# tqch/v-diffusion-torch

Measured on AMD Instinct MI355X. Metric: train_images_per_sec, higher is better.
Workload: dtype fp32 (bf16x3 split products in the tile-engine GEMMs)

## Files before the change

### include/vdiff_hip.h

```cpp
#ifndef VDIFF_HIP_H
#define VDIFF_HIP_H
#include <stddef.h>
#include <stdint.h>

#ifdef __cplusplus
extern "C" {
#endif

#define VD_VERSION 100

int         vd_version(void);
const char* vd_last_error(void);

int         vd_set_reserved_cus(int32_t n);
int         vd_reserved_cus(void);

int         vd_mfma_calibrate(float* sink, unsigned long long* stamps, int32_t blocks, int32_t iters, uint32_t seed, void* stream);

enum { VD_ROW = 0,
       VD_COL = 1,
       VD_IM2COL = 2 };

typedef struct vd_gemm_desc {
    const float* A; const float* B; float* C;
// ... 23 lines not shown
size_t vd_gemm_grouped_wgrad_ws_bytes(int32_t count, int32_t M, int32_t N, int32_t splitk);
int vd_gemm_grouped_wgrad_auto_split(int32_t count, int32_t M, int32_t N, int32_t K, int32_t min_slabs, int32_t max_slabs);
int vd_gemm_grouped_wgrad(const float* const* A, const float* const* B, float* const* C, float* const* colsum, int32_t count,
                          int32_t M, int32_t N, int32_t K, int64_t lda, int64_t ldb, int64_t ldc, int32_t splitk, float* ws, size_t ws_bytes,
                          void* stream);

int vd_conv3x3(const float* xin, int64_t ldx, const float* wpack, const float* bias,
               const float* res, int64_t ldres, float* y, int64_t ldy,
               int32_t nimg, int32_t H, int32_t W, int32_t Cin, int32_t Cout, int32_t accumulate,
               float* stats_part , void* stream);

int vd_conv3x3_wino_supported(int32_t nimg, int32_t H, int32_t W, int32_t Cin, int32_t Cout, int64_t ldx, int64_t ldy, int64_t ldres);
int vd_conv3x3_wino(const float* xin, int64_t ldx, const float* U, const float* bias, const float* res, int64_t ldres,
                    float* y, int64_t ldy, int32_t nimg, int32_t H, int32_t W, int32_t Cin, int32_t Cout,
                    float* stats_part, void* stream);
int vd_conv3x3_wgrad_wino_supported(int32_t nimg, int32_t H, int32_t W, int32_t Cin, int32_t Cout, int64_t ldx, int64_t lddy);
size_t vd_conv3x3_wgrad_wino_ws_bytes(int32_t nimg, int32_t H, int32_t W, int32_t Cin, int32_t Cout);
int vd_conv3x3_wgrad_wino(const float* xin, int64_t ldx, const float* dy, int64_t lddy, int32_t nimg, int32_t H, int32_t W,
                          int32_t Cin, int32_t Cout, float* dw_oihw, float* dbias, int32_t Cin_w, int32_t Cout_w,
                          int32_t accumulate, float* ws, size_t ws_bytes, void* stream);
int vd_conv3x3_wgrad_wino_phase(const float* xin, int64_t ldx, const float* dy, int64_t lddy, int32_t nimg, int32_t H, int32_t W,
                                int32_t Cin, int32_t Cout, float* dw_oihw, float* dbias, int32_t Cin_w, int32_t Cout_w,
                                int32_t accumulate, float* ws, size_t ws_bytes, int32_t phase, void* stream);
int vd_wino_last_kernel(void);
int vd_wino_wgrad_last_kernel(void);
#ifdef VD_PROBES
int vd_wino_set_probe(unsigned long long* buf);
int vd_wino43_set_probe(unsigned long long* buf);
int vd_gn_set_spin_probe(unsigned* buf);
#endif
int vd_wino_pack(const float* w_oihw, int32_t Cout, int32_t Cin, float* uf , float* ud , void* stream);
int vd_conv3x3_dgrad_wino43_supported(int32_t nimg, int32_t H, int32_t W, int32_t Cin, int32_t Cout, int64_t lddy, int64_t lddx);
size_t vd_wino43_u_floats(int32_t Cout, int32_t Cin);
int vd_conv3x3_dgrad_wino43(const float* dy, int64_t lddy, const float* U43, float* dx, int64_t lddx, int32_t nimg, int32_t H, int32_t W,
                            int32_t Cin, int32_t Cout, void* stream);
int vd_wino43_last_kernel(void);
int vd_wino43_pack(const float* w_oihw, int32_t Cout, int32_t Cin, float* U43, void* stream);
int vd_wino43_pack_batched(const int64_t* items_dev, int32_t n, int64_t total_blocks, void* stream);
int vd_conv3x3_wino43_preferred(int32_t nimg, int32_t H, int32_t W, int32_t N);
int vd_conv3x3_wino43_fwd_supported(int32_t nimg, int32_t H, int32_t W, int32_t Cin, int32_t Cout, int64_t ldx, int64_t ldy, int64_t ldres);
int vd_wino43_pack_fwd(const float* w_oihw, int32_t Cout, int32_t Cin, float* U43f, void* stream);
int vd_conv3x3_wino43_fwd_chunk_rows(int32_t H, int32_t W);
int vd_conv3x3_wino43_fwd(const float* xin, int64_t ldx, const float* U43f, const float* bias, const float* res, int64_t ldres, float* y,
                          int64_t ldy, int32_t nimg, int32_t H, int32_t W, int32_t Cin, int32_t Cout, float* stats_part, void* stream);
int vd_conv3x3_wgrad_wino43_supported(int32_t nimg, int32_t H, int32_t W, int32_t Cin, int32_t Cout, int64_t ldx, int64_t lddy);
size_t vd_conv3x3_wgrad_wino43_ws_bytes(int32_t nimg, int32_t H, int32_t W, int32_t Cin, int32_t Cout);
int vd_conv3x3_wgrad_wino43(const float* xin, int64_t ldx, const float* dy, int64_t lddy, int32_t nimg, int32_t H, int32_t W,
                            int32_t Cin, int32_t Cout, float* dw_oihw, float* dbias, int32_t Cin_w, int32_t Cout_w,
                            int32_t accumulate, float* ws, size_t ws_bytes, void* stream);
int vd_conv3x3_wgrad_wino43_phase(const float* xin, int64_t ldx, const float* dy, int64_t lddy, int32_t nimg, int32_t H, int32_t W,
                                  int32_t Cin, int32_t Cout, float* dw_oihw, float* dbias, int32_t Cin_w, int32_t Cout_w,
                                  int32_t accumulate, float* ws, size_t ws_bytes, int32_t phase, void* stream);
int vd_wino43_wgrad_last_kernel(void);

int vd_wino_pack_batched(const int64_t* items_dev, int32_t n, int64_t total_blocks, void* stream);

int vd_im2col3x3(const float* x, int64_t ldx, float* xc , int32_t nimg, int32_t H, int32_t W, int32_t C, void* stream);
int vd_tap_gather(const float* z, int64_t ldz, const float* bias, float* out, int64_t ldo, int32_t nimg, int32_t H, int32_t W, int32_t Cout, void* stream);
int vd_tap_spread(const float* dy, int64_t lddy, float* dz, int64_t ldz, int32_t nimg, int32_t H, int32_t W, int32_t Cout, void* stream);
int vd_thin_wgrad_finish(const float* g, int32_t Cout_w, int32_t Cin, int32_t Cin_w, float* dw_oihw, int32_t accumulate,
                         const float* colsum, int32_t cs_stride, int32_t cs_off, float* dbias, void* stream);

size_t vd_conv3x3_wgrad_ws_bytes(int32_t nimg, int32_t H, int32_t W, int32_t Cin, int32_t Cout);
int vd_conv3x3_wgrad(const float* xin, int64_t ldx, const float* dy, int64_t lddy,
                     int32_t nimg, int32_t H, int32_t W, int32_t Cin, int32_t Cout,
                     float* dw_oihw, float* dbias, int32_t Cin_w, int32_t Cout_w, int32_t accumulate,
                     float* ws, size_t ws_bytes, void* stream);
int vd_conv3x3_wgrad_phase(const float* xin, int64_t ldx, const float* dy, int64_t lddy,
                           int32_t nimg, int32_t H, int32_t W, int32_t Cin, int32_t Cout,
                           float* dw_oihw, float* dbias, int32_t Cin_w, int32_t Cout_w, int32_t accumulate,
                           float* ws, size_t ws_bytes, int32_t phase, void* stream);

int vd_pack_conv3x3(const float* w_oihw, int32_t Cout_w, int32_t Cin_w,
                    float* wf, int32_t Cin_p, float* wd, int32_t Cout_p, void* stream);
int vd_pack_conv3x3_batched(const int64_t* items_dev, int32_t n, int64_t total_blocks, void* stream);

enum { VD_RS_NONE = 0, VD_RS_DOWN = 1, VD_RS_UP = 2 };

size_t vd_gn_ws_bytes(int32_t nimg, int32_t HW, int32_t C);
int vd_gn_stats(const float* x, int64_t ldx, int32_t nimg, int32_t HW, int32_t C, int32_t G, float eps,
                float* stats, float* ws, size_t ws_bytes, void* stream);

int vd_gn_stats_from_partials(const float* part1, int32_t C1, int32_t chunks1, const float* part2, int32_t C2, int32_t chunks2,
                              int32_t nimg, int32_t HW, int32_t G, float eps, float* stats, void* stream);

int vd_gn_coef_from_partials(const float* part1, int32_t C1, int32_t chunks1, const float* part2, int32_t C2, int32_t chunks2,
                             int32_t nimg, int32_t HW, int32_t G, float eps, const float* gamma, const float* beta,
                             const float* film, float* coef, void* stream);

int vd_gn_apply(const float* x, int64_t ldx, const float* stats, const float* gamma, const float* beta,
                const float* film, int32_t act, float p_drop, uint64_t seed,
                int32_t resample, float* y, int64_t ldy,
                int32_t nimg, int32_t H, int32_t W, int32_t C, int32_t G, float* coef, void* stream);

int vd_gn_apply_from_partials(const float* x, int64_t ldx, const float* part1, int32_t C1, int32_t chunks1, const float* part2, int32_t C2,
                              int32_t chunks2, const float* gamma, const float* beta, const float* film, int32_t act, float p_drop,
                              uint64_t seed, int32_t resample, float* y, int64_t ldy, int32_t nimg, int32_t H, int32_t W, int32_t C,
                              int32_t G, float eps, float* coef, void* stream);

int vd_gn_apply_bwd(const float* dy, int64_t lddy, const float* x, int64_t ldx, const float* coef,
                    const float* gamma, const float* beta, const float* film, int32_t act, float p_drop, uint64_t seed,
                    int32_t resample, const float* add, int64_t ldadd, float* dx, int64_t lddx, int32_t accumulate_dx,
                    float* dfilm, float* dgamma, float* dbeta, int32_t accumulate_params,
                    int32_t nimg, int32_t H, int32_t W, int32_t C, int32_t G,
                    float* ws, size_t ws_bytes, void* stream);
int vd_gn_bwd_last_kernel(void);
int vd_gn_apply_bwd_keep(const float* dy, int64_t lddy, const float* x, int64_t ldx, const float* coef, const float* gamma,
                         const float* beta, const float* film, int32_t act, float p_drop, uint64_t seed, int32_t resample,
                         const float* add, int64_t ldadd, float* dx, int64_t lddx, int32_t accumulate_dx, float* dfilm, float* pgb_keep,
                         int32_t nimg, int32_t H, int32_t W, int32_t C, int32_t G, float* ws, size_t ws_bytes, void* stream);
int vd_gn_param_sums_batched(const int64_t* items_dev, int32_t n, int64_t total_blocks, void* stream);

size_t vd_colsum_ws_bytes(int64_t M, int32_t N);
int vd_colsum(const float* x, int64_t ldx, int64_t M, int32_t N, float* out, int32_t accumulate,
              float* ws, size_t ws_bytes, void* stream);
int vd_axpby(const float* x, int64_t ldx, float alpha, float* y, int64_t ldy, float beta, int64_t rows, int32_t C, void* stream);
int vd_silu(const float* x, float* y, int64_t n, void* stream);
int vd_silu_bwd(const float* x, const float* dy, float* dx, int64_t n, int32_t accumulate, void* stream);
int vd_softmax_rows(float* s, int64_t rows, int32_t L, void* stream);
int vd_softmax_rows_bwd(const float* p, float* dp, int64_t rows, int32_t L, float alpha, void* stream);

int vd_attn_supported(int32_t L, int32_t hd, int32_t backward);
int vd_attn_fwd(const float* q, const float* k, const float* v, int64_t ld, float* o, int64_t ldo, float* lse, int32_t B,
                int32_t nh, int32_t L, int32_t hd, float scale, void* stream);
int vd_attn_bwd(const float* q, const float* k, const float* v, int64_t ld, const float* o, int64_t ldo, const float* dout,
                int64_t lddo, const float* lse, float* delta, float* dq, float* dk, float* dv, int64_t ldd, int32_t B,
                int32_t nh, int32_t L, int32_t hd, float scale, void* stream);
int vd_attn_bwd_phase(const float* q, const float* k, const float* v, int64_t ld, const float* o, int64_t ldo, const float* dout,
                      int64_t lddo, const float* lse, float* delta, float* dq, float* dk, float* dv, int64_t ldd, int32_t B,
                      int32_t nh, int32_t L, int32_t hd, float scale, int32_t phase, void* stream);

int vd_nchw_to_nhwc(const float* x, float* y, int32_t nimg, int32_t C, int32_t H, int32_t W, int64_t ldy, void* stream);
int vd_nhwc_to_nchw(const float* x, int64_t ldx, float* y, int32_t nimg, int32_t C, int32_t H, int32_t W, void* stream);

int vd_images_to_uint8_hwc(const float* x_nchw, uint8_t* out_hwc, int32_t n, int32_t C, int32_t HW, void* stream);
int vd_images_from_uint8_hwc(const uint8_t* in_hwc, const uint8_t* flip, float* out_nchw, int32_t n, int32_t C,
                             int32_t H, int32_t W, void* stream);

int vd_timestep_embedding(const double* t, float* out, int32_t n, int32_t dim, double scale, void* stream);
int vd_class_embed(const float* y, const float* w, const float* bias, float* temb, int32_t n, int32_t emb, int32_t ncls, void* stream);
int vd_class_embed_bwd(const float* y, const float* dtemb, float* dw, float* dbias, int32_t n, int32_t emb, int32_t ncls,
                       int32_t accumulate, void* stream);
int vd_multitag_norm(const float* y, float* out, int32_t n, int32_t ncls, void* stream);

int vd_q_sample(const float* x0, const float* eps, const float* logsnr, float* xt, int32_t n, int32_t C, int32_t HW, void* stream);
int vd_loss_fwd(const float* x0, const float* eps, const float* xt, const float* out, const float* logsnr,
                int32_t model_out_type, int32_t reweight, float* loss, float* aux, int32_t n, int32_t C, int32_t HW, void* stream);
int vd_loss_bwd(const float* x0, const float* eps, const float* xt, const float* out, const float* logsnr,
                const float* aux, const float* gloss, int32_t model_out_type, int32_t reweight, float* dout,
                int32_t n, int32_t C, int32_t HW, void* stream);
int vd_bpd_terms(const float* x0, const float* xt, const float* out, const float* coef, int32_t model_out_type, int32_t clip,
// ... 36 lines not shown
```

### v-diffusion-torch_amd/csrc/common.h

```cpp
#pragma once
#include <hip/hip_runtime.h>
#include <stdint.h>
#include <stdio.h>
#include "../../include/vdiff_hip.h"

typedef float f32x4 __attribute__((ext_vector_type(4)));
typedef float f32x16 __attribute__((ext_vector_type(16)));

typedef float f32x2 __attribute__((ext_vector_type(2)));

#ifdef VD_PROBES
constexpr bool VD_PROBE_BUILD = true;
#else
constexpr bool VD_PROBE_BUILD = false;
#endif

void vd_set_error(const char* fmt, ...);
int vd_cu_count(void);
int vd_persistent_cus(void);
int vd_gemm_grouped_wgrad_kblk(const float* const* A, const float* const* B, float* const* C, float* const* colsum, int32_t count, int32_t M,
                               int32_t N, int32_t K, int64_t lda, int64_t ldb, int64_t ldc, int32_t splitk, float* ws, size_t ws_bytes,
                               void* stream, int64_t a_kblk, int64_t b_kblk, int32_t slabs_only);
int vd_gemm_grouped_wgrad_used_slabs(int32_t count, int32_t M, int32_t N, int32_t K, int32_t splitk);
extern thread_local int vd_g_last_tile;
inline int vd_tile_code(bool tr, bool spl, int kt, int bm, int bn) {
    return ((((tr ? 1 : 0) + (spl ? 2 : 0)) * 100 + kt) * 1000 + bm) * 1000 + bn;
}

#define VD_REQUIRE(cond, ...)                                   \
    do { if (!(cond)) { vd_set_error(__VA_ARGS__); return 1; } } while (0)

#define VD_LAUNCH_CHECK(name)                                                            \
    do { hipError_t e_ = hipGetLastError();                                              \
         if (e_ != hipSuccess) { vd_set_error("%s: %s", name, hipGetErrorString(e_)); return 2; } } while (0)

static inline bool vd_aligned16(const void* p) { return (reinterpret_cast<uintptr_t>(p) & 15) == 0; }

__device__ __forceinline__ float vd_sigmoid(float x) { return __builtin_amdgcn_rcpf(1.0f + __expf(-x)); }

__device__ __forceinline__ void vd_philox4(uint64_t seed, uint64_t ctr, uint32_t out[4]) {
    uint32_t k0 = (uint32_t)seed, k1 = (uint32_t)(seed >> 32);
    uint32_t c0 = (uint32_t)ctr, c1 = (uint32_t)(ctr >> 32), c2 = 0x243F6A88u, c3 = 0x85A308D3u;
#pragma unroll
    for (int r = 0; r < 10; ++r) {
        uint64_t p0 = (uint64_t)0xD2511F53u * c0, p1 = (uint64_t)0xCD9E8D57u * c2;
        uint32_t n0 = (uint32_t)(p1 >> 32) ^ c1 ^ k0, n2 = (uint32_t)(p0 >> 32) ^ c3 ^ k1;
        c1 = (uint32_t)p1; c3 = (uint32_t)p0; c0 = n0; c2 = n2;
        k0 += 0x9E3779B9u; k1 += 0xBB67AE85u;
    }
    out[0] = c0; out[1] = c1; out[2] = c2; out[3] = c3;
}
__device__ __forceinline__ f32x4 vd_dropout_scale4(uint64_t seed, uint64_t vec_index, float p) {
    uint32_t r[4];
    vd_philox4(seed, vec_index, r);
    const float inv = 1.0f / (1.0f - p);
    f32x4 m;
#pragma unroll
    for (int j = 0; j < 4; ++j) m[j] = ((r[j] >> 8) * (1.0f / 16777216.0f) >= p) ? inv : 0.0f;
    return m;
}
```

### v-diffusion-torch_amd/csrc/gemm.hip

```cpp
#include "common.h"
#include <math.h>
#include <stdlib.h>
#include <type_traits>

namespace {

constexpr int KT = 32;
#ifndef VD_GEMM_SPLIT_DEFAULT
#define VD_GEMM_SPLIT_DEFAULT 1
#endif

struct GemmArgs {
    const float* A; const float* B; float* C; const float* bias; const float* R;
    int M, N, K;
    long long lda, ldb, ldc, ldr;
    int nh;
    long long sAb, sAh, sBb, sBh, sCb, sCh, sRb, sRh;
    float alpha; int accumulate;
    int H, W, Cin;
    int kt_total, kt_per_split;
    long long slab_stride;
    float* colsum; int colsum_accumulate;
    int probe;
    float* stats; int stats_hw;
    long long sBias;
    int group_S;
    int lgW, lgHW;
    long long a_kblk, b_kblk;
};

__device__ __forceinline__ int PB(const GemmArgs& p) { return VD_PROBE_BUILD ? p.probe : 0; }

__device__ __forceinline__ int row_swz(int row, int chunk) { return row * KT + ((chunk ^ ((row >> 1) & 7)) << 2); }

template <int BM, int BN, int AK, int BK, bool SPLITK>
__global__ __launch_bounds__(256, 2) void gemm_kernel(const GemmArgs p) {
    __shared__ __attribute__((aligned(16))) float smem[2 * (BM + BN) * KT];
    float* As = smem;
    float* Bs = smem + 2 * BM * KT;

    constexpr int MT = BM / 64, NT = BN / 64;
    constexpr int AIT = BM / 32, BIT = BN / 32;
    constexpr int A_CPR = BM / 4, A_RPP = 256 / A_CPR;
    constexpr int B_CPR = BN / 4, B_RPP = 256 / B_CPR;

    const int tid = threadIdx.x, lane = tid & 63, wave = tid >> 6;
    const int li = lane & 31, lh = lane >> 5;
    const int wm = (wave >> 1) * (BM / 2), wn = (wave & 1) * (BN / 2);
    const int m0 = blockIdx.y * BM;
    int n0 = blockIdx.x * BN;
    int tapN = 0, ci0 = 0;
    if (BK == VD_IM2COL) {
        const int cchN = (p.Cin + BN - 1) / BN;
        tapN = blockIdx.x / cchN;
        ci0 = (blockIdx.x % cchN) * BN;
        n0 = tapN * p.Cin + ci0;
    }
    const float* A = p.A;
    const float* B = p.B;
    float* C = p.C;
    const float* R = p.R;
    const float* biasp = p.bias;
    int kt_begin = 0, kt_end = p.kt_total;
    if (SPLITK) {
        kt_begin = blockIdx.z * p.kt_per_split;
        kt_end = min(kt_begin + p.kt_per_split, p.kt_total);
        C += (long long)blockIdx.z * p.slab_stride;
    } else {
        const int zb = blockIdx.z / p.nh, zh = blockIdx.z % p.nh;
        A += zb * p.sAb + zh * p.sAh;
        B += zb * p.sBb + zh * p.sBh;
        C += zb * p.sCb + zh * p.sCh;
        if (R) R += zb * p.sRb + zh * p.sRh;
        if (biasp) biasp += zb * p.sBias;
    }

    const int r_row = tid >> 3, r_chunk = tid & 7;
    int ay[AIT], ax[AIT];
    if (AK == VD_IM2COL) {
#pragma unroll
        for (int it = 0; it < AIT; ++it) {
// ... 338 lines not shown
    } else {
        const int zb = tbz / p.nh, zh = tbz % p.nh;
        A += zb * p.sAb + zh * p.sAh;
        B += zb * p.sBb + zh * p.sBh;
        C += zb * p.sCb + zh * p.sCh;
        if (R) R += zb * p.sRb + zh * p.sRh;
        if (biasp) biasp += zb * p.sBias;
    }

    unsigned voA[AIT], voB[BIT];
    unsigned mkA[AIT];
    int kcA[AIT], kcB[BIT];
    int by[BIT], bx[BIT];
    int tapA = (AK == VD_IM2COL) ? kt_begin % 9 : 0, ccA = (AK == VD_IM2COL) ? kt_begin / 9 : 0;
    const int kinc_x = (BK == VD_IM2COL) ? KT % p.W : 0, kinc_y = (BK == VD_IM2COL) ? KT / p.W : 0;
#pragma unroll
    for (int j = 0; j < AIT; ++j) {
        const int q = j * 4 + wave;
        if (AK == VD_COL) {
            const int kk = q * A_RPP + lane / A_LPR, cm = (lane % A_LPR) * 4;
            const int rowoff = (GROUPED && p.a_kblk) ? (kk >> 4) * (int)p.a_kblk + (kk & 15) * (int)p.lda : kk * (int)p.lda;
            voA[j] = (m0 + cm < p.M) ? (unsigned)(rowoff + cm) * 4u : OOB;
            kcA[j] = kk; mkA[j] = 0;
        } else {
            const int row = q * RRPP + lane / RLPR;
            const int c = (lane % RLPR) ^ swz_of<KT>(row);
            const int m = m0 + row;
            kcA[j] = c * 4;
            voA[j] = (m < p.M) ? (unsigned)(row * (int)p.lda + c * 4) * 4u : OOB;
            unsigned mk = 0;
            if (AK == VD_IM2COL) {
                int y, x;
                pix_yx(p, m, y, x);
                const unsigned xm = (x > 0 ? 1u : 0u) | 2u | (x < p.W - 1 ? 4u : 0u);
                mk = (y > 0 ? xm : 0u) | (xm << 3) | (y < p.H - 1 ? xm << 6 : 0u);
            }
            mkA[j] = mk;
        }
    }
#pragma unroll
    for (int j = 0; j < BIT; ++j) {
        const int q = j * 4 + wave;
        if (BK == VD_ROW) {
            const int row = q * RRPP + lane / RLPR;
            const int c = (lane % RLPR) ^ swz_of<KT>(row);
            kcB[j] = c * 4;
            voB[j] = (n0 + row < p.N) ? (unsigned)(row * (int)p.ldb + c * 4) * 4u : OOB;
            by[j] = bx[j] = 0;
        } else {
            const int kk = q * B_RPP + lane / B_LPR, cn = (lane % B_LPR) * 4;
            kcB[j] = kk;
            const bool ok = (BK == VD_IM2COL) ? (ci0 + cn < p.Cin) : (n0 + cn < p.N);
            const int rowoff = (GROUPED && BK == VD_COL && p.b_kblk) ? (kk >> 4) * (int)p.b_kblk + (kk & 15) * (int)p.ldb : kk * (int)p.ldb;
            voB[j] = ok ? (unsigned)(rowoff + cn) * 4u : OOB;
            if (BK == VD_IM2COL) pix_yx(p, kt_begin * KT + kk, by[j], bx[j]);
            else by[j] = bx[j] = 0;
        }
    }
    const float* Ablk = (AK == VD_COL) ? A + m0 : A + (long long)m0 * p.lda;
    const float* Bblk = (BK == VD_ROW) ? B + (long long)n0 * p.ldb : ((BK == VD_COL) ? B + n0 : B + ci0);
    const long long tapoffB = (BK == VD_IM2COL) ? (long long)((tapN / 3 - 1) * p.W + (tapN % 3 - 1)) * p.ldb : 0;

#ifndef VD_ISSUE_IN
#define VD_ISSUE_IN 2
#endif
    constexpr bool ISSUE_IN = VD_ISSUE_IN == 2 ? (AK == VD_COL) : (VD_ISSUE_IN == 1);
    struct Prep { const float* pA; const float* pB; unsigned vA[AIT], vB[BIT]; };
    auto prep_tiles = [&](int kt, Prep& P) {
        {
            const int tap = tapA, c0 = ccA * KT;
            long long aoff;
            int kwidth;
            if (AK == VD_IM2COL) { aoff = (long long)((tap / 3 - 1) * p.W + (tap % 3 - 1)) * p.lda + c0; kwidth = p.Cin - c0; }
            else if (AK == VD_ROW) { aoff = (long long)kt * KT; kwidth = p.K - kt * KT; }
            else { aoff = (GROUPED && p.a_kblk) ? (long long)kt * (KT / 16) * p.a_kblk : (long long)kt * KT * p.lda; kwidth = p.K - kt * KT; }
            P.pA = Ablk + aoff;
#pragma unroll
            for (int j = 0; j < AIT; ++j) {
                unsigned vo = voA[j];
                if (kcA[j] >= kwidth) vo = OOB;
                if (AK == VD_IM2COL && !((mkA[j] >> tap) & 1u)) vo = OOB;
                P.vA[j] = vo;
            }
        }
        {
            long long boff;
            int kwidth;
            if (BK == VD_ROW) {
                if (AK == VD_IM2COL) { boff = (long long)tapA * p.Cin + ccA * KT; kwidth = p.Cin - ccA * KT; }
                else { boff = (long long)kt * KT; kwidth = p.K - kt * KT; }
            } else { boff = ((GROUPED && BK == VD_COL && p.b_kblk) ? (long long)kt * (KT / 16) * p.b_kblk : (long long)kt * KT * p.ldb) + tapoffB; kwidth = p.K - kt * KT; }
            P.pB = Bblk + boff;
            const int dy = tapN / 3 - 1, dx = tapN % 3 - 1;
            if (BK == VD_IM2COL && p.lgW >= 0) {
#pragma unroll
                for (int j = 0; j < BIT; ++j) {
                    const int k0 = kt * KT + (j * 4 + wave) * B_RPP;
                    unsigned long long lanes = 0;
#pragma unroll
                    for (int u = 0; u < B_RPP; ++u) {
                        const int k = k0 + u;
                        const int rem = k & ((1 << p.lgHW) - 1), y = (rem >> p.lgW) + dy, x = (rem & ((1 << p.lgW) - 1)) + dx;
                        const bool ok = k < p.K && (unsigned)y < (unsigned)p.H && (unsigned)x < (unsigned)p.W;
                        lanes |= ok ? (((B_LPR == 64 ? 0ull : (1ull << (B_LPR & 63))) - 1ull) << (u * (B_LPR & 63))) : 0ull;
                    }
                    unsigned vo;
                    const unsigned oob = OOB;
                    asm("v_cndmask_b32 %0, %1, %2, %3" : "=v"(vo) : "v"(oob), "v"(voB[j]), "s"(lanes));
                    P.vB[j] = vo;
                }
            } else
#pragma unroll
            for (int j = 0; j < BIT; ++j) {
// ... 359 lines not shown
                    v = (v * al + bb) + ad;
                    if (want_stats) {
                        if (!edge) { st1p += v; st2p += v * v; }
                        else {
                            if (rs0 + row_lane < rows_valid) { st1 += v[0]; st2 += v[0] * v[0]; }
                            if (rs1 + row_lane < rows_valid) { st1 += v[1]; st2 += v[1] * v[1]; }
                        }
                    }
                }
                const float v0 = v[0], v1 = v[1];
                __builtin_amdgcn_raw_buffer_store_b32(__float_as_uint(v0), crs, (int)voc, rs0 * ldc4, 0);
                __builtin_amdgcn_raw_buffer_store_b32(__float_as_uint(v1), crs, (int)voc, rs1 * ldc4, 0);
            }
        }
        st1 += st1p[0] + st1p[1];
        st2 += st2p[0] + st2p[1];
        if (want_stats && nok) {
            st1 += __shfl_xor(st1, 32, 64);
            st2 += __shfl_xor(st2, 32, 64);
            const int mrow = m0 + wm;
            if (lh == 0 && mrow < p.M) {
                const int chunks = p.stats_hw / (BM / 2);
                float* o = p.stats + ((long long)(mrow / p.stats_hw) * chunks + (mrow % p.stats_hw) / (BM / 2)) * 2 * p.N + n;
                o[0] = st1; o[p.N] = st2;
            }
        }
    }
    stamp_end();
}

template <int BM, int BN, int AK, int BK, bool SPLITK, int KT, bool TR, bool GROUPED = false>
__global__ __launch_bounds__(256, (KT == 16 ? VD_KT16_BLOCKS : 2)) void gemm_dma_kernel(const GemmArgs p,
                                                                                          const std::conditional_t<GROUPED, GroupPtrs, NoGroup> gp) {
    gemm_dma_body<BM, BN, AK, BK, SPLITK, KT, TR, GROUPED, false>(p, gp);
}
template <int BM, int BN, int AK, int BK, bool SPLITK, int KT, bool TR, bool GROUPED = false>
__global__ __launch_bounds__(256, (KT == 16 ? VD_SPL_BLOCKS : 2)) void gemm_split_kernel(const GemmArgs p,
                                                                                           const std::conditional_t<GROUPED, GroupPtrs, NoGroup> gp) {
    gemm_dma_body<BM, BN, AK, BK, SPLITK, KT, TR, GROUPED, true>(p, gp);
}

__global__ __launch_bounds__(512) void wgrad_planes256_kernel(const GemmArgs p, const GroupPtrs gp) {
    constexpr int BM = 256, BN = 256, KTT = 16, NBUF = 3, STG = (BM + BN) * KTT;
    __shared__ __attribute__((aligned(1024))) float smem[NBUF * STG];
    typedef float f32x2 __attribute__((ext_vector_type(2)));
    const int tid = threadIdx.x, lane = tid & 63;
    const int wave = __builtin_amdgcn_readfirstlane(tid >> 6);
    const int li = lane & 31, lh = lane >> 5;
    const int wm = (wave >> 1) * 64, wn = (wave & 1) * 128;
    const int tbx = blockIdx.x, tby = blockIdx.y, tbz = blockIdx.z;
    const int m0 = tby * BM, n0 = tbx * BN;
    const int e = tbz / p.group_S, slab = tbz - e * p.group_S;
    const float* A = gp.A[e] + m0;
    const float* B = gp.B[e] + n0;
    const int kt_begin = slab * p.kt_per_split, kt_end = min(kt_begin + p.kt_per_split, p.kt_total);
    float* C = p.C + (long long)tbz * p.slab_stride;

    auto issue = [&](int kt, int buf) {
        float* as = smem + buf * STG;
        float* bs = as + BM * KTT;
        const int rec = kt < kt_end ? (int)OOB : 0;
        const __amdgpu_buffer_rsrc_t rsA = make_rsrc(A + (p.a_kblk ? (long long)kt * p.a_kblk : (long long)kt * KTT * p.lda), rec);
        const __amdgpu_buffer_rsrc_t rsB = make_rsrc(B + (p.b_kblk ? (long long)kt * p.b_kblk : (long long)kt * KTT * p.ldb), rec);
#pragma unroll
        for (int h = 0; h < 2; ++h) {
            const int kk = wave + 8 * h;
            __builtin_amdgcn_raw_ptr_buffer_load_lds(rsA, (lds_ptr_t)(as + kk * BM), 16, lane * 16, kk * (int)p.lda * 4, 0, 0);
            __builtin_amdgcn_raw_ptr_buffer_load_lds(rsB, (lds_ptr_t)(bs + kk * BN), 16, lane * 16, kk * (int)p.ldb * 4, 0, 0);
        }
    };

    f32x16 acc[2][4];
#pragma unroll
    for (int a = 0; a < 2; ++a)
#pragma unroll
        for (int b = 0; b < 4; ++b)
#pragma unroll
            for (int r = 0; r < 16; ++r) acc[a][b][r] = 0.f;
    float csum[2] = {0.f, 0.f};
    const bool do_cs = p.colsum != nullptr && tbx == 0 && (wave & 1) == 0;

    if (kt_begin < kt_end) {
        issue(kt_begin, 0);
        issue(kt_begin + 1, 1);
        asm volatile("s_waitcnt vmcnt(4)" ::: "memory");
        asm volatile("s_waitcnt lgkmcnt(0)\n\ts_barrier" ::: "memory");
        int buf = 0;
        for (int kt = kt_begin; kt < kt_end; ++kt) {
            const float* as = smem + buf * STG;
            const float* bs = as + BM * KTT;
            issue(kt + 2, buf >= 1 ? buf - 1 : 2);
            float fa[2][8];
            f32x4 fbq[8];
#pragma unroll
            for (int j = 0; j < 8; ++j) {
                const f32x2 v = *reinterpret_cast<const f32x2*>(as + (8 * lh + j) * BM + wm + 2 * li);
                fa[0][j] = v[0]; fa[1][j] = v[1];
                fbq[j] = *reinterpret_cast<const f32x4*>(bs + (8 * lh + j) * BN + wn + 4 * li);
            }
            bf16x8 ah[2], am[2], al[2];
#pragma unroll
            for (int a = 0; a < 2; ++a) split8(fa[a], ah[a], am[a], al[a]);
            if (do_cs) {
                asm volatile("" ::: "memory");
#pragma unroll
                for (int a = 0; a < 2; ++a)
                    csum[a] += ((fa[a][0] + fa[a][1]) + (fa[a][2] + fa[a][3])) + ((fa[a][4] + fa[a][5]) + (fa[a][6] + fa[a][7]));
            }
#pragma unroll
            for (int hb = 0; hb < 2; ++hb) {
                bf16x8 bh[2], bm[2], bl[2];
#pragma unroll
                for (int b2 = 0; b2 < 2; ++b2) {
                    float fb[8];
#pragma unroll
                    for (int j = 0; j < 8; ++j) fb[j] = fbq[j][2 * hb + b2];
                    split8(fb, bh[b2], bm[b2], bl[b2]);
                }
#pragma unroll
                for (int a = 0; a < 2; ++a)
#pragma unroll
// ... 360 lines not shown
        if (eff > best) best = eff;
    }
    return best >= 0.85;
}

void grouped_tiles(int tile, bool p256, int M, int N, long long* nm, long long* nn) {
    const int bm = p256 ? 256 : TILES[tile].bm, bn = p256 ? 256 : TILES[tile].bn;
    *nm = (M + bm - 1) / bm; *nn = (N + bn - 1) / bn;
}

struct GroupedPlan { int tile; bool p256, k16; long long nm, nn; int kt_total, kt_per_split, used; };
GroupedPlan plan_grouped(int count, int M, int N, int K, int S) {
    GroupedPlan g;
    g.tile = choose_tile(M, N, false, (long long)count * S, 0);
    g.p256 = planes256(count, M, N, K);
    grouped_tiles(g.tile, g.p256, M, N, &g.nm, &g.nn);
    g.k16 = g.p256 || (g.tile == 0 && g.nm * g.nn * count * S >= GROUPED_K16_MIN_WGS);
    g.kt_total = g.k16 ? (K + 15) / 16 : (K + 31) / 32;
    g.kt_per_split = (g.kt_total + S - 1) / S;
    g.used = (g.kt_total + g.kt_per_split - 1) / g.kt_per_split;
    return g;
}
}

extern "C" int vd_gemm_grouped_wgrad_auto_split(int32_t count, int32_t M, int32_t N, int32_t K, int32_t min_slabs, int32_t max_slabs) {
    const int tile = choose_tile(M, N, false, (long long)count * 8, 0);
    const bool p256 = planes256(count, M, N, K);
    long long nm, nn;
    grouped_tiles(tile, p256, M, N, &nm, &nn);
    const long long blocks = nm * nn * count;
    const long long slots = (long long)vd_cu_count() * (p256 ? 1 : (tile == 0 && blocks * (min_slabs > 1 ? min_slabs : 1) >= GROUPED_K16_MIN_WGS / 2 ? 4 : TILES[tile].per_cu));
    int lo = min_slabs > 1 ? min_slabs : 1, hi = max_slabs > lo ? max_slabs : lo;
    const int kmax = K / 256 > 1 ? K / 256 : 1;
    if (hi > kmax) hi = kmax;
    if (lo > hi) lo = hi;
    int best = lo;
    double best_eff = -1.0;
    for (int s = lo; s <= hi; ++s) {
        const long long wgs = blocks * s, rounds = (wgs + slots - 1) / slots;
        double eff = (double)wgs / (double)(rounds * slots);
        eff *= 1.0 - 0.004 * s;
        if (eff > best_eff) { best_eff = eff; best = s; }
    }
    return best;
}

extern "C" size_t vd_gemm_grouped_wgrad_ws_bytes(int32_t count, int32_t M, int32_t N, int32_t splitk) {
    return (size_t)count * (splitk > 1 ? splitk : 1) * ((size_t)M * N + M) * sizeof(float);
}

extern "C" int vd_gemm_grouped_wgrad(const float* const* A, const float* const* B, float* const* C, float* const* colsum, int32_t count,
                                     int32_t M, int32_t N, int32_t K, int64_t lda, int64_t ldb, int64_t ldc, int32_t splitk, float* ws,
                                     size_t ws_bytes, void* stream) {
    return vd_gemm_grouped_wgrad_kblk(A, B, C, colsum, count, M, N, K, lda, ldb, ldc, splitk, ws, ws_bytes, stream, 0, 0, 0);
}

int vd_gemm_grouped_wgrad_used_slabs(int32_t count, int32_t M, int32_t N, int32_t K, int32_t splitk) {
    return plan_grouped(count, M, N, K, splitk > 1 ? splitk : 1).used;
}

int vd_gemm_grouped_wgrad_kblk(const float* const* A, const float* const* B, float* const* C, float* const* colsum, int32_t count,
                               int32_t M, int32_t N, int32_t K, int64_t lda, int64_t ldb, int64_t ldc, int32_t splitk, float* ws,
                               size_t ws_bytes, void* stream, int64_t a_kblk, int64_t b_kblk, int32_t slabs_only) {
    VD_REQUIRE(A && B && C && count > 0 && count <= VD_GROUP_MAX, "vd_gemm_grouped_wgrad: 1..%d entries (got %d)", VD_GROUP_MAX, count);
    VD_REQUIRE(M > 0 && N > 0 && K > 0 && M % 4 == 0 && N % 4 == 0 && lda % 4 == 0 && ldb % 4 == 0 && ldc >= N,
               "vd_gemm_grouped_wgrad: M, N, lda, ldb must be multiples of 4 (M=%d N=%d)", M, N);
    const int S = splitk > 1 ? splitk : 1;
    VD_REQUIRE(ws && ws_bytes >= vd_gemm_grouped_wgrad_ws_bytes(count, M, N, S), "vd_gemm_grouped_wgrad: workspace too small");
    GemmArgs a = {};
    GroupPtrs gp = {};
    GroupOut go = {};
    for (int e = 0; e < count; ++e) {
        VD_REQUIRE(A[e] && B[e] && C[e] && vd_aligned16(A[e]) && vd_aligned16(B[e]), "vd_gemm_grouped_wgrad: entry %d: null / unaligned operand", e);
        gp.A[e] = A[e]; gp.B[e] = B[e]; go.C[e] = C[e]; go.cs[e] = colsum ? colsum[e] : nullptr;
    }
    a.A = A[0]; a.B = B[0];
    a.M = M; a.N = N; a.K = K; a.lda = lda; a.ldb = ldb; a.ldc = N; a.ldr = 0; a.nh = 1;
    a.alpha = 1.f; a.lgW = a.lgHW = -1; a.probe = 0;
    a.a_kblk = a_kblk; a.b_kblk = b_kblk;
    VD_REQUIRE(a_kblk >= 0 && b_kblk >= 0 && a_kblk % 4 == 0 && b_kblk % 4 == 0 && 2 * a_kblk + 16 * lda + 128 < 0x70000000LL / 4 &&
               2 * b_kblk + 16 * ldb + 128 < 0x70000000LL / 4, "vd_gemm_grouped_wgrad: K-block strides outside the LDS-DMA kernel's range");
    VD_REQUIRE(dma_in_range(a), "vd_gemm_grouped_wgrad: operands outside the LDS-DMA kernel's range (alignment / row pitch)");
    const GroupedPlan g = plan_grouped(count, M, N, K, S);
    const int used = g.used;
    a.kt_total = g.kt_total; a.kt_per_split = g.kt_per_split; a.group_S = used;
    a.slab_stride = (long long)M * N;
    a.C = ws;
    float* cpart = ws + (long long)count * used * a.slab_stride;
    a.colsum = colsum ? cpart : nullptr;
    const dim3 grid((unsigned)g.nn, (unsigned)g.nm, (unsigned)(count * used));
    hipStream_t st = (hipStream_t)stream;
    if (g.p256) {
        vd_g_last_tile = vd_tile_code(true, true, 16, 256, 256);
        hipLaunchKernelGGL(wgrad_planes256_kernel, grid, dim3(512), 0, st, a, gp);
    } else if (g.tile == 0 && g.k16) launch_grouped<128, 128, 16>(a, gp, grid, st);
    else if (g.tile == 0) launch_grouped<128, 128>(a, gp, grid, st);
    else if (g.tile == 1) launch_grouped<128, 64>(a, gp, grid, st);
    else if (g.tile == 2) launch_grouped<64, 128>(a, gp, grid, st);
    else launch_grouped<64, 64>(a, gp, grid, st);
    VD_LAUNCH_CHECK("gemm_dma_kernel(grouped)");
    if (slabs_only) return 0;
    const long long tot = (long long)M * N;
    hipLaunchKernelGGL(reduce_slabs_grouped_kernel, dim3((unsigned)((tot + 255) / 256), (unsigned)count), dim3(256), 0, st, ws, used,
                       a.slab_stride, M, N, go, (long long)ldc, cpart);
    VD_LAUNCH_CHECK("reduce_slabs_grouped_kernel");
    return 0;
}

thread_local int vd_g_last_tile = 0;
extern "C" int vd_gemm_last_tile(void) { return vd_g_last_tile; }

extern "C" int vd_gemm(const vd_gemm_desc* d, void* stream) {
    VD_REQUIRE(d != nullptr, "vd_gemm: null descriptor");
    return run_gemm(*d, (hipStream_t)stream);
}

extern "C" int vd_conv3x3(const float* xin, int64_t ldx, const float* wpack, const float* bias, const float* res,
                          int64_t ldres, float* y, int64_t ldy, int32_t nimg, int32_t H, int32_t W, int32_t Cin,
                          int32_t Cout, int32_t accumulate, float* stats_part, void* stream) {
    VD_REQUIRE(Cin % 4 == 0, "vd_conv3x3: Cin must be a multiple of 4 (got %d)", Cin);
    vd_gemm_desc d = {};
    d.A = xin; d.B = wpack; d.C = y; d.bias = bias; d.R = res;
    d.M = nimg * H * W; d.N = Cout; d.K = 9 * Cin;
    d.a_kind = VD_IM2COL; d.b_kind = VD_ROW;
    d.lda = ldx; d.ldb = 9LL * Cin; d.ldc = ldy; d.ldr = ldres;
    d.batch = 1; d.nh = 1; d.alpha = 1.f; d.accumulate = accumulate;
    d.H = H; d.W = W; d.Cin = Cin;
    d.stats = stats_part; d.stats_hw = H * W;
    if (stats_part && (H * W) % 64 != 0) d.tile = 64;
    return run_gemm(d, (hipStream_t)stream);
}

// ... 107 lines not shown
```

### v-diffusion-torch_amd/csrc/norm.hip

```cpp
#include "common.h"
#include <stdlib.h>

namespace {

constexpr int PPC = 128;

template <bool NT>
__device__ __forceinline__ f32x4 ld_stream(const float* p) {
    if (NT) return __builtin_nontemporal_load(reinterpret_cast<const f32x4*>(p));
    return *reinterpret_cast<const f32x4*>(p);
}
template <bool NT>
__device__ __forceinline__ void st_stream(float* p, f32x4 v) {
    if (NT) __builtin_nontemporal_store(v, reinterpret_cast<f32x4*>(p));
    else *reinterpret_cast<f32x4*>(p) = v;
}

struct ReduceArgs {
    const float* x; long long ldx;
    const float* dy; long long lddy;
    const float* coef;
    int act; float p_drop; unsigned long long seed; int resample; int has_norm;
    int H, W;
    long long HW;
// ... 134 lines not shown
    const int idx = blockIdx.x * 4 + (threadIdx.x >> 6), lane = threadIdx.x & 63;
    if (idx >= nimg * G) return;
    const int b = idx / G, g = idx % G, C = C1 + C2, cg = C / G;
    double s1 = 0.0, s2 = 0.0;
    const int cbeg = g * cg;
    const int n1 = ch1 * cg, n2 = ch2 * cg;
    for (int e = lane; e < max(n1, n2); e += 64) {
        const int c = cbeg + e % cg, ch = e / cg;
        const bool first = c < C1;
        const int Cs = first ? C1 : C2, cs = first ? c : c - C1, chunks = first ? ch1 : ch2;
        if (ch < chunks) {
            const float* q = (first ? p1 : p2) + ((long long)(b * chunks + ch) * 2) * Cs + cs;
            s1 += (double)q[0]; s2 += (double)q[Cs];
        }
    }
#pragma unroll
    for (int o = 32; o > 0; o >>= 1) { s1 += __shfl_xor(s1, o, 64); s2 += __shfl_xor(s2, o, 64); }
    const double n = (double)cg * (double)HW;
    const double mean_d = s1 / n;
    double var = s2 / n - mean_d * mean_d;
    if (var < 0.0) var = 0.0;
    const float mean = (float)mean_d, rstd = (float)(1.0 / sqrt(var + (double)eps));
    if (stats && lane == 0) { stats[2 * idx] = mean; stats[2 * idx + 1] = rstd; }
    if (coef) {
        for (int c = cbeg + lane; c < cbeg + cg; c += 64) {
            float sc = rstd * gamma[c];
            float of = beta[c] - mean * sc;
            if (film) {
                const float shift = film[(long long)b * 2 * C + c], scale = film[(long long)b * 2 * C + C + c];
                sc *= (1.f + scale);
                of = of * (1.f + scale) + shift;
            }
            float* o = coef + (long long)b * 4 * C + c;
            o[0] = sc; o[C] = of; o[2 * C] = rstd; o[3 * C] = -mean * rstd;
        }
    }
}

__global__ void gn_coef_kernel(const float* stats, const float* gamma, const float* beta, const float* film, int nimg,
                               int C, int G, float* coef) {
    const int idx = blockIdx.x * blockDim.x + threadIdx.x;
    if (idx >= nimg * C) return;
    const int b = idx / C, c = idx % C, g = c / (C / G);
    const float mean = stats[2 * (b * G + g)], rstd = stats[2 * (b * G + g) + 1];
    float sc = rstd * gamma[c];
    float of = beta[c] - mean * sc;
    if (film) {
        const float shift = film[(long long)b * 2 * C + c], scale = film[(long long)b * 2 * C + C + c];
        sc *= (1.f + scale);
        of = of * (1.f + scale) + shift;
    }
    float* o = coef + (long long)b * 4 * C + c;
    o[0] = sc; o[C] = of; o[2 * C] = rstd; o[3 * C] = -mean * rstd;
}

struct ApplyArgs {
    const float* x; long long ldx; const float* coef; int has_norm; int act; float p_drop; unsigned long long seed;
    int resample; float* y; long long ldy; int nimg, H, W, C;
};
struct PartArgs {
    const float* p1; int C1, ch1; const float* p2; int C2, ch2; int G; float eps;
    const float* gamma; const float* beta; const float* film; float* coef_out;
};

__device__ __forceinline__ f32x4 fwd_val(const ApplyArgs& p, f32x4 v, int pix, int c4, f32x4 sc, f32x4 of, int b) {
    if (p.has_norm) v = v * sc + of;
    if (p.act) {
#pragma unroll
        for (int j = 0; j < 4; ++j) v[j] = v[j] * vd_sigmoid(v[j]);
    }
    if (p.p_drop > 0.f) {
        const unsigned long long vi = ((unsigned long long)b * p.H * p.W + pix) * (p.C >> 2) + (c4 >> 2);
        v *= vd_dropout_scale4(p.seed, vi, p.p_drop);
    }
    return v;
}
__device__ __forceinline__ f32x4 fwd_one(const ApplyArgs& p, const float* ximg, int pix, int c4, f32x4 sc, f32x4 of, int b) {
    return fwd_val(p, *reinterpret_cast<const f32x4*>(ximg + (long long)pix * p.ldx + c4), pix, c4, sc, of, b);
}

constexpr int APIX = 64;

template <bool FROM_PARTS>
__global__ __launch_bounds__(256) void gn_apply_kernel(const ApplyArgs p, int Cb, const PartArgs q) {
    __shared__ double ps[FROM_PARTS ? 2 : 1][FROM_PARTS ? 1024 : 1];
    __shared__ float gst[FROM_PARTS ? 2 : 1][FROM_PARTS ? 256 : 1];
    const int b = blockIdx.y, c0 = blockIdx.z * Cb;
    const int cbw = min(Cb, p.C - c0);
    const int vecs = cbw >> 2, rows = 256 / vecs;
    const int r = threadIdx.x / vecs, c4 = c0 + 4 * (threadIdx.x % vecs);
    const int Ho = p.resample == VD_RS_DOWN ? p.H >> 1 : (p.resample == VD_RS_UP ? p.H << 1 : p.H);
    const int Wo = p.resample == VD_RS_DOWN ? p.W >> 1 : (p.resample == VD_RS_UP ? p.W << 1 : p.W);
    const int p0 = blockIdx.x * APIX, np = min(APIX, Ho * Wo - p0);
    f32x4 sc = {1.f, 1.f, 1.f, 1.f}, of = {0.f, 0.f, 0.f, 0.f};
    if (FROM_PARTS) {
        const int C = p.C, cg = C / q.G;
        for (int cl = threadIdx.x; cl < cbw; cl += 256) {
            const int c = c0 + cl;
            const bool first = c < q.C1;
            const int Cs = first ? q.C1 : q.C2, cs = first ? c : c - q.C1, chunks = first ? q.ch1 : q.ch2;
            const float* src = (first ? q.p1 : q.p2) + (long long)b * chunks * 2 * Cs + cs;
            double s1 = 0.0, s2 = 0.0;
            for (int ch = 0; ch < chunks; ++ch) { s1 += (double)src[(long long)ch * 2 * Cs]; s2 += (double)src[(long long)ch * 2 * Cs + Cs]; }
            ps[0][cl] = s1; ps[1][cl] = s2;
        }
        __syncthreads();
        const int ng = cbw / cg;
        for (int g = threadIdx.x; g < ng; g += 256) {
            double s1 = 0.0, s2 = 0.0;
            for (int c = g * cg; c < (g + 1) * cg; ++c) { s1 += ps[0][c]; s2 += ps[1][c]; }
            const double n = (double)cg * (double)p.H * (double)p.W;
            const double mean = s1 / n;
            double var = s2 / n - mean * mean;
            if (var < 0.0) var = 0.0;
            gst[0][g] = (float)mean; gst[1][g] = (float)(1.0 / sqrt(var + (double)q.eps));
        }
        __syncthreads();
        if (r >= rows) return;
        f32x4 nr, nm;
#pragma unroll
        for (int j = 0; j < 4; ++j) {
            const int c = c4 + j, g = (c - c0) / cg;
            const float mean = gst[0][g], rstd = gst[1][g];
            float s_ = rstd * q.gamma[c];
            float o_ = q.beta[c] - mean * s_;
            if (q.film) {
                const float shift = q.film[(long long)b * 2 * C + c], scale = q.film[(long long)b * 2 * C + C + c];
                s_ *= (1.f + scale);
                o_ = o_ * (1.f + scale) + shift;
            }
            sc[j] = s_; of[j] = o_; nr[j] = rstd; nm[j] = -mean * rstd;
        }
        if (blockIdx.x == 0 && r == 0 && q.coef_out) {
            float* o = q.coef_out + (long long)b * 4 * C + c4;
            *reinterpret_cast<f32x4*>(o) = sc; *reinterpret_cast<f32x4*>(o + C) = of;
            *reinterpret_cast<f32x4*>(o + 2 * C) = nr; *reinterpret_cast<f32x4*>(o + 3 * C) = nm;
        }
    } else {
        if (r >= rows) return;
        if (p.has_norm) {
            const float* cf = p.coef + (long long)b * 4 * p.C;
            sc = *reinterpret_cast<const f32x4*>(cf + c4);
            of = *reinterpret_cast<const f32x4*>(cf + p.C + c4);
        }
    }
    const float* ximg = p.x + (long long)b * p.H * p.W * p.ldx;
    float* yimg = p.y + (long long)b * Ho * Wo * p.ldy;
    if (p.resample == VD_RS_NONE) {
        for (int i = r; i < np; i += 4 * rows) {
            f32x4 v[4];
#pragma unroll
            for (int u = 0; u < 4; ++u)
                if (i + u * rows < np) v[u] = *reinterpret_cast<const f32x4*>(ximg + (long long)(p0 + i + u * rows) * p.ldx + c4);
#pragma unroll
            for (int u = 0; u < 4; ++u)
                if (i + u * rows < np) {
                    const int po = p0 + i + u * rows;
                    *reinterpret_cast<f32x4*>(yimg + (long long)po * p.ldy + c4) = fwd_val(p, v[u], po, c4, sc, of, b);
                }
        }
        return;
    }
    for (int i = r; i < np; i += rows) {
        const int po = p0 + i;
        f32x4 out;
        {
            const int yo = po / Wo, xo = po - yo * Wo;
            if (p.resample == VD_RS_UP) out = fwd_one(p, ximg, (yo >> 1) * p.W + (xo >> 1), c4, sc, of, b);
            else {
                const int q = (2 * yo) * p.W + 2 * xo;
                out = (fwd_one(p, ximg, q, c4, sc, of, b) + fwd_one(p, ximg, q + 1, c4, sc, of, b) +
                       fwd_one(p, ximg, q + p.W, c4, sc, of, b) + fwd_one(p, ximg, q + p.W + 1, c4, sc, of, b)) * 0.25f;
            }
        }
        *reinterpret_cast<f32x4*>(yimg + (long long)po * p.ldy + c4) = out;
    }
}

__global__ __launch_bounds__(256) void gn_bwd_finalize_kernel(const float* part, int chunks, const float* coef,
                                                              const float* gamma, const float* beta, const float* film,
                                                              int C, int G, long long HW, float* q, float* dfilm,
                                                              float* pgb) {
    extern __shared__ float sh[];
    float* k1 = sh; float* k2 = sh + C; float* gm = sh + 2 * C;
    const int b = blockIdx.x, cg = C / G;
    const float* cf = coef + (long long)b * 4 * C;
    for (int c = threadIdx.x; c < C; c += blockDim.x) {
        float s1 = 0.f, s2 = 0.f;
        for (int ch = 0; ch < chunks; ++ch) {
            const float* pp = part + ((long long)(b * chunks + ch) * 2) * C;
            s1 += pp[c]; s2 += pp[C + c];
        }
        float fs = 1.f;
        if (film) {
            fs = 1.f + film[(long long)b * 2 * C + C + c];
            dfilm[(long long)b * 2 * C + c] = s1;
            dfilm[(long long)b * 2 * C + C + c] = gamma[c] * s2 + beta[c] * s1;
        }
        const float k = gamma[c] * fs;
        k1[c] = k * s1; k2[c] = k * s2;
        pgb[((long long)b * 2) * C + c] = fs * s2;
        pgb[((long long)b * 2 + 1) * C + c] = fs * s1;
    }
    __syncthreads();
    if (threadIdx.x < G) {
        float m1 = 0.f, m2 = 0.f;
        for (int c = threadIdx.x * cg; c < (threadIdx.x + 1) * cg; ++c) { m1 += k1[c]; m2 += k2[c]; }
        const float inv = 1.f / ((float)cg * (float)HW);
        gm[threadIdx.x] = m1 * inv; gm[G + threadIdx.x] = m2 * inv;
    }
    __syncthreads();
    for (int c = threadIdx.x; c < C; c += blockDim.x) {
        const int g = c / cg;
        const float rstd = cf[2 * C + c];
        const float fs = film ? 1.f + film[(long long)b * 2 * C + C + c] : 1.f;
        float* qq = q + (long long)b * 3 * C + c;
        qq[0] = rstd * gamma[c] * fs; qq[C] = rstd * gm[g]; qq[2 * C] = rstd * gm[G + g];
    }
}

__global__ __launch_bounds__(256) void sum_over_images_kernel(const float* pgb, int nimg, int C, float* dgamma, float* dbeta,
                                                              int accumulate) {
    __shared__ float sh[2][16][17];
    const int cx = threadIdx.x & 15, ly = threadIdx.x >> 4;
    const int c = blockIdx.x * 16 + cx;
    float a = 0.f, bsum = 0.f;
    if (c < C)
        for (int b = ly; b < nimg; b += 16) { a += pgb[((long long)b * 2) * C + c]; bsum += pgb[((long long)b * 2 + 1) * C + c]; }
// ... 405 lines not shown
}

extern "C" int vd_gn_apply(const float* x, int64_t ldx, const float* stats, const float* gamma, const float* beta,
                           const float* film, int32_t act, float p_drop, uint64_t seed, int32_t resample, float* y,
                           int64_t ldy, int32_t nimg, int32_t H, int32_t W, int32_t C, int32_t G, float* coef,
                           void* stream) {
    hipStream_t st = (hipStream_t)stream;
    VD_REQUIRE(C % 4 == 0 && ldx % 4 == 0 && ldy % 4 == 0, "vd_gn_apply: C/ld must be multiples of 4");
    VD_REQUIRE(resample != VD_RS_DOWN || (H % 2 == 0 && W % 2 == 0), "vd_gn_apply: odd size cannot be average-pooled");
    const int has_norm = gamma != nullptr;
    if (has_norm && !stats) {
        VD_REQUIRE(coef != nullptr, "vd_gn_apply: neither statistics nor a coefficient table given");
    } else if (has_norm) {
        VD_REQUIRE(stats && beta && coef && C % G == 0, "vd_gn_apply: missing norm operands");
        hipLaunchKernelGGL(gn_coef_kernel, dim3((nimg * C + 255) / 256), dim3(256), 0, st, stats, gamma, beta, film, nimg, C,
                           G, coef);
        VD_LAUNCH_CHECK("gn_coef_kernel");
    }
    ApplyArgs p = {x, ldx, coef, has_norm, act, p_drop, seed, resample, y, ldy, nimg, H, W, C};
    const long long Ho = resample == VD_RS_DOWN ? H / 2 : (resample == VD_RS_UP ? H * 2 : H);
    const long long Wo = resample == VD_RS_DOWN ? W / 2 : (resample == VD_RS_UP ? W * 2 : W);
    const int Cba = pick_cb(C);
    VD_REQUIRE(C % Cba == 0 && Cba % 4 == 0 && Cba <= 1024 && nimg <= 65535, "vd_gn_apply: cannot split C=%d / nimg=%d", C, nimg);
    hipLaunchKernelGGL(gn_apply_kernel<false>, dim3((unsigned)((Ho * Wo + APIX - 1) / APIX), nimg, C / Cba), dim3(256), 0, st, p, Cba, PartArgs{});
    VD_LAUNCH_CHECK("gn_apply_kernel");
    return 0;
}

extern "C" int vd_gn_apply_from_partials(const float* x, int64_t ldx, const float* part1, int32_t C1, int32_t chunks1, const float* part2,
                                         int32_t C2, int32_t chunks2, const float* gamma, const float* beta, const float* film, int32_t act,
                                         float p_drop, uint64_t seed, int32_t resample, float* y, int64_t ldy, int32_t nimg, int32_t H,
                                         int32_t W, int32_t C, int32_t G, float eps, float* coef, void* stream) {
    hipStream_t st = (hipStream_t)stream;
    VD_REQUIRE(x && y && part1 && gamma && beta, "vd_gn_apply_from_partials: null operand");
    VD_REQUIRE(C % 4 == 0 && ldx % 4 == 0 && ldy % 4 == 0 && C % G == 0 && C1 + C2 == C && C1 > 0 && chunks1 > 0,
               "vd_gn_apply_from_partials: bad channel split C=%d C1=%d C2=%d G=%d", C, C1, C2, G);
    VD_REQUIRE(C2 == 0 || (part2 && chunks2 > 0), "vd_gn_apply_from_partials: second source incomplete");
    VD_REQUIRE(resample != VD_RS_DOWN || (H % 2 == 0 && W % 2 == 0), "vd_gn_apply_from_partials: odd size cannot be average-pooled");
    VD_REQUIRE(vd_aligned16(x) && vd_aligned16(y) && (!coef || vd_aligned16(coef)), "vd_gn_apply_from_partials: operands must be 16-byte aligned");
    ApplyArgs p = {x, ldx, coef, 1, act, p_drop, seed, resample, y, ldy, nimg, H, W, C};
    PartArgs q = {part1, C1, chunks1, part2, C2, chunks2, G, eps, gamma, beta, film, coef};
    const long long Ho = resample == VD_RS_DOWN ? H / 2 : (resample == VD_RS_UP ? H * 2 : H);
    const long long Wo = resample == VD_RS_DOWN ? W / 2 : (resample == VD_RS_UP ? W * 2 : W);
    const int cg = C / G;
    int Cba = pick_cb(C);
    if (Cba % cg) {
        Cba = 0;
        for (int k = G; k >= 1; --k) if (G % k == 0 && (k * cg) % 4 == 0 && k * cg <= 1024) { Cba = k * cg; break; }
    }
    VD_REQUIRE(Cba > 0 && C % Cba == 0 && Cba % 4 == 0 && Cba % cg == 0 && Cba <= 1024 && Cba / cg <= 256 && nimg <= 65535,
               "vd_gn_apply_from_partials: cannot split C=%d into whole-group channel ranges", C);
    hipLaunchKernelGGL(gn_apply_kernel<true>, dim3((unsigned)((Ho * Wo + APIX - 1) / APIX), nimg, C / Cba), dim3(256), 0, st, p, Cba, q);
    VD_LAUNCH_CHECK("gn_apply_kernel<from partials>");
    return 0;
}

static int gn_apply_bwd_impl(const float* dy, int64_t lddy, const float* x, int64_t ldx, const float* coef,
                             const float* gamma, const float* beta, const float* film, int32_t act, float p_drop,
                             uint64_t seed, int32_t resample, const float* add, int64_t ldadd, float* dx, int64_t lddx,
                             int32_t accumulate_dx, float* dfilm, float* dgamma, float* dbeta, int32_t accumulate_params,
                             int32_t nimg, int32_t H, int32_t W, int32_t C, int32_t G, float* ws, size_t ws_bytes,
                             float* pgb_keep, void* stream) {
    hipStream_t st = (hipStream_t)stream;
    VD_REQUIRE(C % 4 == 0 && lddy % 4 == 0 && lddx % 4 == 0, "vd_gn_apply_bwd: C/ld must be multiples of 4");
    const int has_norm = gamma != nullptr;
    const long long HW = (long long)H * W;
    BwdApplyArgs a = {};
    ReduceArgs& p = a.r;
    p.x = x; p.ldx = ldx; p.dy = dy; p.lddy = lddy; p.coef = coef; p.act = act; p.p_drop = p_drop; p.seed = seed;
    p.resample = resample; p.has_norm = has_norm; p.H = H; p.W = W; p.HW = HW; p.C = C; p.nimg = nimg;
    p.chunks = (int)((HW + PPC - 1) / PPC);
    a.add = add; a.ldadd = ldadd; a.dx = dx; a.lddx = lddx; a.accumulate_dx = accumulate_dx;
    g_last_gn_bwd = has_norm ? -1 : 0;
    if (has_norm) {
        VD_REQUIRE(x && coef && beta && ((dgamma && dbeta) || pgb_keep) && C % G == 0 && ldx % 4 == 0, "vd_gn_apply_bwd: missing norm operands");
        VD_REQUIRE(!film || dfilm, "vd_gn_apply_bwd: film given without dfilm");
        VD_REQUIRE(ws && ws_bytes >= vd_gn_ws_bytes(nimg, (int)HW, C), "vd_gn_apply_bwd: workspace too small");
        const int Cb = pick_cb(C);
        VD_REQUIRE(C % Cb == 0 && Cb % 4 == 0 && Cb <= 1024, "vd_gn_apply_bwd: cannot split C=%d", C);
        float* part = ws;
        float* q = part + (long long)nimg * p.chunks * 2 * C;
        float* pgb = pgb_keep ? pgb_keep : q + (long long)nimg * 3 * C;
        p.part = part;
        static const bool two_pass = getenv("VD_GN_TWO_PASS") != nullptr;
        int CS = fused_slab(C, G);
        static const bool wide = !(getenv("VD_GN_WIDE") && atoi(getenv("VD_GN_WIDE")) == 0);
        if (wide && CS > 0 && CS % 32 != 0 && C >= 384) {
            const int cg = C / G;
            for (int k = 1; k * cg <= 128 && k <= G; ++k)
                if ((k * cg) % 32 == 0 && C % (k * cg) == 0) { CS = k * cg; break; }
        }
        if (!two_pass && CS > 0 && nimg <= 65535) {
            static const bool big = getenv("VD_GN_TPB") && atoi(getenv("VD_GN_TPB")) == 1024;
            const int TPB = (HW * (CS / 4) > 2048 || (big && HW * (CS / 4) >= 1024)) ? 1024 : 256;
            const int rows = TPB / (CS / 4);
            const int npt = (int)((HW + rows - 1) / rows);
            static const bool no_split = getenv("VD_GN_SPLIT") && atoi(getenv("VD_GN_SPLIT")) == 0;
            if (npt > 8 && !no_split && resample == VD_RS_NONE && CS % 32 == 0) {
                int nsplit = 0;
                for (int k = 2; k <= 32; k *= 2)
                    if (HW % k == 0 && (HW / k + (1024 / (CS / 4)) - 1) / (1024 / (CS / 4)) <= 8) { nsplit = k; break; }
                const long long units = (long long)nimg * (C / CS), upad = (units + 7) / 8 * 8;
                const size_t cnt_bytes = ((size_t)upad * sizeof(unsigned) + 255) / 256 * 256;
                static const int split_occ = [] {
                    int occ = 0;
                    if (hipOccupancyMaxActiveBlocksPerMultiprocessor(&occ, gn_bwd_fused_kernel<8, 1024, true, true>, 1024, 0) != hipSuccess) occ = 0;
// ... 105 lines not shown
```

### v-diffusion-torch_amd/csrc/wino43.hip

```cpp
#include "common.h"
#include <type_traits>

namespace {

typedef __attribute__((address_space(3))) void* lds_ptr_t;
constexpr unsigned OOB = 0x80000000u;
constexpr int KT = 8;
constexpr int TN = 32;
constexpr int TILES = 64;
constexpr int U_STAGE = 36 * 4 * 16 * 2 * 2;
constexpr int THREADS = 512;

struct Args43 {
    const float* x; long long ldx;
    const float* U;
    float* y; long long ldy;
    int nimg, H, W, K, N;
    int items_per_img;
    int ngrp;
    int ncb, nitems;
    const float* bias; const float* res; long long ldr;
    float* stats;
    int chunks_per_img;
    unsigned long long* probe;
// ... 9 lines not shown
constexpr int U_AHEAD = 2;
template <int HALF, bool DY, typename T>
__device__ __forceinline__ void bt_half(const T (&d)[6], T& o0, T& o1, T& o2) {
    if (DY) {
        if (HALF == 0) {
            const T e1 = d[4] - 2.25f * d[2], f1 = d[3] - 2.25f * d[1];
            o0 = 1.265625f * d[0] + (d[4] - 2.8125f * d[2]);
            o1 = e1 + 0.75f * f1;
            o2 = e1 - 0.75f * f1;
        } else {
            const T e2 = d[4] - 0.5625f * d[2], f2 = d[3] - 0.5625f * d[1];
            o0 = e2 + 1.5f * f2;
            o1 = e2 - 1.5f * f2;
            o2 = 1.265625f * d[1] + (d[5] - 2.8125f * d[3]);
        }
    } else if (HALF == 0) {
        const T t = d[4] - 4.f * d[2], u = d[3] - 4.f * d[1];
        o0 = 4.f * d[0] + (d[4] - 5.f * d[2]);
        o1 = t + u;
        o2 = t - u;
    } else {
        const T c = d[4] - d[2], e = d[3] - d[1];
        o0 = c + 2.f * e;
        o1 = c - 2.f * e;
        o2 = 4.f * d[1] + (d[5] - 5.f * d[3]);
    }
}
template <bool DY, typename T>
__device__ __forceinline__ void bt_full(const T (&r)[6], T (&v)[6]) {
    if (DY) {
        const T e1 = r[4] - 2.25f * r[2], f1 = r[3] - 2.25f * r[1];
        const T e2 = r[4] - 0.5625f * r[2], f2 = r[3] - 0.5625f * r[1];
        v[0] = 1.265625f * r[0] + (r[4] - 2.8125f * r[2]);
        v[1] = e1 + 0.75f * f1;
        v[2] = e1 - 0.75f * f1;
        v[3] = e2 + 1.5f * f2;
        v[4] = e2 - 1.5f * f2;
        v[5] = 1.265625f * r[1] + (r[5] - 2.8125f * r[3]);
        return;
    }
    const T t = r[4] - 4.f * r[2], u = r[3] - 4.f * r[1], c = r[4] - r[2], e = r[3] - r[1];
    v[0] = 4.f * r[0] + (r[4] - 5.f * r[2]);
    v[1] = t + u;
    v[2] = t - u;
    v[3] = c + 2.f * e;
    v[4] = c - 2.f * e;
    v[5] = 4.f * r[1] + (r[5] - 5.f * r[3]);
}
template <int HALF, bool DY>
__device__ __forceinline__ void bt_half2(const f32x2 (&d)[6], f32x2& o0, f32x2& o1, f32x2& o2) { bt_half<HALF, DY, f32x2>(d, o0, o1, o2); }
template <bool DY>
__device__ __forceinline__ void bt_full2(const f32x2 (&r)[6], f32x2 (&v)[6]) { bt_full<DY, f32x2>(r, v); }

template <int TWT, bool FWD>
__global__ __launch_bounds__(THREADS) void wino43_conv_kernel(const Args43 p) {
    constexpr bool QUAD = TWT == 4;
    constexpr int RUN = TWT + 1;
    constexpr int RUNS = QUAD ? 4 * RUN - 2 : 4 * RUN;
    constexpr int RP = QUAD ? RUNS + 1 : RUNS + ((TWT / 4) & 3);
    constexpr int NTR = TILES / TWT;
    constexpr int RIN = QUAD ? 4 * 17 + 1 : 4 * NTR + 2;
    constexpr int NS = RIN * RP;
    constexpr int NPG = (NS + 63) / 64;
    constexpr int A_STAGE = 2 * NPG * 256;
    constexpr int STAGE = A_STAGE + U_STAGE;
    constexpr int LGT = TWT == 4 ? 2 : TWT == 8 ? 3 : 4;
    static_assert((4 * RP * 16) % 256 == (TWT * 16) % 256 || (QUAD && (4 * RP * 16) % 256 == 192), "row pitch leaves bank conflicts");
    static_assert(2 * STAGE * 4 <= 163840, "stages exceed the LDS");
    static_assert(8 * 16 * 64 * 16 + 8 * 4 * 8 * 4 <= 2 * STAGE * 4, "epilogue exchange + statistics area exceeds the stages");
    __shared__ __attribute__((aligned(1024))) float smem[2 * STAGE];

    const int tid = threadIdx.x, lane = tid & 63;
    const int wave = __builtin_amdgcn_readfirstlane(tid >> 6);
    const int li = lane & 15, lq = lane >> 4;
    const int tg = wave & 3;
    const int nkt = p.K / KT;
    const int G = gridDim.x;
    int probe_n = 0;
    auto stamp = [&](int slot) {
        if (VD_PROBE_BUILD && p.probe && probe_n < 4) {
            const unsigned long long t = slot == 12 ? __builtin_amdgcn_s_memrealtime() : __builtin_amdgcn_s_memtime();
            if (lane == 0) p.probe[(((long long)blockIdx.x * 8 + wave) * 4 + probe_n) * 16 + slot] = t;
        }
    };
    auto stamp_val = [&](int slot, unsigned long long v) {
        if (VD_PROBE_BUILD && p.probe && probe_n < 4 && lane == 0) p.probe[(((long long)blockIdx.x * 8 + wave) * 4 + probe_n) * 16 + slot] = v;
    };

    constexpr int APL = (NPG + 3) / 4;
    unsigned pxo[APL];
    const float* xitem = p.x;
    auto offsets = [&](int grp) {
        const int img = grp / p.items_per_img;
        const int part = grp - img * p.items_per_img;
        const int y_first = 4 * NTR * part - 1;
#pragma unroll
        for (int j = 0; j < APL; ++j) {
            const int s = (wave >> 1) + 4 * j;
            const int slot = s * 64 + lane;
            const int r = slot / RP, cs = slot - r * RP;
            int c, idx, yy, im;
            if (QUAD) {
                c = cs >= 3 * RUN - 1 ? 3 : cs >= 2 * RUN ? 2 : cs >= RUN ? 1 : 0;
                idx = cs - (c * RUN - (c == 3 ? 1 : 0));
                const int i4 = r / 17;
                im = i4; yy = r - 17 * i4 - 1;
                if (i4 >= 4) yy = -1;
            } else {
                c = cs / RUN; idx = cs - c * RUN;
                im = 0; yy = y_first + r;
            }
            const int xx = 4 * idx + c - 1;
            unsigned vo = OOB;
            if (s < NPG && r < RIN && cs < RUNS && (unsigned)xx < (unsigned)p.W && (unsigned)yy < (unsigned)p.H)
                vo = (unsigned)(((im * p.H + yy) * p.W + xx) * (int)p.ldx) * 4u;
            pxo[j] = vo;
        }
    };
    auto issue_piece = [&](int i, int kt, int st, int cb) {
        float* sb = smem + st * STAGE;
        if (i < 5) {
            const int q = wave + 8 * i;
            if (q < 36) {
                const float* src = p.U + ((long long)cb * nkt + kt) * U_STAGE;
                const __amdgpu_buffer_rsrc_t rs = make_rsrc(src);
                __builtin_amdgcn_raw_ptr_buffer_load_lds(rs, (lds_ptr_t)(sb + A_STAGE + q * 256), 16, lane * 16, q * 1024, 0, 0);
            }
        } else {
            const int j = i - 5;
            const int s = (wave >> 1) + 4 * j, g = wave & 1;
            if (s < NPG) {
                const __amdgpu_buffer_rsrc_t rs = make_rsrc(xitem + kt * KT);
                __builtin_amdgcn_raw_ptr_buffer_load_lds(rs, (lds_ptr_t)(sb + (g * NPG + s) * 256), 16, (int)pxo[j], g * 16, 0, 0);
            }
        }
    };
    constexpr int NPIECE = 5 + APL;
    constexpr int SB = SB_STEP, NAFTER = 18 - SB, PAFTER = NAFTER;
    constexpr int UPF = U_AHEAD;
    static_assert(PAFTER <= NPIECE && NPIECE - PAFTER <= SB, "DMA schedule does not fit the tile");

    const int tl = 16 * tg + li;
    const int tyl = tl >> LGT, tx = tl & (TWT - 1);
    const int prow0 = QUAD ? 17 * (tyl >> 2) + 4 * (tyl & 3) : 4 * tyl;
    const int pbase = ((lq >> 1) * NPG * 64 + prow0 * RP + tx) * 4 + (lq & 1) * 2;
    auto poff = [](int pr, int q) { return (pr * RP + ((q & 3) * RUN - (QUAD && (q & 3) == 3 ? 1 : 0)) + (q >> 2)) * 4; };
    const int uoff = A_STAGE + lane * 4;

    const int ngrp = p.ngrp;
    auto item_of = [&](int n, int& cb, int& grp) -> bool {
        int t = n * G + (int)blockIdx.x;
        if ((G & 7) == 0 && (n + 1) * G <= p.nitems) t = n * G + ((int)blockIdx.x & 7) * (G >> 3) + ((int)blockIdx.x >> 3);
        if (t >= p.nitems) return false;
        if ((p.ncb & 3) == 0 && (ngrp & 7) == 0) {
            const int c = t >> 5, i = t & 31, ncg = p.ncb >> 2;
            cb = (c % ncg) * 4 + (i & 3); grp = (c / ncg) * 8 + (i >> 2);
            return true;
        }
        cb = t % p.ncb; grp = t / p.ncb;
        return true;
    };

    auto run = [&](auto Hc) {
        constexpr int HALF = decltype(Hc)::value;
        auto rowpass = [&](const float* sa, f32x2 (&Rn)[3][6], int q0, int q1) {
#pragma unroll
            for (int q = 0; q < 6; ++q) {
                if (q < q0 || q >= q1) continue;
                f32x2 d[6];
#pragma unroll
                for (int pr = 0; pr < 6; ++pr) {
                    if ((HALF == 0 && pr == 5) || (HALF == 1 && pr == 0)) d[pr] = f32x2{0.f, 0.f};
                    else d[pr] = *(const volatile __attribute__((address_space(3))) f32x2*)((const __attribute__((address_space(3))) float*)sa + poff(pr, q));
                }
                bt_half2<HALF, FWD>(d, Rn[0][q], Rn[1][q], Rn[2][q]);
            }
        };
        auto first_stage = [&](int cbx, int grpx) {
            if (QUAD) xitem = p.x + (long long)grpx * (4 * 16 * 16) * p.ldx;
            else { offsets(grpx); xitem = p.x + (long long)(grpx / p.items_per_img) * p.H * p.W * p.ldx; }
#pragma unroll
            for (int i = 0; i < NPIECE; ++i) issue_piece(i, 0, 0, cbx);
        };
        int cb = 0, grp = 0, cb_next = 0, grp_next = 0;
        if (QUAD) offsets(0);
        bool have = item_of(0, cb, grp);
        if (have) first_stage(cb, grp);
        for (int n = 0; have; ++n) {
            probe_n = n;
            stamp(0); stamp(12);
            unsigned long long t_vm = 0, t_bar = 0;
            f32x4 acc[18][2];
#pragma unroll
            for (int x = 0; x < 18; ++x) { acc[x][0] = f32x4{0.f, 0.f, 0.f, 0.f}; acc[x][1] = f32x4{0.f, 0.f, 0.f, 0.f}; }
            if (n == 0) asm volatile("s_waitcnt vmcnt(0)" ::: "memory");
            else asm volatile("s_waitcnt vmcnt(16)" ::: "memory");
            lds_barrier();
            stamp(1);
            if (nkt > 1) {
#pragma unroll
                for (int i = 0; i < PAFTER; ++i) issue_piece(i, 1, 1, cb);
            }
            f32x2 R[3][6];
            rowpass(smem + pbase, R, 0, 6);
            stamp(2);
            for (int kt = 0; kt < nkt; ++kt) {
                const int st = kt & 1;
                const float* su = smem + st * STAGE + uoff;
                const float* san = smem + (st ^ 1) * STAGE + pbase;
                const bool n1 = kt + 1 < nkt, n2 = kt + 2 < nkt;
                f32x2 Rn[3][6];
                f32x4 uf[UPF + 1], ufl[NAFTER];
#pragma unroll
                for (int e = 0; e < UPF; ++e) uf[e] = *reinterpret_cast<const f32x4*>(su + (18 * HALF + e) * 256);
#pragma unroll
                for (int a = 0; a < 3; ++a) {
                    f32x2 V[6];
                    bt_full2<FWD>(R[a], V);
#pragma unroll
                    for (int b = 0; b < 6; ++b) {
                        const int xl = 6 * a + b;
                        if (xl == SB) {
#pragma unroll
                            for (int e = 0; e < NAFTER; ++e) ufl[e] = *reinterpret_cast<const f32x4*>(su + (18 * HALF + SB + e) * 256);
                            if (VD_PROBE_BUILD && p.probe) {
                                const unsigned long long ta = __builtin_amdgcn_s_memtime();
                                asm volatile("s_waitcnt vmcnt(0)" ::: "memory");
                                const unsigned long long tb = __builtin_amdgcn_s_memtime();
                                __syncthreads();
                                const unsigned long long tc = __builtin_amdgcn_s_memtime();
                                t_vm += tb - ta; t_bar += tc - tb;
                            } else {
                                asm volatile("s_waitcnt vmcnt(0)" ::: "memory");
                                __syncthreads();
                            }
                        }
                        if (xl + UPF < SB) uf[(xl + UPF) % (UPF + 1)] = *reinterpret_cast<const f32x4*>(su + (18 * HALF + xl + UPF) * 256);
                        if (xl + PAFTER < NPIECE) { if (n1) issue_piece(xl + PAFTER, kt + 1, st ^ 1, cb); }
                        if (xl >= SB) {
                            if (n2) issue_piece(xl - SB, kt + 2, st, cb);
                            rowpass(san, Rn, (6 * (xl - SB)) / NAFTER, (6 * (xl - SB + 1)) / NAFTER);
                        }
                        const f32x4 u = xl < SB ? uf[xl % (UPF + 1)] : ufl[xl < SB ? 0 : xl - SB];
                        acc[xl][0] = __builtin_amdgcn_mfma_f32_16x16x4f32(u[0], V[b][0], acc[xl][0], 0, 0, 0);
                        acc[xl][1] = __builtin_amdgcn_mfma_f32_16x16x4f32(u[2], V[b][0], acc[xl][1], 0, 0, 0);
                        acc[xl][0] = __builtin_amdgcn_mfma_f32_16x16x4f32(u[1], V[b][1], acc[xl][0], 0, 0, 0);
                        acc[xl][1] = __builtin_amdgcn_mfma_f32_16x16x4f32(u[3], V[b][1], acc[xl][1], 0, 0, 0);
                    }
                }
#pragma unroll
                for (int a = 0; a < 3; ++a)
#pragma unroll
                    for (int q = 0; q < 6; ++q) R[a][q] = Rn[a][q];
            }
            stamp(3);
            __syncthreads();
            stamp(4);

            f32x4* xch = reinterpret_cast<f32x4*>(smem);
            const int lane_e = FWD ? (int)__builtin_amdgcn_mbcnt_hi(~0u, __builtin_amdgcn_mbcnt_lo(~0u, 0u)) : lane;
            const int li_e = lane_e & 15, lq_e = lane_e >> 4;
            const int tl_e = 16 * tg + li_e, tyl_e = tl_e >> LGT, tx_e = tl_e & (TWT - 1);
            f32x4 Y[4][4];
            f32x4 RV[FWD ? 4 : 1][FWD ? 4 : 1];
#pragma unroll
            for (int pass = 0; pass < 2; ++pass) {
                const int blk = pass == 0 ? 1 - HALF : HALF;
                f32x4 S[3][4];
#pragma unroll
                for (int a = 0; a < 3; ++a) {
                    const f32x4 m0 = acc[6 * a][blk], m1 = acc[6 * a + 1][blk], m2 = acc[6 * a + 2][blk], m3 = acc[6 * a + 3][blk],
                                m4 = acc[6 * a + 4][blk], m5 = acc[6 * a + 5][blk];
                    const f32x4 p12 = m1 + m2, q12 = m1 - m2, p34 = m3 + m4, q34 = m3 - m4;
                    S[a][0] = m0 + p12 + p34;
                    if (FWD) {
                        S[a][1] = 0.75f * q12 + 1.5f * q34;
                        S[a][2] = 0.5625f * p12 + 2.25f * p34;
                        S[a][3] = 0.421875f * q12 + 3.375f * q34 + m5;
                    } else {
                        S[a][1] = q12 + 2.f * q34;
                        S[a][2] = p12 + 4.f * p34;
                        S[a][3] = q12 + 8.f * q34 + m5;
                    }
                }
#pragma unroll
                for (int v = 0; v < 4; ++v) {
                    if (HALF == 0) {
                        const f32x4 s12 = S[1][v] + S[2][v], d12 = S[1][v] - S[2][v];
                        if (FWD) { Y[0][v] = S[0][v] + s12; Y[1][v] = 0.75f * d12; Y[2][v] = 0.5625f * s12; Y[3][v] = 0.421875f * d12; }
                        else { Y[0][v] = S[0][v] + s12; Y[1][v] = d12; Y[2][v] = s12; Y[3][v] = d12; }
                    } else {
                        const f32x4 s34 = S[0][v] + S[1][v], d34 = S[0][v] - S[1][v];
                        if (FWD) { Y[0][v] = s34; Y[1][v] = 1.5f * d34; Y[2][v] = 2.25f * s34; Y[3][v] = 3.375f * d34 + S[2][v]; }
                        else { Y[0][v] = s34; Y[1][v] = 2.f * d34; Y[2][v] = 4.f * s34; Y[3][v] = 8.f * d34 + S[2][v]; }
                    }
                }
                if (pass == 0) {
#pragma unroll
                    for (int u = 0; u < 4; ++u)
#pragma unroll
                        for (int v = 0; v < 4; ++v) xch[(wave * 16 + 4 * u + v) * 64 + lane_e] = Y[u][v];
                    if (FWD) {
                        const int img_r = QUAD ? 4 * grp + (tyl_e >> 2) : grp / p.items_per_img;
                        const int part_r = QUAD ? 0 : grp - img_r * p.items_per_img;
                        const int y0r = QUAD ? 4 * (tyl_e & 3) : 4 * (NTR * part_r + tyl_e);
                        const unsigned pixr = (unsigned)(((QUAD ? img_r : 0) * p.H + y0r) * p.W + 4 * tx_e);
// ... 97 lines not shown
    else run(std::integral_constant<int, 1>{});
}

__device__ __forceinline__ void pack43_tile(const float* w, float* U, int Cout, int Cin, int tile, int fwd) {
    const int nkt = (fwd ? Cin : Cout) / KT;
    const int nb = tile / nkt, kt = tile - nb * nkt;
    const int t = threadIdx.x;
    const int kq = t >> 6, n = (t >> 2) & 15, cbk = (t >> 1) & 1, j = t & 1;
    const int cn = nb * 32 + 16 * cbk + n, ck = kt * KT + 2 * kq + j;
    const int ci = fwd ? ck : cn, co = fwd ? cn : ck;
    const float* src = w + ((long long)co * Cin + ci) * 9;
    double g[3][3];
#pragma unroll
    for (int a = 0; a < 3; ++a)
#pragma unroll
        for (int b = 0; b < 3; ++b) g[a][b] = (double)(fwd ? src[a * 3 + b] : src[(2 - a) * 3 + (2 - b)]);
    const double Gc[6][3] = {{0.25, 0.0, 0.0}, {-1.0 / 6, -1.0 / 6, -1.0 / 6}, {-1.0 / 6, 1.0 / 6, -1.0 / 6},
                             {1.0 / 24, 1.0 / 12, 1.0 / 6}, {1.0 / 24, -1.0 / 12, 1.0 / 6}, {0.0, 0.0, 1.0}};
    const double Gd[6][3] = {{64.0 / 81, 0.0, 0.0}, {-128.0 / 243, -32.0 / 81, -8.0 / 27}, {-128.0 / 243, 32.0 / 81, -8.0 / 27},
                             {32.0 / 243, 16.0 / 81, 8.0 / 27}, {32.0 / 243, -16.0 / 81, 8.0 / 27}, {0.0, 0.0, 1.0}};
    double Gm[6][3];
#pragma unroll
    for (int a = 0; a < 6; ++a)
#pragma unroll
        for (int c = 0; c < 3; ++c) Gm[a][c] = fwd ? Gd[a][c] : Gc[a][c];
    double tmp[6][3];
#pragma unroll
    for (int a = 0; a < 6; ++a)
#pragma unroll
        for (int c = 0; c < 3; ++c) tmp[a][c] = Gm[a][0] * g[0][c] + Gm[a][1] * g[1][c] + Gm[a][2] * g[2][c];
    float* dst = U + ((long long)nb * nkt + kt) * U_STAGE + t;
#pragma unroll
    for (int a = 0; a < 6; ++a)
#pragma unroll
        for (int b = 0; b < 6; ++b)
            dst[(6 * a + b) * 256] = (float)(tmp[a][0] * Gm[b][0] + tmp[a][1] * Gm[b][1] + tmp[a][2] * Gm[b][2]);
}

__global__ __launch_bounds__(256) void wino43_pack_kernel(const float* w, float* U, int Cout, int Cin, int fwd) {
    pack43_tile(w, U, Cout, Cin, blockIdx.x, fwd);
}

__global__ __launch_bounds__(256) void wino43_pack_batched_kernel(const long long* items, int n) {
    int lo = 0, hi = n - 1;
    while (lo < hi) {
        const int mid = (lo + hi + 1) >> 1;
        if (items[8 * mid + 7] <= (long long)blockIdx.x) lo = mid; else hi = mid - 1;
    }
    const long long* it = items + 8 * lo;
    pack43_tile(reinterpret_cast<const float*>(it[0]), reinterpret_cast<float*>(it[1]), (int)it[3], (int)it[4],
                (int)((long long)blockIdx.x - it[7]), (int)it[2]);
}

__device__ __forceinline__ void bt6(const f32x4 (&d)[6], f32x4 (&o)[6]) {
    const f32x4 e1 = d[4] - 2.25f * d[2], f1 = 0.75f * d[3] - 1.6875f * d[1];
    const f32x4 e2 = d[4] - 0.5625f * d[2], f2 = 1.5f * d[3] - 0.84375f * d[1];
    o[0] = 1.265625f * d[0] + (d[4] - 2.8125f * d[2]);
    o[1] = e1 + f1;
    o[2] = e1 - f1;
    o[3] = e2 + f2;
    o[4] = e2 - f2;
    o[5] = 1.265625f * d[1] + (d[5] - 2.8125f * d[3]);
}
__device__ __forceinline__ void a6(const f32x4 (&y)[4], f32x4 (&o)[6]) {
    const f32x4 e1 = y[0] + 0.5625f * y[2], f1 = 0.75f * y[1] + 0.421875f * y[3];
    const f32x4 e2 = y[0] + 2.25f * y[2], f2 = 1.5f * y[1] + 3.375f * y[3];
    o[0] = y[0];
    o[1] = e1 + f1;
    o[2] = e1 - f1;
    o[3] = e2 + f2;
    o[4] = e2 - f2;
    o[5] = y[3];
}

__device__ __forceinline__ void st_once(float* p, f32x4 v) { *reinterpret_cast<f32x4*>(p) = v; }
struct WgT43 {
    const float* x; long long ldx; const float* dy; long long lddy;
    float* V; float* dM;
    int nimg, H, W, Cin, Cout, TW, TPI, T;
};

__global__ __launch_bounds__(256) void wino43_wgrad_transform_kernel(const WgT43 p) {
    const int quad = blockIdx.y * 64 + threadIdx.x, tile = blockIdx.x * 4 + threadIdx.y;
    if (tile >= p.T) return;
    const int img = tile / p.TPI, tin = tile - img * p.TPI;
    const int ty = tin / p.TW, tx = tin - ty * p.TW;
    const int c4 = 4 * quad;
    if (blockIdx.z == 0) {
        if (c4 >= p.Cin) return;
        f32x4 R[6][6];
#pragma unroll
        for (int pr = 0; pr < 6; ++pr) {
            const int yy = 4 * ty - 1 + pr;
            f32x4 d[6];
#pragma unroll
            for (int q = 0; q < 6; ++q) {
                const int xx = 4 * tx - 1 + q;
                d[q] = f32x4{0.f, 0.f, 0.f, 0.f};
                if ((unsigned)yy < (unsigned)p.H && (unsigned)xx < (unsigned)p.W)
                    d[q] = *reinterpret_cast<const f32x4*>(p.x + ((long long)(img * p.H + yy) * p.W + xx) * p.ldx + c4);
            }
            bt6(d, R[pr]);
        }
#pragma unroll
        for (int b = 0; b < 6; ++b) {
            f32x4 col[6], o[6];
#pragma unroll
            for (int pr = 0; pr < 6; ++pr) col[pr] = R[pr][b];
            bt6(col, o);
#pragma unroll
            for (int a = 0; a < 6; ++a)
                st_once(p.V + ((long long)((tile >> 4) * 36 + 6 * a + b) * 16 + (tile & 15)) * p.Cin + c4, o[a]);
        }
    } else {
        if (c4 >= p.Cout) return;
        f32x4 R[4][6];
#pragma unroll
        for (int u = 0; u < 4; ++u) {
            f32x4 y[4];
#pragma unroll
            for (int v = 0; v < 4; ++v)
                y[v] = *reinterpret_cast<const f32x4*>(p.dy + ((long long)(img * p.H + 4 * ty + u) * p.W + 4 * tx + v) * p.lddy + c4);
            a6(y, R[u]);
        }
#pragma unroll
        for (int b = 0; b < 6; ++b) {
            const f32x4 col[4] = {R[0][b], R[1][b], R[2][b], R[3][b]};
            f32x4 o[6];
            a6(col, o);
#pragma unroll
            for (int a = 0; a < 6; ++a)
                st_once(p.dM + ((long long)((tile >> 4) * 36 + 6 * a + b) * 16 + (tile & 15)) * p.Cout + c4, o[a]);
        }
    }
}

__global__ __launch_bounds__(256) void wino43_wgrad_finish_kernel(const float* dU, const float* cs, int Cout, int Cin, int Cout_w, int Cin_w,
                                                                  float* dw, float* dbias, int accumulate) {
    const long long idx = (long long)blockIdx.x * blockDim.x + threadIdx.x;
    if (dbias && idx < Cout_w) {
        const double pv[6] = {-1.0 / 9, 8.0 / 9, 0.0, 2.0 / 9, 0.0, -1.0 / 8};
// ... 139 lines not shown
               "vd_conv3x3_dgrad_wino43: unsupported geometry nimg=%d H=%d W=%d Cin=%d Cout=%d", nimg, H, W, Cin, Cout);
    VD_REQUIRE(vd_aligned16(dy) && vd_aligned16(U43) && vd_aligned16(dx), "vd_conv3x3_dgrad_wino43: operands must be 16-byte aligned");
    Args43 a = {};
    a.x = dy; a.ldx = lddy; a.U = U43; a.y = dx; a.ldy = lddx;
    a.nimg = nimg; a.H = H; a.W = W; a.K = Cout; a.N = Cin;
    a.items_per_img = W == 64 ? H / 16 : 1;
    a.ngrp = W == 16 ? nimg / 4 : nimg * a.items_per_img;
    a.ncb = Cin / TN;
    const long long items = (long long)a.ngrp * a.ncb;
    VD_REQUIRE(items < (1LL << 30), "vd_conv3x3_dgrad_wino43: too many work items");
    a.nitems = (int)items;
    a.probe = g_probe43;
    const int ncu = vd_persistent_cus();
    const dim3 grid((unsigned)(items < ncu ? items : ncu)), blk(THREADS);
    hipStream_t st = (hipStream_t)stream;
    if (W == 16) hipLaunchKernelGGL((wino43_conv_kernel<4, false>), grid, blk, 0, st, a);
    else if (W == 32) hipLaunchKernelGGL((wino43_conv_kernel<8, false>), grid, blk, 0, st, a);
    else hipLaunchKernelGGL((wino43_conv_kernel<16, false>), grid, blk, 0, st, a);
    VD_LAUNCH_CHECK("wino43_conv_kernel<., false>");
    g_last43 = W / 4;
    return 0;
}

extern "C" int vd_wino43_last_kernel(void) { return g_last43; }
#ifdef VD_PROBES
extern "C" int vd_wino43_set_probe(unsigned long long* buf) { g_probe43 = buf; return 0; }
#endif

extern "C" int vd_wino43_pack(const float* w_oihw, int32_t Cout, int32_t Cin, float* U43, void* stream) {
    VD_REQUIRE(w_oihw && U43 && Cout % KT == 0 && Cin % TN == 0, "vd_wino43_pack: needs Cout %% 8 == 0 and Cin %% 32 == 0");
    hipLaunchKernelGGL(wino43_pack_kernel, dim3((unsigned)((Cin / TN) * (Cout / KT))), dim3(256), 0, (hipStream_t)stream, w_oihw, U43, Cout, Cin, 0);
    VD_LAUNCH_CHECK("wino43_pack_kernel");
    return 0;
}

extern "C" int vd_conv3x3_wino43_fwd_supported(int32_t nimg, int32_t H, int32_t W, int32_t Cin, int32_t Cout, int64_t ldx, int64_t ldy,
                                               int64_t ldres) {
    if (nimg <= 0 || Cin % KT || Cout % TN || ldx % 4 || ldy % 4 || ldres % 4) return 0;
    if (!((W == 32 && H == 32) || (W == 64 && H % 16 == 0 && H >= 16) || (W == 16 && H == 16 && nimg % 4 == 0))) return 0;
    const long long px = (W == 16 ? (long long)nimg : 1LL) * H * W, lim = 0x7FFFFFF0LL / 4;
    if (px * ldx >= lim || px * ldy >= lim || (ldres > 0 && px * ldres >= lim)) return 0;
    return 1;
}

extern "C" int vd_wino43_pack_fwd(const float* w_oihw, int32_t Cout, int32_t Cin, float* U43f, void* stream) {
    VD_REQUIRE(w_oihw && U43f && Cin % KT == 0 && Cout % TN == 0, "vd_wino43_pack_fwd: needs Cin %% 8 == 0 and Cout %% 32 == 0");
    hipLaunchKernelGGL(wino43_pack_kernel, dim3((unsigned)((Cout / TN) * (Cin / KT))), dim3(256), 0, (hipStream_t)stream, w_oihw, U43f, Cout, Cin, 1);
    VD_LAUNCH_CHECK("wino43_pack_kernel(fwd)");
    return 0;
}

extern "C" int vd_conv3x3_wino43_fwd_chunk_rows(int32_t H, int32_t W) { return W == 16 ? H * W : (W == 32 ? H * W : 16 * W); }

extern "C" int vd_conv3x3_wino43_fwd(const float* xin, int64_t ldx, const float* U43f, const float* bias, const float* res, int64_t ldres,
                                     float* y, int64_t ldy, int32_t nimg, int32_t H, int32_t W, int32_t Cin, int32_t Cout,
                                     float* stats_part, void* stream) {
    VD_REQUIRE(xin && U43f && y, "vd_conv3x3_wino43_fwd: null operand");
    VD_REQUIRE(vd_conv3x3_wino43_fwd_supported(nimg, H, W, Cin, Cout, ldx, ldy, res ? ldres : 0),
               "vd_conv3x3_wino43_fwd: unsupported geometry nimg=%d H=%d W=%d Cin=%d Cout=%d", nimg, H, W, Cin, Cout);
    VD_REQUIRE(vd_aligned16(xin) && vd_aligned16(U43f) && vd_aligned16(y) && (!res || vd_aligned16(res)) && (!bias || vd_aligned16(bias)),
               "vd_conv3x3_wino43_fwd: operands must be 16-byte aligned");
    Args43 a = {};
    a.x = xin; a.ldx = ldx; a.U = U43f; a.y = y; a.ldy = ldy;
    a.nimg = nimg; a.H = H; a.W = W; a.K = Cin; a.N = Cout;
    a.items_per_img = W == 64 ? H / 16 : 1;
    a.ngrp = W == 16 ? nimg / 4 : nimg * a.items_per_img;
    a.ncb = Cout / TN;
    a.bias = bias; a.res = res; a.ldr = ldres; a.stats = stats_part;
    a.chunks_per_img = (H * W) / vd_conv3x3_wino43_fwd_chunk_rows(H, W);
    VD_REQUIRE(a.chunks_per_img == a.items_per_img, "vd_conv3x3_wino43_fwd: statistics chunks (%d per image) do not match the work items (%d)", a.chunks_per_img, a.items_per_img);
    const long long items = (long long)a.ngrp * a.ncb;
    VD_REQUIRE(items < (1LL << 30), "vd_conv3x3_wino43_fwd: too many work items");
    a.nitems = (int)items;
    a.probe = g_probe43;
    const int ncu = vd_persistent_cus();
    const dim3 grid((unsigned)(items < ncu ? items : ncu)), blk(THREADS);
    hipStream_t st = (hipStream_t)stream;
    if (W == 16) hipLaunchKernelGGL((wino43_conv_kernel<4, true>), grid, blk, 0, st, a);
    else if (W == 32) hipLaunchKernelGGL((wino43_conv_kernel<8, true>), grid, blk, 0, st, a);
    else hipLaunchKernelGGL((wino43_conv_kernel<16, true>), grid, blk, 0, st, a);
    VD_LAUNCH_CHECK("wino43_conv_kernel<., true>");
    g_last43 = -(W / 4);
    return 0;
}

extern "C" int vd_wino43_pack_batched(const int64_t* items_dev, int32_t n, int64_t total_blocks, void* stream) {
    VD_REQUIRE(items_dev && n > 0 && total_blocks > 0 && total_blocks < (1LL << 31), "vd_wino43_pack_batched: bad table");
    hipLaunchKernelGGL(wino43_pack_batched_kernel, dim3((unsigned)total_blocks), dim3(256), 0, (hipStream_t)stream,
                       reinterpret_cast<const long long*>(items_dev), n);
    VD_LAUNCH_CHECK("wino43_pack_batched_kernel");
    return 0;
}

extern "C" int vd_conv3x3_wgrad_wino43_supported(int32_t nimg, int32_t H, int32_t W, int32_t Cin, int32_t Cout, int64_t ldx, int64_t lddy) {
    const Wg43Plan g = wg43_plan(nimg, H, W, Cin, Cout);
    if (!g.ok || ldx % 4 || lddy % 4 || g.T < 512 || g.T % 4) return 0;
    const long long px = (long long)nimg * H * W, lim = 0x7FFFFFF0LL / 4;
    if (px * ldx >= lim || px * lddy >= lim) return 0;
    if ((long long)g.T * (Cin > Cout ? Cin : Cout) * 4 >= (1LL << 40)) return 0;
    return 1;
}

extern "C" size_t vd_conv3x3_wgrad_wino43_ws_bytes(int32_t nimg, int32_t H, int32_t W, int32_t Cin, int32_t Cout) {
    const Wg43Plan g = wg43_plan(nimg, H, W, Cin, Cout);
    if (!g.ok) return 0;
    return (g.v_f + g.m_f + g.u_f + g.cs_f) * sizeof(float) + g.gemm_bytes;
}

static int wgrad43_impl(const float* xin, int64_t ldx, const float* dy, int64_t lddy, int32_t nimg, int32_t H, int32_t W, int32_t Cin,
                        int32_t Cout, float* dw_oihw, float* dbias, int32_t Cin_w, int32_t Cout_w, int32_t accumulate, float* ws,
                        size_t ws_bytes, void* stream, int phases) {
    VD_REQUIRE(xin && dy && dw_oihw && ws, "vd_conv3x3_wgrad_wino43: null operand");
    VD_REQUIRE(vd_conv3x3_wgrad_wino43_supported(nimg, H, W, Cin, Cout, ldx, lddy),
               "vd_conv3x3_wgrad_wino43: unsupported geometry nimg=%d H=%d W=%d Cin=%d Cout=%d", nimg, H, W, Cin, Cout);
    VD_REQUIRE(Cin_w <= Cin && Cout_w <= Cout, "vd_conv3x3_wgrad_wino43: real dims exceed padded dims");
    VD_REQUIRE(vd_aligned16(xin) && vd_aligned16(dy) && vd_aligned16(ws), "vd_conv3x3_wgrad_wino43: operands must be 16-byte aligned");
    VD_REQUIRE(ws_bytes >= vd_conv3x3_wgrad_wino43_ws_bytes(nimg, H, W, Cin, Cout), "vd_conv3x3_wgrad_wino43: workspace too small");
    const Wg43Plan g = wg43_plan(nimg, H, W, Cin, Cout);
    float* V = ws;
    float* dM = V + g.v_f;
    float* dU = dM + g.m_f;
    float* cs = dU + g.u_f;
    float* gws = cs + g.cs_f;
    hipStream_t st = (hipStream_t)stream;
    if (phases & 1) {
        WgT43 t = {};
        t.x = xin; t.ldx = ldx; t.dy = dy; t.lddy = lddy; t.V = V; t.dM = dM;
        t.nimg = nimg; t.H = H; t.W = W; t.Cin = Cin; t.Cout = Cout; t.TW = W / 4; t.TPI = (H / 4) * (W / 4); t.T = g.T;
        const int cmax = Cin > Cout ? Cin : Cout;
        hipLaunchKernelGGL(wino43_wgrad_transform_kernel, dim3((unsigned)(g.T / 4), (unsigned)((cmax + 255) / 256), 2), dim3(64, 4), 0, st, t);
        VD_LAUNCH_CHECK("wino43_wgrad_transform_kernel");
    }
    if (phases & 2) {
        const float* A[36]; const float* B[36]; float* C[36]; float* colsum[36];
        for (int e = 0; e < 36; ++e) {
            A[e] = dM + (size_t)e * 16 * Cout; B[e] = V + (size_t)e * 16 * Cin;
            C[e] = dU + (size_t)e * Cout * Cin; colsum[e] = cs + (size_t)e * Cout;
        }
        const int rc = vd_gemm_grouped_wgrad_kblk(A, B, C, colsum, 36, Cout, Cin, g.T, Cout, Cin, Cin, g.S, gws, g.gemm_bytes, stream,
                                                  36LL * 16 * Cout, 36LL * 16 * Cin,
                                                  (long long)Cout * Cin >= FUSED_FINISH_MIN ? 1 : 0);
        if (rc) return rc;
        g_last43w = g.S;
    }
    if (phases & 4) {
        const long long tot = (long long)Cout * Cin;
        if (tot >= FUSED_FINISH_MIN) {
            const int used = vd_gemm_grouped_wgrad_used_slabs(36, Cout, Cin, g.T, g.S);
            hipLaunchKernelGGL(wino43_wgrad_reduce_finish_kernel, dim3((unsigned)((tot + 63) / 64)), dim3(64, 6), 0, st, gws,
                               gws + (size_t)36 * used * Cout * Cin, used, Cout, Cin, Cout_w, Cin_w, dw_oihw, dbias, accumulate);
        } else {
            hipLaunchKernelGGL(wino43_wgrad_finish_kernel, dim3((unsigned)((tot + 255) / 256)), dim3(256), 0, st, dU, cs, Cout, Cin, Cout_w, Cin_w,
                               dw_oihw, dbias, accumulate);
        }
        VD_LAUNCH_CHECK("wino43_wgrad_finish_kernel");
    }
    return 0;
}

extern "C" int vd_conv3x3_wgrad_wino43(const float* xin, int64_t ldx, const float* dy, int64_t lddy, int32_t nimg, int32_t H, int32_t W,
                                       int32_t Cin, int32_t Cout, float* dw_oihw, float* dbias, int32_t Cin_w, int32_t Cout_w,
                                       int32_t accumulate, float* ws, size_t ws_bytes, void* stream) {
    return wgrad43_impl(xin, ldx, dy, lddy, nimg, H, W, Cin, Cout, dw_oihw, dbias, Cin_w, Cout_w, accumulate, ws, ws_bytes, stream, 7);
}

extern "C" int vd_conv3x3_wgrad_wino43_phase(const float* xin, int64_t ldx, const float* dy, int64_t lddy, int32_t nimg, int32_t H,
                                             int32_t W, int32_t Cin, int32_t Cout, float* dw_oihw, float* dbias, int32_t Cin_w,
                                             int32_t Cout_w, int32_t accumulate, float* ws, size_t ws_bytes, int32_t phase, void* stream) {
    VD_REQUIRE(phase == 1 || phase == 2 || phase == 4, "vd_conv3x3_wgrad_wino43_phase: phase must be 1 (transforms), 2 (GEMMs) or 4 (reduction + finish)");
    return wgrad43_impl(xin, ldx, dy, lddy, nimg, H, W, Cin, Cout, dw_oihw, dbias, Cin_w, Cout_w, accumulate, ws, ws_bytes, stream, phase);
}

extern "C" int vd_wino43_wgrad_last_kernel(void) { return g_last43w; }
```

### v-diffusion-torch_amd/v_diffusion/_hip.py

```python
import ctypes as C
import os

import torch

_HERE = os.path.dirname(os.path.abspath(__file__))
LIB_PATH = os.environ.get("VDIFF_HIP_LIB") or os.path.join(os.path.dirname(_HERE), "lib", "libvdiff_hip.so")

ROW, COL, IM2COL = 0, 1, 2
RS_NONE, RS_DOWN, RS_UP = 0, 1, 2
OUT_TYPES = {"v": 0, "x0": 1, "eps": 2, "both": 3}
REWEIGHTS = {"constant": 0, "snr": 1, "snr_trunc": 2, "snr_1plus": 3}

_i32, _i64, _f32, _f64, _u64, _vp, _sz = C.c_int32, C.c_int64, C.c_float, C.c_double, C.c_uint64, C.c_void_p, C.c_size_t


class GemmDesc(C.Structure):
    _fields_ = [("A", _vp), ("B", _vp), ("C", _vp), ("bias", _vp), ("R", _vp),
                ("M", _i32), ("N", _i32), ("K", _i32), ("a_kind", _i32), ("b_kind", _i32),
                ("lda", _i64), ("ldb", _i64), ("ldc", _i64), ("ldr", _i64),
                ("batch", _i32), ("nh", _i32),
                ("sAb", _i64), ("sAh", _i64), ("sBb", _i64), ("sBh", _i64),
                ("sCb", _i64), ("sCh", _i64), ("sRb", _i64), ("sRh", _i64),
                ("alpha", _f32), ("accumulate", _i32), ("H", _i32), ("W", _i32), ("Cin", _i32),
                ("splitk", _i32), ("ws", _vp), ("ws_bytes", _i64), ("tile", _i32),
                ("colsum", _vp), ("colsum_accumulate", _i32), ("stats", _vp), ("stats_hw", _i32), ("sBias", _i64)]


_SIGNATURES = {
    "vd_version": (C.c_int, []),
    "vd_last_error": (C.c_char_p, []),
    "vd_set_reserved_cus": (C.c_int, [_i32]),
    "vd_reserved_cus": (C.c_int, []),
    "vd_mfma_calibrate": (C.c_int, [_vp, _vp, _i32, _i32, C.c_uint32, _vp]),
    "vd_gemm": (C.c_int, [C.POINTER(GemmDesc), _vp]),
    "vd_gemm_last_tile": (C.c_int, []),
    "vd_gemm_split_forms": (C.c_int, []),
    "vd_gemm_grouped_wgrad_ws_bytes": (_sz, [_i32, _i32, _i32, _i32]),
    "vd_gemm_grouped_wgrad_auto_split": (C.c_int, [_i32, _i32, _i32, _i32, _i32, _i32]),
    "vd_gemm_grouped_wgrad": (C.c_int, [_vp, _vp, _vp, _vp, _i32, _i32, _i32, _i32, _i64, _i64, _i64, _i32, _vp, _sz, _vp]),
    "vd_conv3x3": (C.c_int, [_vp, _i64, _vp, _vp, _vp, _i64, _vp, _i64, _i32, _i32, _i32, _i32, _i32, _i32, _vp, _vp]),
    "vd_conv3x3_wino_supported": (C.c_int, [_i32, _i32, _i32, _i32, _i32, _i64, _i64, _i64]),
    "vd_conv3x3_wino": (C.c_int, [_vp, _i64, _vp, _vp, _vp, _i64, _vp, _i64, _i32, _i32, _i32, _i32, _i32, _vp, _vp]),
    "vd_wino_pack": (C.c_int, [_vp, _i32, _i32, _vp, _vp, _vp]),
    "vd_conv3x3_wgrad_wino_supported": (C.c_int, [_i32, _i32, _i32, _i32, _i32, _i64, _i64]),
    "vd_conv3x3_wgrad_wino_ws_bytes": (_sz, [_i32, _i32, _i32, _i32, _i32]),
    "vd_conv3x3_wgrad_wino": (C.c_int, [_vp, _i64, _vp, _i64, _i32, _i32, _i32, _i32, _i32, _vp, _vp, _i32, _i32, _i32, _vp, _sz, _vp]),
    "vd_conv3x3_wgrad_wino_phase": (C.c_int, [_vp, _i64, _vp, _i64, _i32, _i32, _i32, _i32, _i32, _vp, _vp, _i32, _i32, _i32, _vp, _sz, _i32, _vp]),
    "vd_wino_last_kernel": (C.c_int, []),
    "vd_wino_wgrad_last_kernel": (C.c_int, []),
    "vd_wino_pack_batched": (C.c_int, [_vp, _i32, _i64, _vp]),
    "vd_conv3x3_dgrad_wino43_supported": (C.c_int, [_i32, _i32, _i32, _i32, _i32, _i64, _i64]),
    "vd_wino43_u_floats": (_sz, [_i32, _i32]),
    "vd_conv3x3_dgrad_wino43": (C.c_int, [_vp, _i64, _vp, _vp, _i64, _i32, _i32, _i32, _i32, _i32, _vp]),
    "vd_wino43_last_kernel": (C.c_int, []),
    "vd_conv3x3_wino43_fwd_supported": (C.c_int, [_i32, _i32, _i32, _i32, _i32, _i64, _i64, _i64]),
    "vd_conv3x3_wino43_preferred": (C.c_int, [_i32, _i32, _i32, _i32]),
    "vd_wino43_pack_fwd": (C.c_int, [_vp, _i32, _i32, _vp, _vp]),
    "vd_conv3x3_wino43_fwd_chunk_rows": (C.c_int, [_i32, _i32]),
    "vd_conv3x3_wino43_fwd": (C.c_int, [_vp, _i64, _vp, _vp, _vp, _i64, _vp, _i64, _i32, _i32, _i32, _i32, _i32, _vp, _vp]),
    "vd_wino43_pack": (C.c_int, [_vp, _i32, _i32, _vp, _vp]),
    "vd_wino43_pack_batched": (C.c_int, [_vp, _i32, _i64, _vp]),
    "vd_conv3x3_wgrad_wino43_supported": (C.c_int, [_i32, _i32, _i32, _i32, _i32, _i64, _i64]),
    "vd_conv3x3_wgrad_wino43_ws_bytes": (_sz, [_i32, _i32, _i32, _i32, _i32]),
    "vd_conv3x3_wgrad_wino43": (C.c_int, [_vp, _i64, _vp, _i64, _i32, _i32, _i32, _i32, _i32, _vp, _vp, _i32, _i32, _i32, _vp, _sz, _vp]),
    "vd_wino43_wgrad_last_kernel": (C.c_int, []),
    "vd_conv3x3_wgrad_wino43_phase": (C.c_int, [_vp, _i64, _vp, _i64, _i32, _i32, _i32, _i32, _i32, _vp, _vp, _i32, _i32, _i32, _vp, _sz, _i32, _vp]),
    "vd_gn_stats_from_partials": (C.c_int, [_vp, _i32, _i32, _vp, _i32, _i32, _i32, _i32, _i32, _f32, _vp, _vp]),
    "vd_gn_coef_from_partials": (C.c_int, [_vp, _i32, _i32, _vp, _i32, _i32, _i32, _i32, _i32, _f32, _vp, _vp, _vp, _vp, _vp]),
    "vd_conv3x3_wgrad_ws_bytes": (_sz, [_i32, _i32, _i32, _i32, _i32]),
    "vd_conv3x3_wgrad": (C.c_int, [_vp, _i64, _vp, _i64, _i32, _i32, _i32, _i32, _i32, _vp, _vp, _i32, _i32, _i32, _vp, _sz, _vp]),
    "vd_conv3x3_wgrad_phase": (C.c_int, [_vp, _i64, _vp, _i64, _i32, _i32, _i32, _i32, _i32, _vp, _vp, _i32, _i32, _i32, _vp, _sz, _i32, _vp]),
    "vd_pack_conv3x3": (C.c_int, [_vp, _i32, _i32, _vp, _i32, _vp, _i32, _vp]),
    "vd_pack_conv3x3_batched": (C.c_int, [_vp, _i32, _i64, _vp]),
    "vd_gn_ws_bytes": (_sz, [_i32, _i32, _i32]),
    "vd_gn_stats": (C.c_int, [_vp, _i64, _i32, _i32, _i32, _i32, _f32, _vp, _vp, _sz, _vp]),
    "vd_gn_apply": (C.c_int, [_vp, _i64, _vp, _vp, _vp, _vp, _i32, _f32, _u64, _i32, _vp, _i64, _i32, _i32, _i32, _i32, _i32, _vp, _vp]),
    "vd_gn_apply_from_partials": (C.c_int, [_vp, _i64, _vp, _i32, _i32, _vp, _i32, _i32, _vp, _vp, _vp, _i32, _f32, _u64, _i32, _vp, _i64, _i32,
                                            _i32, _i32, _i32, _i32, _f32, _vp, _vp]),
    "vd_gn_apply_bwd": (C.c_int, [_vp, _i64, _vp, _i64, _vp, _vp, _vp, _vp, _i32, _f32, _u64, _i32, _vp, _i64, _vp, _i64, _i32,
                                  _vp, _vp, _vp, _i32, _i32, _i32, _i32, _i32, _i32, _vp, _sz, _vp]),
    "vd_gn_bwd_last_kernel": (C.c_int, []),
    "vd_gn_apply_bwd_keep": (C.c_int, [_vp, _i64, _vp, _i64, _vp, _vp, _vp, _vp, _i32, _f32, _u64, _i32, _vp, _i64, _vp, _i64, _i32,
                                       _vp, _vp, _i32, _i32, _i32, _i32, _i32, _vp, _sz, _vp]),
    "vd_gn_param_sums_batched": (C.c_int, [_vp, _i32, _i64, _vp]),
    "vd_colsum_ws_bytes": (_sz, [_i64, _i32]),
    "vd_colsum": (C.c_int, [_vp, _i64, _i64, _i32, _vp, _i32, _vp, _sz, _vp]),
    "vd_axpby": (C.c_int, [_vp, _i64, _f32, _vp, _i64, _f32, _i64, _i32, _vp]),
    "vd_silu": (C.c_int, [_vp, _vp, _i64, _vp]),
    "vd_silu_bwd": (C.c_int, [_vp, _vp, _vp, _i64, _i32, _vp]),
    "vd_softmax_rows": (C.c_int, [_vp, _i64, _i32, _vp]),
    "vd_softmax_rows_bwd": (C.c_int, [_vp, _vp, _i64, _i32, _f32, _vp]),
    "vd_attn_supported": (C.c_int, [_i32, _i32, _i32]),
    "vd_attn_fwd": (C.c_int, [_vp, _vp, _vp, _i64, _vp, _i64, _vp, _i32, _i32, _i32, _i32, _f32, _vp]),
    "vd_attn_bwd": (C.c_int, [_vp, _vp, _vp, _i64, _vp, _i64, _vp, _i64, _vp, _vp, _vp, _vp, _vp, _i64, _i32, _i32, _i32, _i32, _f32, _vp]),
    "vd_attn_bwd_phase": (C.c_int, [_vp, _vp, _vp, _i64, _vp, _i64, _vp, _i64, _vp, _vp, _vp, _vp, _vp, _i64, _i32, _i32, _i32, _i32, _f32,
                                    _i32, _vp]),
    "vd_nchw_to_nhwc": (C.c_int, [_vp, _vp, _i32, _i32, _i32, _i32, _i64, _vp]),
    "vd_nhwc_to_nchw": (C.c_int, [_vp, _i64, _vp, _i32, _i32, _i32, _i32, _vp]),
    "vd_images_to_uint8_hwc": (C.c_int, [_vp, _vp, _i32, _i32, _i32, _vp]),
    "vd_images_from_uint8_hwc": (C.c_int, [_vp, _vp, _vp, _i32, _i32, _i32, _i32, _vp]),
    "vd_timestep_embedding": (C.c_int, [_vp, _vp, _i32, _i32, _f64, _vp]),
    "vd_class_embed": (C.c_int, [_vp, _vp, _vp, _vp, _i32, _i32, _i32, _vp]),
    "vd_class_embed_bwd": (C.c_int, [_vp, _vp, _vp, _vp, _i32, _i32, _i32, _i32, _vp]),
    "vd_multitag_norm": (C.c_int, [_vp, _vp, _i32, _i32, _vp]),
    "vd_im2col3x3": (C.c_int, [_vp, _i64, _vp, _i32, _i32, _i32, _i32, _vp]),
    "vd_tap_gather": (C.c_int, [_vp, _i64, _vp, _vp, _i64, _i32, _i32, _i32, _i32, _vp]),
    "vd_tap_spread": (C.c_int, [_vp, _i64, _vp, _i64, _i32, _i32, _i32, _i32, _vp]),
    "vd_thin_wgrad_finish": (C.c_int, [_vp, _i32, _i32, _i32, _vp, _i32, _vp, _i32, _i32, _vp, _vp]),
    "vd_q_sample": (C.c_int, [_vp, _vp, _vp, _vp, _i32, _i32, _i32, _vp]),
    "vd_loss_fwd": (C.c_int, [_vp, _vp, _vp, _vp, _vp, _i32, _i32, _vp, _vp, _i32, _i32, _i32, _vp]),
    "vd_loss_bwd": (C.c_int, [_vp, _vp, _vp, _vp, _vp, _vp, _vp, _i32, _i32, _vp, _i32, _i32, _i32, _vp]),
    "vd_bpd_terms": (C.c_int, [_vp, _vp, _vp, _vp, _i32, _i32, _vp, _vp, _vp, _vp, _i32, _i32, _i32, _vp]),
    "vd_bpd_bwd": (C.c_int, [_vp, _vp, _vp, _vp, _vp, _vp, _i32, _i32, _vp, _i32, _i32, _i32, _vp]),
    "vd_sample_step": (C.c_int, [_vp, _vp, _vp, C.POINTER(_f32), _vp, _i32, _i32, _i32, _i32, _vp, _vp, _i32, _i32, _i32, _vp]),
    "vd_sumsq_ws_bytes": (_sz, [_i64]),
    "vd_sumsq": (C.c_int, [_vp, _i64, _vp, _vp, _sz, _vp]),
    "vd_adamw_ema": (C.c_int, [_vp, _vp, _vp, _vp, _vp, _i64, _vp, _f32, _f32, _f32, _f32, _f32, _f32, _f32, _f32, _f32, _i64, _i64, _i32,
                               _f32, _f32, _vp]),
    "vd_adamw_ema_flagged": (C.c_int, [_vp, _vp, _vp, _vp, _vp, _i64, _vp, _f32, _f32, _f32, _f32, _f32, _f32, _f32, _f32, _f32, _i64, _i64,
# ... 235 lines not shown
        _check(lib().vd_mfma_calibrate(sink.data_ptr(), stamps.data_ptr(), blocks, iters, 12345, stream()), "vd_mfma_calibrate")
        e1.record()
        torch.cuda.synchronize()
        ms = e0.elapsed_time(e1)
        if time.perf_counter() >= t_end:
            break
    st = stamps.view(blocks, 2).double().cpu()
    mhz = float((st[:, 0] / st[:, 1].clamp(min=1)).median()) * 100.0
    tflops = blocks * 8 * iters * 16 * 2048.0 / (ms * 1e-3) / 1e12
    return mhz, tflops


WINO43 = os.environ.get("VD_WINO43", "1") != "0"
WINO43_MIN_W = int(os.environ.get("VD_WINO43_MIN_W", "16"))


WINO43_OCC = os.environ.get("VD_WINO43_OCC", "1") != "0"


def wino43_preferred(nimg, H, W, N):
    return not WINO43_OCC or bool(lib().vd_conv3x3_wino43_preferred(nimg, H, W, N))


def wino43_supported(nimg, H, W, Cin, Cout, lddy, lddx):
    return (WINO and WINO43 and W >= WINO43_MIN_W and bool(lib().vd_conv3x3_dgrad_wino43_supported(nimg, H, W, Cin, Cout, lddy, lddx))
            and wino43_preferred(nimg, H, W, Cin))


def wino43_pack(w, Cout, Cin, U43):
    _check(lib().vd_wino43_pack(ptr(w), Cout, Cin, ptr(U43), stream()), "vd_wino43_pack")


def wino43_pack_batched(table, n, total_blocks):
    assert table.is_cuda and table.dtype == torch.int64 and table.is_contiguous()
    _check(lib().vd_wino43_pack_batched(table.data_ptr(), n, total_blocks, stream()), "vd_wino43_pack_batched")


WINO43_FWD = os.environ.get("VD_WINO43_FWD", "1") != "0"


def wino43_fwd_supported(nimg, H, W, Cin, Cout, ldx, ldy, ldres=0):
    return (WINO and WINO43_FWD and bool(lib().vd_conv3x3_wino43_fwd_supported(nimg, H, W, Cin, Cout, ldx, ldy, ldres))
            and wino43_preferred(nimg, H, W, Cout))


def wino43_pack_fwd(w, Cout, Cin, U43f):
    _check(lib().vd_wino43_pack_fwd(ptr(w), Cout, Cin, ptr(U43f), stream()), "vd_wino43_pack_fwd")


def wino43_fwd_chunk_rows(H, W):
    return int(lib().vd_conv3x3_wino43_fwd_chunk_rows(H, W))


def conv3x3_wino43_fwd(x, ldx, U43f, bias, y, ldy, nimg, H, W, Cin, Cout, res=None, ldres=0, stats_part=None):
    name = f"wino43_conv_kernel<{W // 4}, true>"
    with _TimedName(name, 2.0 * nimg * H * W * Cout * 9 * Cin):
        _check(lib().vd_conv3x3_wino43_fwd(ptr(x), ldx, ptr(U43f), ptr(bias), ptr(res), ldres, ptr(y), ldy, nimg, H, W, Cin, Cout,
                                           ptr(stats_part), stream()), "vd_conv3x3_wino43_fwd")
    _note_bytes(name, 4.0 * (nimg * H * W * (Cin + Cout + (Cout if res is not None else 0)) + 36 * Cout * Cin))


def conv3x3_dgrad_wino43(dy, lddy, U43, dx, lddx, nimg, H, W, Cin, Cout):
    with _TimedName(f"wino43_conv_kernel<{W // 4}, false>", 2.0 * nimg * H * W * Cout * 9 * Cin):
        _check(lib().vd_conv3x3_dgrad_wino43(ptr(dy), lddy, ptr(U43), ptr(dx), lddx, nimg, H, W, Cin, Cout, stream()),
               "vd_conv3x3_dgrad_wino43")
    _note_bytes(f"wino43_conv_kernel<{W // 4}, false>", 4.0 * (nimg * H * W * (Cin + Cout) + 36 * Cout * Cin))


def conv3x3(x, ldx, wpack, bias, y, ldy, nimg, H, W, Cin, Cout, res=None, ldres=0, accumulate=False, stats_part=None):
    with _TimedTile("gemm_dma_kernel<{tile}, 2, 0, false, {kt}>", 2.0 * nimg * H * W * Cout * 9 * Cin):
        _check(lib().vd_conv3x3(ptr(x), ldx, ptr(wpack), ptr(bias), ptr(res), ldres, ptr(y), ldy, nimg, H, W, Cin, Cout,
                                int(accumulate), ptr(stats_part), stream()), "vd_conv3x3")


def conv3x3_wgrad_wino(x, ldx, dy, lddy, nimg, H, W, Cin, Cout, dw, Cin_w, Cout_w, accumulate=False, dbias=None):
    nb = lib().vd_conv3x3_wgrad_wino_ws_bytes(nimg, H, W, Cin, Cout)
    ws = workspace(nb, x.device, "wgrad")
    args = _wgrad_args(x, ldx, dy, lddy, nimg, H, W, Cin, Cout, dw, dbias, Cin_w, Cout_w, accumulate, ws)
    if PROFILE is None:
        _check(lib().vd_conv3x3_wgrad_wino(*args, stream()), "vd_conv3x3_wgrad_wino")
        return
    tws = min(W // 2, 16)
    with _TimedName(f"wino_wgrad_kernel<{tws}, {'true' if dbias is not None else 'false'}>", 2.0 * nimg * H * W * Cout * 9 * Cin):
        _check(lib().vd_conv3x3_wgrad_wino_phase(*args, 1, stream()), "vd_conv3x3_wgrad_wino_phase")
    with _TimedName("wino_wgrad_reduce_kernel", 0.0):
        _check(lib().vd_conv3x3_wgrad_wino_phase(*args, 2, stream()), "vd_conv3x3_wgrad_wino_phase")


WGRAD_STREAM = os.environ.get("VD_WGRAD_STREAM", "1") != "0"
GROUPED_AUTO_SPLIT = os.environ.get("VD_GROUPED_AUTO_SPLIT", "1") != "0"
GN_FOLD = os.environ.get("VD_GN_FOLD", "1") != "0"
GN_FOLD_MAX_CHUNKS = int(os.environ.get("VD_GN_FOLD_MAX_CHUNKS", "8"))
READY_PER_BLOCK = os.environ.get("VD_READY_PER_BLOCK", "0") != "0"
AUTOGRAD_CHAIN = os.environ.get("VD_AUTOGRAD_CHAIN", "1") != "0"
WINO43_WGRAD = os.environ.get("VD_WINO43_WGRAD", "1") != "0"
WINO43_WGRAD_MIN_TILES = int(os.environ.get("VD_WINO43_WGRAD_MIN_TILES", "512"))


W43_WGRAD_TAG = "[36 planes of the F(4x4,3x3) weight gradient]"


def wgrad43_supported(nimg, H, W, Cin, Cout, ldx, lddy):
    return (WINO and WINO43_WGRAD and nimg * (H // 4) * (W // 4) >= WINO43_WGRAD_MIN_TILES
            and bool(lib().vd_conv3x3_wgrad_wino43_supported(nimg, H, W, Cin, Cout, ldx, lddy)))


def conv3x3_wgrad_wino43(x, ldx, dy, lddy, nimg, H, W, Cin, Cout, dw, Cin_w, Cout_w, accumulate=False, dbias=None):
    nb = lib().vd_conv3x3_wgrad_wino43_ws_bytes(nimg, H, W, Cin, Cout)
    ws = workspace(nb, x.device, "wgrad43")
    args = _wgrad_args(x, ldx, dy, lddy, nimg, H, W, Cin, Cout, dw, dbias, Cin_w, Cout_w, accumulate, ws)
    if PROFILE is None:
        _check(lib().vd_conv3x3_wgrad_wino43(*args, stream()), "vd_conv3x3_wgrad_wino43")
        return
    with _TimedBytes("wino43_wgrad_transform_kernel", 4.0 * nimg * H * W * (Cin + Cout) * (1 + 2.25)):
        _check(lib().vd_conv3x3_wgrad_wino43_phase(*args, 1, stream()), "vd_conv3x3_wgrad_wino43_phase")
    with _TimedTile("gemm_dma_kernel<{tile}, 1, 1, true, {kt}, true> " + W43_WGRAD_TAG, 2.0 * nimg * H * W * Cout * 9 * Cin) as t:
        _check(lib().vd_conv3x3_wgrad_wino43_phase(*args, 2, stream()), "vd_conv3x3_wgrad_wino43_phase")
    _note_bytes(PROFILE[-1][0], 4.0 * (36.0 * nimg * (H // 4) * (W // 4) * (Cin + Cout) + 36.0 * Cout * Cin))
    with _TimedName("wino43_wgrad_finish_kernel", 0.0):
        _check(lib().vd_conv3x3_wgrad_wino43_phase(*args, 4, stream()), "vd_conv3x3_wgrad_wino43_phase")


def conv3x3_wgrad(x, ldx, dy, lddy, nimg, H, W, Cin, Cout, dw, Cin_w, Cout_w, accumulate=False, dbias=None, direct=False):
    if not direct and wgrad43_supported(nimg, H, W, Cin, Cout, ldx, lddy):
        return conv3x3_wgrad_wino43(x, ldx, dy, lddy, nimg, H, W, Cin, Cout, dw, Cin_w, Cout_w, accumulate, dbias)
    if WINO and not direct and lib().vd_conv3x3_wgrad_wino_supported(nimg, H, W, Cin, Cout, ldx, lddy):
        return conv3x3_wgrad_wino(x, ldx, dy, lddy, nimg, H, W, Cin, Cout, dw, Cin_w, Cout_w, accumulate, dbias)
    nb = lib().vd_conv3x3_wgrad_ws_bytes(nimg, H, W, Cin, Cout)
    ws = workspace(nb, x.device, "wgrad")
    args = _wgrad_args(x, ldx, dy, lddy, nimg, H, W, Cin, Cout, dw, dbias, Cin_w, Cout_w, accumulate, ws)
    flops = 2.0 * nimg * H * W * Cout * 9 * Cin
    if PROFILE is None:
        _check(lib().vd_conv3x3_wgrad(*args, stream()), "vd_conv3x3_wgrad")
        return
    with _TimedTile("gemm_dma_kernel<{tile}, 1, 2, true, {kt}>", flops):
        _check(lib().vd_conv3x3_wgrad_phase(*args, 1, stream()), "vd_conv3x3_wgrad_phase")
    with _TimedTile("reduce_slabs_oihw_kernel", 0.0):
        _check(lib().vd_conv3x3_wgrad_phase(*args, 2, stream()), "vd_conv3x3_wgrad_phase")


def im2col3x3(x, ldx, xc, nimg, H, W, Cc):
    _check(lib().vd_im2col3x3(ptr(x), ldx, ptr(xc), nimg, H, W, Cc, stream()), "vd_im2col3x3")


def tap_gather(z, ldz, bias, out, ldo, nimg, H, W, Cout):
    _check(lib().vd_tap_gather(ptr(z), ldz, ptr(bias), ptr(out), ldo, nimg, H, W, Cout, stream()), "vd_tap_gather")


def tap_spread(dy, lddy, dz, ldz, nimg, H, W, Cout):
    _check(lib().vd_tap_spread(ptr(dy), lddy, ptr(dz), ldz, nimg, H, W, Cout, stream()), "vd_tap_spread")


def thin_wgrad_finish(g, Cout_w, Cin, Cin_w, dw, accumulate=False, colsum=None, cs_stride=1, cs_off=0, dbias=None):
    _check(lib().vd_thin_wgrad_finish(ptr(g), Cout_w, Cin, Cin_w, ptr(dw), int(accumulate), ptr(colsum), cs_stride, cs_off,
                                      ptr(dbias), stream()), "vd_thin_wgrad_finish")


def pack_conv3x3(w, Cout_w, Cin_w, wf=None, Cin_p=0, wd=None, Cout_p=0):
    _check(lib().vd_pack_conv3x3(ptr(w), Cout_w, Cin_w, ptr(wf), Cin_p, ptr(wd), Cout_p, stream()), "vd_pack_conv3x3")


def pack_conv3x3_batched(table, n, total_blocks):
    assert table.is_cuda and table.dtype == torch.int64 and table.is_contiguous()
    _check(lib().vd_pack_conv3x3_batched(table.data_ptr(), n, total_blocks, stream()), "vd_pack_conv3x3_batched")


def gn_stats(x, ldx, nimg, HW, Cc, stats, G=32, eps=1e-6):
    nb = lib().vd_gn_ws_bytes(nimg, HW, Cc)
    ws = workspace(nb, x.device, "gn")
    _check(lib().vd_gn_stats(ptr(x), ldx, nimg, HW, Cc, G, eps, ptr(stats), ws.data_ptr(), ws.numel() * 4, stream()),
           "vd_gn_stats")


def _gn_bwd_name():
    k = lib().vd_gn_bwd_last_kernel()
    if k > 0:
# ... 290 lines not shown
```

### v-diffusion-torch_amd/v_diffusion/engine.py

```python
import math

import torch

from . import _hip as H

GROUPS = 32
EPS = 1e-6
THIN = 8


def _ld(t):
    return t.stride(2)


def _chk(t):
    B, Hh, Ww, C = t.shape
    ld = t.stride(2)
    assert t.stride(3) == 1 and t.stride(1) == Ww * ld and t.stride(0) == Hh * Ww * ld, "not an NHWC view"
    return B, Hh, Ww, C, ld


def _splitk(M, N, K):
    tiles = ((M + 63) // 64) * ((N + 63) // 64)
    s = max(1, min(64, 1024 // max(tiles, 1), K // 256))
# ... 73 lines not shown
        self.levels = levels
        self.film_groups, self.film_slot = {}, {}
        for b in plan:
            if b.res is not None:
                pre = b.prefix + (".0" if b.att is not None else "")
                grp = self.film_groups.setdefault(2 * b.cout, [])
                self.film_slot[pre] = (2 * b.cout, len(grp))
                grp.append(b.res)
        self.pack_cache = None
        self._pack_state = None
        self._last_pack_state = None
        self._packed = None
        self._norm_channels = sum(p.numel() for k, p in model.named_parameters()
                                  if k.endswith(".weight") and p.ndim == 1)
        self._pgb_arena = self._pgb_table = None
        self._side = self._side_stream = None
        self._wq = None
        self._active_run = None
        self._segments = None

    @staticmethod
    def _new(ref, *shape):
        return torch.empty(shape, dtype=torch.float32, device=ref.device)

    def _res_of(self, level, H0, W0):
        return H0 >> level, W0 >> level

    def _part(self, ref, nimg, HW, C):
        if HW % 32:
            return None
        return torch.empty(H.stats_part_numel(nimg, HW, C), dtype=torch.float32, device=ref.device)

    @staticmethod
    def _parts(part, C, HW, rows=None):
        if part is None:
            return None
        return [(part, C, HW // (rows or (H.last_row_tile() // 2)))]

    def _norm(self, x, x_parts, gn, film, act, p_drop, seed, rs, y, B, Hh, Ww, C):
        coef = self._new(x, B, 4, C)
        stats = None
        if x_parts is not None and H.GN_FOLD and max(k for _, _, k in x_parts) <= H.GN_FOLD_MAX_CHUNKS:
            H.gn_apply_from_partials(x, _ld(x), x_parts, gn.weight, gn.bias, film, act, p_drop, seed, rs, y, _ld(y), B, Hh, Ww, C, coef,
                                     GROUPS, EPS)
            return coef
        if x_parts is not None:
            H.gn_coef_from_partials(x_parts, B, Hh * Ww, gn.weight, gn.bias, film, coef, GROUPS, EPS)
        else:
            stats = self._new(x, B, GROUPS, 2)
            H.gn_stats(x, _ld(x), B, Hh * Ww, C, stats, GROUPS, EPS)
        H.gn_apply(x, _ld(x), stats, gn.weight, gn.bias, film, act, p_drop, seed, rs, y, _ld(y), B, Hh, Ww, C, coef, GROUPS)
        return coef

    def _wgrad(self, dy, x, dw, db, M, N, K, lda, ldb, ldc):
        if self._wq is None or not H.GROUPED_WGRAD:
            H.gemm(dy, x, dw, M, N, K, a_kind=H.COL, b_kind=H.COL, lda=lda, ldb=ldb, ldc=ldc, splitk=_splitk(M, N, K), colsum=db)
            return
        key = (M, N, K, lda, ldb, ldc, db is not None)
        q = self._wq.setdefault(key, [])
        q.append((dy, x, dw, db))
        if len(q) == H.GROUP_MAX:
            self._wgrad_flush_key(key)

    def _cwgrad(self, x, ldx, dy, lddy, *args, **kw):
        side = self._side
        if side is None:
            return H.conv3x3_wgrad(x, ldx, dy, lddy, *args, **kw)
        side.wait_stream(torch.cuda.current_stream())
        x.record_stream(side)
        dy.record_stream(side)
        with torch.cuda.stream(side):
            H.conv3x3_wgrad(x, ldx, dy, lddy, *args, **kw)

    def _side_join(self):
        if self._side is not None:
            torch.cuda.current_stream().wait_stream(self._side)

    def _wgrad_flush_key(self, key):
        q = self._wq.pop(key, None)
        if not q:
            return
        M, N, K, lda, ldb, ldc, _ = key
        ok = M % 4 == 0 and N % 4 == 0 and lda % 4 == 0 and ldb % 4 == 0 and max(lda, ldb, ldc) * 128 + 128 < 0x70000000 // 4 and \
            all(dy.data_ptr() % 16 == 0 and x.data_ptr() % 16 == 0 for dy, x, _, _ in q)
        if len(q) == 1 or not ok:
            for dy, x, dw, db in q:
                H.gemm(dy, x, dw, M, N, K, a_kind=H.COL, b_kind=H.COL, lda=lda, ldb=ldb, ldc=ldc, splitk=_splitk(M, N, K), colsum=db)
            return
        if H.GROUPED_AUTO_SPLIT:
            S = H.lib().vd_gemm_grouped_wgrad_auto_split(len(q), M, N, K, 1, 64)
        else:
            tiles = ((M + 63) // 64) * ((N + 63) // 64) * len(q)
            S = max(1, min(64, 1024 // max(tiles, 1), K // 256))
        H.gemm_grouped_wgrad(q, M, N, K, lda, ldb, ldc, S)

    def _wgrad_flush(self):
        if not self._wq:
            return
        side = self._side
        if side is None:
            for key in list(self._wq):
                self._wgrad_flush_key(key)
            return
        side.wait_stream(torch.cuda.current_stream())
        for q in self._wq.values():
            for dy, x, _, _ in q:
                dy.record_stream(side)
                x.record_stream(side)
        with torch.cuda.stream(side):
            for key in list(self._wq):
                self._wgrad_flush_key(key)

    def _pgb_begin(self, ref, B):
        need = B * 2 * self._norm_channels
        if self._pgb_arena is None or self._pgb_arena.numel() < need or self._pgb_arena.device != ref.device:
            self._pgb_arena = torch.empty(need, dtype=torch.float32, device=ref.device)
            self._pgb_table = None
        self._pgb_rows, self._pgb_off, self._pgb_blk = [], 0, 0

    def _pgb(self, B, C, dgamma, dbeta):
        sl = self._pgb_arena[self._pgb_off: self._pgb_off + B * 2 * C]
        self._pgb_rows.append([sl.data_ptr(), dgamma.data_ptr(), dbeta.data_ptr(), B, C, 0, 0, self._pgb_blk])
        self._pgb_off += B * 2 * C
        self._pgb_blk += (C + 15) // 16
        return sl
# ... 223 lines not shown
        dte = torch.empty_like(dta)
        H.silu_bwd(te, dta, dte)
        if yn is not None:
            if m.multitags:
                self._linear_bwd(yn, m.class_embed.weight, dte, G["class_embed.weight"], G["class_embed.bias"], None)
            else:
                H.class_embed_bwd(yn, dte, G["class_embed.1.weight"], G["class_embed.1.bias"], B, m.embedding_dim, m.num_classes)
        elif m.num_classes:
            for k in G:
                if k.startswith("class_embed."):
                    G[k].zero_()
        l0, l2 = m.time_embed[0], m.time_embed[2]
        da0 = torch.empty_like(dte)
        self._linear_bwd(a0, l2.weight, dte, G["time_embed.2.weight"], G["time_embed.2.bias"], da0)
        dh0 = torch.empty_like(da0)
        H.silu_bwd(h0, da0, dh0)
        self._linear_bwd(te0, l0.weight, dh0, G["time_embed.0.weight"], G["time_embed.0.bias"], None)

    def _film_fwd(self, ta, tape):
        B, E = ta.shape
        films, stacks = {}, {}
        cache = self.pack_cache
        for c2, mods in self.film_groups.items():
            key = ("film", c2)
            if cache is not None and key in cache:
                W, bv = cache[key]
            else:
                W = torch.stack([mm.fc.weight.detach() for mm in mods])
                bv = torch.stack([mm.fc.bias.detach() for mm in mods])
                if cache is not None:
                    cache[key] = (W, bv)
            nb = len(mods)
            out = self._new(ta, nb, B, c2)
            H.gemm(ta, W, out, B, c2, E, a_kind=H.ROW, b_kind=H.ROW, lda=E, ldb=E, ldc=c2, bias=bv, sBias=c2, batch=nb,
                   sA=(0, 0), sB=(c2 * E, 0), sC=(B * c2, 0))
            films[c2], stacks[c2] = out, W
        if tape is not None:
            tape["film_w"] = stacks
        return films

    def _film_bwd(self, dfilms, stacks, dta):
        B, E = dta.shape
        for c2, df in dfilms.items():
            nb, W = df.shape[0], stacks[c2]
            P = self._new(dta, nb, B * E)
            H.gemm(df, W, P, B, E, c2, a_kind=H.ROW, b_kind=H.COL, lda=c2, ldb=E, ldc=E, batch=nb, sA=(B * c2, 0), sB=(c2 * E, 0),
                   sC=(B * E, 0))
            H.colsum(P, B * E, nb, B * E, dta.view(-1), accumulate=True)

    def _res_fwd(self, blk, mod, prefix, x, films, dest, p_drop, seed, tape, x_parts=None):
        B, Hh, Ww, Cin, ldx = _chk(x)
        Cout, rs = blk.cout, blk.rs
        Ho, Wo = (Hh // 2, Ww // 2) if rs == H.RS_DOWN else ((Hh * 2, Ww * 2) if rs == H.RS_UP else (Hh, Ww))
        a1 = self._new(x, B, Ho, Wo, Cin)
        coef1 = self._norm(x, x_parts, mod.norm1, None, 1, 0.0, 0, rs, a1, B, Hh, Ww, Cin)
        h1 = self._new(x, B, Ho, Wo, Cout)
        ph = self._part(x, B, Ho * Wo, Cout)
        rows = self._conv(a1, Cin, mod.conv1.weight, mod.conv1.bias, h1, Cout, B, Ho, Wo, Cin, Cout, stats_part=ph)
        h1_parts = self._parts(ph, Cout, Ho * Wo, rows)
        c2, fi = self.film_slot[prefix]
        film = films[c2][fi]
        a2 = self._new(x, B, Ho, Wo, Cout)
        coef2 = self._norm(h1, h1_parts, mod.norm2, film, 1, p_drop, seed, H.RS_NONE, a2, B, Ho, Wo, Cout)
        if rs != H.RS_NONE:
            xs = self._new(x, B, Ho, Wo, Cin)
            H.gn_apply(x, ldx, None, None, None, None, 0, 0.0, 0, rs, xs, Cin, B, Hh, Ww, Cin, None, GROUPS)
        else:
            xs = x
        has_skip = Cin != Cout
        if has_skip:
            sk = self._new(x, B, Ho, Wo, Cout)
            w = mod.skip.weight
            H.gemm(xs, w, sk, B * Ho * Wo, Cout, Cin, a_kind=H.ROW, b_kind=H.ROW, lda=_ld(xs), ldb=Cin, ldc=Cout, bias=mod.skip.bias)
        else:
            sk = xs
        pd = self._part(x, B, Ho * Wo, Cout)
        rows = self._conv(a2, Cout, mod.conv2.weight, mod.conv2.bias, dest, _ld(dest), B, Ho, Wo, Cout, Cout, res=sk,
                          ldres=_ld(sk), stats_part=pd)
        out_parts = self._parts(pd, Cout, Ho * Wo, rows)
        if tape is not None:
            tape[prefix] = dict(x=x, coef1=coef1, a1=a1, h1=h1, coef2=coef2, a2=a2, film=film, xs=xs if has_skip else None,
                                seed=seed, p=p_drop)
        return out_parts

    def _res_bwd(self, blk, mod, prefix, ctx, dy, dx, dx_accumulate, ta, dfilms, G):
        x, a1, h1, a2, film = ctx["x"], ctx["a1"], ctx["h1"], ctx["a2"], ctx["film"]
        B, Hh, Ww, Cin, ldx = _chk(x)
        _, Ho, Wo, Cout, lddy = _chk(dy)
        rs = blk.rs
        self._cwgrad(a2, Cout, dy, lddy, B, Ho, Wo, Cout, Cout, G[prefix + ".conv2.weight"], Cout, Cout,
                        dbias=G[prefix + ".conv2.bias"])
        da2 = self._new(x, B, Ho, Wo, Cout)
        self._conv(dy, lddy, mod.conv2.weight, None, da2, Cout, B, Ho, Wo, Cout, Cout, dgrad=True)
        dh1 = self._new(x, B, Ho, Wo, Cout)
        c2, fi = self.film_slot[prefix]
        dfilm = dfilms[c2][fi]
        H.gn_apply_bwd(da2, Cout, h1, Cout, ctx["coef2"], mod.norm2.weight, mod.norm2.bias, film, 1, ctx["p"], ctx["seed"],
                       H.RS_NONE, None, 0, dh1, Cout, False, dfilm, None, None, False, B, Ho, Wo, Cout, GROUPS,
                       pgb_keep=self._pgb(B, Cout, G[prefix + ".norm2.weight"], G[prefix + ".norm2.bias"]))
        del da2
        self._cwgrad(a1, Cin, dh1, Cout, B, Ho, Wo, Cin, Cout, G[prefix + ".conv1.weight"], Cin, Cout,
                        dbias=G[prefix + ".conv1.bias"])
        da1 = self._new(x, B, Ho, Wo, Cin)
        self._conv(dh1, Cout, mod.conv1.weight, None, da1, Cin, B, Ho, Wo, Cout, Cin, dgrad=True)
        del dh1
        if Cin != Cout:
            xs = ctx["xs"]
            P = B * Ho * Wo
            w = mod.skip.weight
            self._wgrad(dy, xs, G[prefix + ".skip.weight"], G[prefix + ".skip.bias"], Cout, Cin, P, lddy, _ld(xs), Cin)
            dsk = self._new(x, B, Ho, Wo, Cin)
            H.gemm(dy, w, dsk, P, Cin, Cout, a_kind=H.ROW, b_kind=H.COL, lda=lddy, ldb=Cin, ldc=Cin)
        else:
            dsk = dy
        if rs != H.RS_NONE:
            addt = self._new(x, B, Hh, Ww, Cin)
            H.gn_apply_bwd(dsk, _ld(dsk), None, 0, None, None, None, None, 0, 0.0, 0, rs, None, 0, addt, Cin, False, None, None,
                           None, False, B, Hh, Ww, Cin, GROUPS)
        else:
            addt = dsk
        H.gn_apply_bwd(da1, Cin, x, ldx, ctx["coef1"], mod.norm1.weight, mod.norm1.bias, None, 1, 0.0, 0, rs, addt, _ld(addt),
                       dx, _ld(dx), dx_accumulate, None, None, None, False, B, Hh, Ww, Cin, GROUPS,
                       pgb_keep=self._pgb(B, Cin, G[prefix + ".norm1.weight"], G[prefix + ".norm1.bias"]))
        self._linear_bwd(ta, mod.fc.weight, dfilm, G[prefix + ".fc.weight"], G[prefix + ".fc.bias"], None)

    def _attn_fwd(self, mod, prefix, x, dest, tape, x_parts=None):
        B, Hh, Ww, C, ldx = _chk(x)
        L, nh, hd = Hh * Ww, mod.num_heads, mod.head_dim
        hid = nh * hd
        xn = self._new(x, B, Hh, Ww, C)
        coef = self._norm(x, x_parts, mod.norm, None, 0, 0.0, 0, H.RS_NONE, xn, B, Hh, Ww, C)
        qkv = self._new(x, B, L, 3 * hid)
        H.gemm(xn, mod.proj_in.weight, qkv, B * L, 3 * hid, C, a_kind=H.ROW, b_kind=H.ROW, lda=C, ldb=C, ldc=3 * hid,
               bias=mod.proj_in.bias)
        ld = 3 * hid
        alpha = 1.0 / math.sqrt(hd)
        q, k, v = qkv[0, 0, 0:], qkv[0, 0, hid:], qkv[0, 0, 2 * hid:]
        O = self._new(x, B, L, hid)
        S = lse = None
        if B * nh <= 65535 and H.attn_use_fused(L, hd, B * nh, tape is not None):
            if tape is not None:
                lse = self._new(x, B * nh * L)
            H.attn_fwd(q, k, v, ld, O, hid, lse, B, nh, L, hd, alpha)
        else:
            S = self._new(x, B, nh, L, L)
            H.gemm(q, k, S, L, L, hd, a_kind=H.ROW, b_kind=H.ROW, lda=ld, ldb=ld, ldc=L, batch=B * nh, nh=nh, sA=(L * ld, hd),
                   sB=(L * ld, hd), sC=(nh * L * L, L * L), alpha=alpha)
            H.softmax_rows(S, B * nh * L, L)
            H.gemm(S, v, O, L, hd, L, a_kind=H.ROW, b_kind=H.COL, lda=L, ldb=ld, ldc=hid, batch=B * nh, nh=nh, sA=(nh * L * L, L * L),
                   sB=(L * ld, hd), sC=(L * hid, hd))
        pd = self._part(x, B, L, C)
        if pd is not None and L % 64:
            pd = None
        H.gemm(O, mod.proj_out.weight, dest, B * L, C, hid, a_kind=H.ROW, b_kind=H.ROW, lda=hid, ldb=hid, ldc=_ld(dest),
               bias=mod.proj_out.bias, R=x, ldr=ldx, stats=pd, stats_hw=L)
# ... 331 lines not shown
```

Measured before the change: 2210.

## Fuse GroupNorm apply with Winograd input transform and reuse V in wgrad

Adds a GroupNorm-apply kernel that writes the Winograd F(4,3) input-transformed tiles (V) directly instead of the normalized activation. The forward conv and the weight-gradient GEMM then consume V through new entry points. For wgrad this uses a K-tile-major channel-grouped B layout in the grouped GEMM. The aim is to drop the activation write/read round trip and the separate input transforms in both forward and backward. In exchange it stores the 2.25x-larger V tensor on the tape for backward, which raises memory traffic and footprint.

```diff
diff --git a/include/vdiff_hip.h b/include/vdiff_hip.h
--- a/include/vdiff_hip.h
+++ b/include/vdiff_hip.h
@@ -99,6 +99,13 @@
                                   int32_t Cin, int32_t Cout, float* dw_oihw, float* dbias, int32_t Cin_w, int32_t Cout_w,
                                   int32_t accumulate, float* ws, size_t ws_bytes, int32_t phase, void* stream);
 int vd_wino43_wgrad_last_kernel(void);
+size_t vd_wino43_v_floats(int32_t nimg, int32_t H, int32_t W, int32_t Cin);
+int vd_conv3x3_wino43_fwd_v_supported(int32_t nimg, int32_t H, int32_t W, int32_t Cin, int32_t Cout, int64_t ldy, int64_t ldres);
+int vd_conv3x3_wino43_fwd_v(const float* V, const float* U43f, const float* bias, const float* res, int64_t ldres, float* y, int64_t ldy,
+                            int32_t nimg, int32_t H, int32_t W, int32_t Cin, int32_t Cout, float* stats_part, void* stream);
+int vd_conv3x3_wgrad_wino43_v(const float* V, const float* dy, int64_t lddy, int32_t nimg, int32_t H, int32_t W, int32_t Cin, int32_t Cout,
+                              float* dw_oihw, float* dbias, int32_t Cin_w, int32_t Cout_w, int32_t accumulate, float* ws, size_t ws_bytes,
+                              int32_t phase, void* stream);
 
 int vd_wino_pack_batched(const int64_t* items_dev, int32_t n, int64_t total_blocks, void* stream);
 
@@ -144,6 +151,11 @@
                               int32_t chunks2, const float* gamma, const float* beta, const float* film, int32_t act, float p_drop,
                               uint64_t seed, int32_t resample, float* y, int64_t ldy, int32_t nimg, int32_t H, int32_t W, int32_t C,
                               int32_t G, float eps, float* coef, void* stream);
+int vd_gn_apply_from_partials_v_supported(int32_t nimg, int32_t H, int32_t W, int32_t C, int32_t G, int64_t ldx);
+int vd_gn_apply_from_partials_v(const float* x, int64_t ldx, const float* part1, int32_t C1, int32_t chunks1, const float* part2, int32_t C2,
+                                int32_t chunks2, const float* gamma, const float* beta, const float* film, int32_t act, float p_drop,
+                                uint64_t seed, float* V, int32_t nimg, int32_t H, int32_t W, int32_t C, int32_t G, float eps, float* coef,
+                                void* stream);
 
 int vd_gn_apply_bwd(const float* dy, int64_t lddy, const float* x, int64_t ldx, const float* coef,
                     const float* gamma, const float* beta, const float* film, int32_t act, float p_drop, uint64_t seed,
diff --git a/v-diffusion-torch_amd/csrc/common.h b/v-diffusion-torch_amd/csrc/common.h
--- a/v-diffusion-torch_amd/csrc/common.h
+++ b/v-diffusion-torch_amd/csrc/common.h
@@ -20,7 +20,7 @@
 int vd_persistent_cus(void);
 int vd_gemm_grouped_wgrad_kblk(const float* const* A, const float* const* B, float* const* C, float* const* colsum, int32_t count, int32_t M,
                                int32_t N, int32_t K, int64_t lda, int64_t ldb, int64_t ldc, int32_t splitk, float* ws, size_t ws_bytes,
-                               void* stream, int64_t a_kblk, int64_t b_kblk, int32_t slabs_only);
+                               void* stream, int64_t a_kblk, int64_t b_kblk, int32_t slabs_only, int64_t b_cgrp);
 int vd_gemm_grouped_wgrad_used_slabs(int32_t count, int32_t M, int32_t N, int32_t K, int32_t splitk);
 extern thread_local int vd_g_last_tile;
 inline int vd_tile_code(bool tr, bool spl, int kt, int bm, int bn) {
@@ -59,3 +59,14 @@
     for (int j = 0; j < 4; ++j) m[j] = ((r[j] >> 8) * (1.0f / 16777216.0f) >= p) ? inv : 0.0f;
     return m;
 }
+
+__device__ __forceinline__ void vd_wino43_bt6(const f32x4 (&d)[6], f32x4 (&o)[6]) {
+    const f32x4 e1 = d[4] - 2.25f * d[2], f1 = 0.75f * d[3] - 1.6875f * d[1];
+    const f32x4 e2 = d[4] - 0.5625f * d[2], f2 = 1.5f * d[3] - 0.84375f * d[1];
+    o[0] = 1.265625f * d[0] + (d[4] - 2.8125f * d[2]);
+    o[1] = e1 + f1;
+    o[2] = e1 - f1;
+    o[3] = e2 + f2;
+    o[4] = e2 - f2;
+    o[5] = 1.265625f * d[1] + (d[5] - 2.8125f * d[3]);
+}
diff --git a/v-diffusion-torch_amd/csrc/gemm.hip b/v-diffusion-torch_amd/csrc/gemm.hip
--- a/v-diffusion-torch_amd/csrc/gemm.hip
+++ b/v-diffusion-torch_amd/csrc/gemm.hip
@@ -27,6 +27,7 @@
     int group_S;
     int lgW, lgHW;
     long long a_kblk, b_kblk;
+    long long b_cgrp;
 };
 
 __device__ __forceinline__ int PB(const GemmArgs& p) { return VD_PROBE_BUILD ? p.probe : 0; }
@@ -471,13 +472,14 @@
             kcB[j] = kk;
             const bool ok = (BK == VD_IM2COL) ? (ci0 + cn < p.Cin) : (n0 + cn < p.N);
             const int rowoff = (GROUPED && BK == VD_COL && p.b_kblk) ? (kk >> 4) * (int)p.b_kblk + (kk & 15) * (int)p.ldb : kk * (int)p.ldb;
-            voB[j] = ok ? (unsigned)(rowoff + cn) * 4u : OOB;
+            const int coloff = (GROUPED && BK == VD_COL && p.b_cgrp) ? (cn >> 3) * (int)p.b_cgrp + (cn & 7) : cn;
+            voB[j] = ok ? (unsigned)(rowoff + coloff) * 4u : OOB;
             if (BK == VD_IM2COL) pix_yx(p, kt_begin * KT + kk, by[j], bx[j]);
             else by[j] = bx[j] = 0;
         }
     }
     const float* Ablk = (AK == VD_COL) ? A + m0 : A + (long long)m0 * p.lda;
-    const float* Bblk = (BK == VD_ROW) ? B + (long long)n0 * p.ldb : ((BK == VD_COL) ? B + n0 : B + ci0);
+    const float* Bblk = (BK == VD_ROW) ? B + (long long)n0 * p.ldb : ((BK == VD_COL) ? B + ((GROUPED && p.b_cgrp) ? (long long)(n0 >> 3) * p.b_cgrp : (long long)n0) : B + ci0);
     const long long tapoffB = (BK == VD_IM2COL) ? (long long)((tapN / 3 - 1) * p.W + (tapN % 3 - 1)) * p.ldb : 0;
 
 #ifndef VD_ISSUE_IN
@@ -943,7 +945,8 @@
     const int m0 = tby * BM, n0 = tbx * BN;
     const int e = tbz / p.group_S, slab = tbz - e * p.group_S;
     const float* A = gp.A[e] + m0;
-    const float* B = gp.B[e] + n0;
+    const float* B = gp.B[e] + (p.b_cgrp ? (long long)(n0 >> 3) * p.b_cgrp : (long long)n0);
+    const int boffB = p.b_cgrp ? ((lane >> 1) * (int)p.b_cgrp + (lane & 1) * 4) * 4 : lane * 16;
     const int kt_begin = slab * p.kt_per_split, kt_end = min(kt_begin + p.kt_per_split, p.kt_total);
     float* C = p.C + (long long)tbz * p.slab_stride;
 
@@ -957,7 +960,7 @@
         for (int h = 0; h < 2; ++h) {
             const int kk = wave + 8 * h;
             __builtin_amdgcn_raw_ptr_buffer_load_lds(rsA, (lds_ptr_t)(as + kk * BM), 16, lane * 16, kk * (int)p.lda * 4, 0, 0);
-            __builtin_amdgcn_raw_ptr_buffer_load_lds(rsB, (lds_ptr_t)(bs + kk * BN), 16, lane * 16, kk * (int)p.ldb * 4, 0, 0);
+            __builtin_amdgcn_raw_ptr_buffer_load_lds(rsB, (lds_ptr_t)(bs + kk * BN), 16, boffB, kk * (int)p.ldb * 4, 0, 0);
         }
     };
 
@@ -1424,7 +1427,7 @@
 extern "C" int vd_gemm_grouped_wgrad(const float* const* A, const float* const* B, float* const* C, float* const* colsum, int32_t count,
                                      int32_t M, int32_t N, int32_t K, int64_t lda, int64_t ldb, int64_t ldc, int32_t splitk, float* ws,
                                      size_t ws_bytes, void* stream) {
-    return vd_gemm_grouped_wgrad_kblk(A, B, C, colsum, count, M, N, K, lda, ldb, ldc, splitk, ws, ws_bytes, stream, 0, 0, 0);
+    return vd_gemm_grouped_wgrad_kblk(A, B, C, colsum, count, M, N, K, lda, ldb, ldc, splitk, ws, ws_bytes, stream, 0, 0, 0, 0);
 }
 
 int vd_gemm_grouped_wgrad_used_slabs(int32_t count, int32_t M, int32_t N, int32_t K, int32_t splitk) {
@@ -1433,7 +1436,7 @@
 
 int vd_gemm_grouped_wgrad_kblk(const float* const* A, const float* const* B, float* const* C, float* const* colsum, int32_t count,
                                int32_t M, int32_t N, int32_t K, int64_t lda, int64_t ldb, int64_t ldc, int32_t splitk, float* ws,
-                               size_t ws_bytes, void* stream, int64_t a_kblk, int64_t b_kblk, int32_t slabs_only) {
+                               size_t ws_bytes, void* stream, int64_t a_kblk, int64_t b_kblk, int32_t slabs_only, int64_t b_cgrp) {
     VD_REQUIRE(A && B && C && count > 0 && count <= VD_GROUP_MAX, "vd_gemm_grouped_wgrad: 1..%d entries (got %d)", VD_GROUP_MAX, count);
     VD_REQUIRE(M > 0 && N > 0 && K > 0 && M % 4 == 0 && N % 4 == 0 && lda % 4 == 0 && ldb % 4 == 0 && ldc >= N,
                "vd_gemm_grouped_wgrad: M, N, lda, ldb must be multiples of 4 (M=%d N=%d)", M, N);
@@ -1449,7 +1452,10 @@
     a.A = A[0]; a.B = B[0];
     a.M = M; a.N = N; a.K = K; a.lda = lda; a.ldb = ldb; a.ldc = N; a.ldr = 0; a.nh = 1;
     a.alpha = 1.f; a.lgW = a.lgHW = -1; a.probe = 0;
-    a.a_kblk = a_kblk; a.b_kblk = b_kblk;
+    a.a_kblk = a_kblk; a.b_kblk = b_kblk; a.b_cgrp = b_cgrp;
+    VD_REQUIRE(b_cgrp >= 0 && (b_cgrp == 0 || (b_kblk > 0 && ldb == 8 && N % 8 == 0 && b_cgrp % 4 == 0 && b_cgrp >= 128 &&
+                                               2 * b_kblk + (long long)(N / 8) * b_cgrp + 256 < 0x70000000LL / 4)),
+               "vd_gemm_grouped_wgrad: K-tile-major B operand needs K blocks, ldb = 8 and N %% 8 == 0");
     VD_REQUIRE(a_kblk >= 0 && b_kblk >= 0 && a_kblk % 4 == 0 && b_kblk % 4 == 0 && 2 * a_kblk + 16 * lda + 128 < 0x70000000LL / 4 &&
                2 * b_kblk + 16 * ldb + 128 < 0x70000000LL / 4, "vd_gemm_grouped_wgrad: K-block strides outside the LDS-DMA kernel's range");
     VD_REQUIRE(dma_in_range(a), "vd_gemm_grouped_wgrad: operands outside the LDS-DMA kernel's range (alignment / row pitch)");
diff --git a/v-diffusion-torch_amd/csrc/norm.hip b/v-diffusion-torch_amd/csrc/norm.hip
--- a/v-diffusion-torch_amd/csrc/norm.hip
+++ b/v-diffusion-torch_amd/csrc/norm.hip
@@ -210,6 +210,13 @@
     }
     float* o = coef + (long long)b * 4 * C + c;
     o[0] = sc; o[C] = of; o[2 * C] = rstd; o[3 * C] = -mean * rstd;
+}
+
+__device__ __forceinline__ void group_stat(double s1, double s2, double n, float eps, float& mean_o, float& rstd_o) {
+    const double mean = s1 / n;
+    double var = s2 / n - mean * mean;
+    if (var < 0.0) var = 0.0;
+    mean_o = (float)mean; rstd_o = (float)(1.0 / sqrt(var + (double)eps));
 }
 
 struct ApplyArgs {
@@ -267,11 +274,7 @@
         for (int g = threadIdx.x; g < ng; g += 256) {
             double s1 = 0.0, s2 = 0.0;
             for (int c = g * cg; c < (g + 1) * cg; ++c) { s1 += ps[0][c]; s2 += ps[1][c]; }
-            const double n = (double)cg * (double)p.H * (double)p.W;
-            const double mean = s1 / n;
-            double var = s2 / n - mean * mean;
-            if (var < 0.0) var = 0.0;
-            gst[0][g] = (float)mean; gst[1][g] = (float)(1.0 / sqrt(var + (double)q.eps));
+            group_stat(s1, s2, (double)cg * (double)p.H * (double)p.W, q.eps, gst[0][g], gst[1][g]);
         }
         __syncthreads();
         if (r >= rows) return;
@@ -332,6 +335,101 @@
             }
         }
         *reinterpret_cast<f32x4*>(yimg + (long long)po * p.ldy + c4) = out;
+    }
+}
+
+constexpr int VA_CB = 32, VA_PIX = 402;
+__global__ __launch_bounds__(256) void gn_apply_v_kernel(const ApplyArgs p, const PartArgs q, float* V, int TW) {
+    __shared__ f32x4 act[8 * VA_PIX];
+    __shared__ double ps[2][VA_CB + 64];
+    __shared__ float gst[2][VA_CB + 2];
+    const int tid = threadIdx.x, b = blockIdx.y, c0 = blockIdx.z * VA_CB;
+    const int C = p.C, cg = C / q.G;
+    const int g_lo = c0 / cg, g_hi = (min(c0 + VA_CB, C) - 1) / cg, cbeg = g_lo * cg, ncs = (g_hi + 1) * cg - cbeg;
+    for (int cl = tid; cl < ncs; cl += 256) {
+        const int c = cbeg + cl;
+        const bool first = c < q.C1;
+        const int Cs = first ? q.C1 : q.C2, cs = first ? c : c - q.C1, chunks = first ? q.ch1 : q.ch2;
+        const float* src = (first ? q.p1 : q.p2) + (long long)b * chunks * 2 * Cs + cs;
+        double s1 = 0.0, s2 = 0.0;
+        for (int ch = 0; ch < chunks; ++ch) { s1 += (double)src[(long long)ch * 2 * Cs]; s2 += (double)src[(long long)ch * 2 * Cs + Cs]; }
+        ps[0][cl] = s1; ps[1][cl] = s2;
+    }
+    __syncthreads();
+    for (int g = tid; g <= g_hi - g_lo; g += 256) {
+        double s1 = 0.0, s2 = 0.0;
+        for (int c = g * cg; c < (g + 1) * cg; ++c) { s1 += ps[0][c]; s2 += ps[1][c]; }
+        group_stat(s1, s2, (double)cg * (double)p.H * (double)p.W, q.eps, gst[0][g], gst[1][g]);
+    }
+    __syncthreads();
+    const int TWR = 16 / TW, RW = p.W + 2, RH = 4 * TWR + 2, npix = RH * RW;
+    const int row0 = 4 * TWR * (int)blockIdx.x - 1;
+    {
+        const int qd = tid & 7, c4 = c0 + 4 * qd;
+        const bool chan = c4 < C;
+        f32x4 sc = {1.f, 1.f, 1.f, 1.f}, of = {0.f, 0.f, 0.f, 0.f}, nr = sc, nm = of;
+        if (chan) {
+#pragma unroll
+            for (int j = 0; j < 4; ++j) {
+                const int c = c4 + j, g = c / cg - g_lo;
+                const float mean = gst[0][g], rstd = gst[1][g];
+                float s_ = rstd * q.gamma[c];
+                float o_ = q.beta[c] - mean * s_;
+                if (q.film) {
+                    const float shift = q.film[(long long)b * 2 * C + c], scale = q.film[(long long)b * 2 * C + C + c];
+                    s_ *= (1.f + scale);
+                    o_ = o_ * (1.f + scale) + shift;
+                }
+                sc[j] = s_; of[j] = o_; nr[j] = rstd; nm[j] = -mean * rstd;
+            }
+            if (blockIdx.x == 0 && tid < 8 && q.coef_out) {
+                float* o = q.coef_out + (long long)b * 4 * C + c4;
+                *reinterpret_cast<f32x4*>(o) = sc; *reinterpret_cast<f32x4*>(o + C) = of;
+                *reinterpret_cast<f32x4*>(o + 2 * C) = nr; *reinterpret_cast<f32x4*>(o + 3 * C) = nm;
+            }
+        }
+        const float* ximg = p.x + (long long)b * p.H * p.W * p.ldx;
+        for (int i0 = tid >> 3; i0 < npix; i0 += 4 * 32) {
+            f32x4 v[4];
+            int pix[4];
+#pragma unroll
+            for (int u = 0; u < 4; ++u) {
+                const int i = i0 + 32 * u;
+                const int ry = i / RW, yy = row0 + ry, xx = i - ry * RW - 1;
+                pix[u] = (chan && i < npix && (unsigned)yy < (unsigned)p.H && (unsigned)xx < (unsigned)p.W) ? yy * p.W + xx : -1;
+                if (pix[u] >= 0) v[u] = *reinterpret_cast<const f32x4*>(ximg + (long long)pix[u] * p.ldx + c4);
+            }
+#pragma unroll
+            for (int u = 0; u < 4; ++u) {
+                const int i = i0 + 32 * u;
+                if (i < npix) act[qd * VA_PIX + i] = pix[u] >= 0 ? fwd_val(p, v[u], pix[u], c4, sc, of, b) : f32x4{0.f, 0.f, 0.f, 0.f};
+            }
+        }
+    }
+    __syncthreads();
+    const int lane = tid & 63, wave = tid >> 6;
+    const int ti = (lane >> 1) & 15, h = lane >> 5, qd = 2 * wave + (lane & 1);
+    if (c0 + 8 * wave >= C) return;
+    const int tyl = ti / TW, tx = ti - tyl * TW;
+    const f32x4* a0 = act + qd * VA_PIX + (4 * tyl) * RW + 4 * tx;
+    f32x4 R[6][6];
+#pragma unroll
+    for (int pr = 0; pr < 6; ++pr) {
+        f32x4 d[6];
+#pragma unroll
+        for (int qq = 0; qq < 6; ++qq) d[qq] = a0[pr * RW + qq];
+        vd_wino43_bt6(d, R[pr]);
+    }
+    const long long tb = (long long)b * (p.H / 4) * (p.W / 4) / 16 + blockIdx.x;
+    float* vo = V + ((tb * (C / 8) + (c0 / 8 + wave)) * 36) * 128 + ti * 8 + (lane & 1) * 4;
+#pragma unroll
+    for (int bb = 0; bb < 3; ++bb) {
+        f32x4 col[6], o[6];
+#pragma unroll
+        for (int pr = 0; pr < 6; ++pr) col[pr] = h ? R[pr][bb + 3] : R[pr][bb];
+        vd_wino43_bt6(col, o);
+#pragma unroll
+        for (int a = 0; a < 6; ++a) *reinterpret_cast<f32x4*>(vo + (6 * a + bb + 3 * h) * 128) = o[a];
     }
 }
 
@@ -843,6 +941,29 @@
                "vd_gn_apply_from_partials: cannot split C=%d into whole-group channel ranges", C);
     hipLaunchKernelGGL(gn_apply_kernel<true>, dim3((unsigned)((Ho * Wo + APIX - 1) / APIX), nimg, C / Cba), dim3(256), 0, st, p, Cba, q);
     VD_LAUNCH_CHECK("gn_apply_kernel<from partials>");
+    return 0;
+}
+
+extern "C" int vd_gn_apply_from_partials_v_supported(int32_t nimg, int32_t H, int32_t W, int32_t C, int32_t G, int64_t ldx) {
+    if (nimg <= 0 || nimg > 65535 || G <= 0 || C % 8 || C % G || C / G > 32 || ldx % 4 || H % 4 || H < 4) return 0;
+    if (!(W == 16 || W == 32 || W == 64) || ((H / 4) * (W / 4)) % 16) return 0;
+    if (H * (long long)W * ldx >= 0x7FFFFFF0LL / 4) return 0;
+    return 1;
+}
+extern "C" int vd_gn_apply_from_partials_v(const float* x, int64_t ldx, const float* part1, int32_t C1, int32_t chunks1, const float* part2,
+                                           int32_t C2, int32_t chunks2, const float* gamma, const float* beta, const float* film, int32_t act,
+                                           float p_drop, uint64_t seed, float* V, int32_t nimg, int32_t H, int32_t W, int32_t C, int32_t G,
+                                           float eps, float* coef, void* stream) {
+    VD_REQUIRE(x && V && part1 && gamma && beta, "vd_gn_apply_from_partials_v: null operand");
+    VD_REQUIRE(C1 + C2 == C && C1 > 0 && chunks1 > 0 && (C2 == 0 || (part2 && chunks2 > 0)), "vd_gn_apply_from_partials_v: bad channel split C=%d C1=%d C2=%d", C, C1, C2);
+    VD_REQUIRE(vd_gn_apply_from_partials_v_supported(nimg, H, W, C, G, ldx), "vd_gn_apply_from_partials_v: unsupported geometry nimg=%d H=%d W=%d C=%d", nimg, H, W, C);
+    VD_REQUIRE(vd_aligned16(x) && vd_aligned16(V) && (!coef || vd_aligned16(coef)), "vd_gn_apply_from_partials_v: operands must be 16-byte aligned");
+    ApplyArgs p = {x, ldx, coef, 1, act, p_drop, seed, VD_RS_NONE, nullptr, 0, nimg, H, W, C};
+    PartArgs q = {part1, C1, chunks1, part2, C2, chunks2, G, eps, gamma, beta, film, coef};
+    const int TW = W / 4;
+    hipLaunchKernelGGL(gn_apply_v_kernel, dim3((unsigned)((H / 4) * TW / 16), nimg, (unsigned)((C + VA_CB - 1) / VA_CB)), dim3(256), 0,
+                       (hipStream_t)stream, p, q, V, TW);
+    VD_LAUNCH_CHECK("gn_apply_v_kernel");
     return 0;
 }
 
diff --git a/v-diffusion-torch_amd/csrc/wino43.hip b/v-diffusion-torch_amd/csrc/wino43.hip
--- a/v-diffusion-torch_amd/csrc/wino43.hip
+++ b/v-diffusion-torch_amd/csrc/wino43.hip
@@ -85,8 +85,9 @@
 template <bool DY>
 __device__ __forceinline__ void bt_full2(const f32x2 (&r)[6], f32x2 (&v)[6]) { bt_full<DY, f32x2>(r, v); }
 
-template <int TWT, bool FWD>
+template <int TWT, bool FWD, bool VIN = false>
 __global__ __launch_bounds__(THREADS) void wino43_conv_kernel(const Args43 p) {
+    static_assert(FWD || !VIN, "the input gradient has no V-input form");
     constexpr bool QUAD = TWT == 4;
     constexpr int RUN = TWT + 1;
     constexpr int RUNS = QUAD ? 4 * RUN - 2 : 4 * RUN;
@@ -95,13 +96,14 @@
     constexpr int RIN = QUAD ? 4 * 17 + 1 : 4 * NTR + 2;
     constexpr int NS = RIN * RP;
     constexpr int NPG = (NS + 63) / 64;
-    constexpr int A_STAGE = 2 * NPG * 256;
+    constexpr int A_STAGE = VIN ? 0 : 2 * NPG * 256;
     constexpr int STAGE = A_STAGE + U_STAGE;
     constexpr int LGT = TWT == 4 ? 2 : TWT == 8 ? 3 : 4;
     static_assert((4 * RP * 16) % 256 == (TWT * 16) % 256 || (QUAD && (4 * RP * 16) % 256 == 192), "row pitch leaves bank conflicts");
     static_assert(2 * STAGE * 4 <= 163840, "stages exceed the LDS");
-    static_assert(8 * 16 * 64 * 16 + 8 * 4 * 8 * 4 <= 2 * STAGE * 4, "epilogue exchange + statistics area exceeds the stages");
-    __shared__ __attribute__((aligned(1024))) float smem[2 * STAGE];
+    constexpr int XCH_F = 8 * 16 * 64 * 4 + 8 * 4 * 8;
+    static_assert(VIN || XCH_F <= 2 * STAGE, "epilogue exchange + statistics area exceeds the stages");
+    __shared__ __attribute__((aligned(1024))) float smem[2 * STAGE > XCH_F ? 2 * STAGE : XCH_F];
 
     const int tid = threadIdx.x, lane = tid & 63;
     const int wave = __builtin_amdgcn_readfirstlane(tid >> 6);
@@ -168,8 +170,8 @@
             }
         }
     };
-    constexpr int NPIECE = 5 + APL;
-    constexpr int SB = SB_STEP, NAFTER = 18 - SB, PAFTER = NAFTER;
+    constexpr int NPIECE = VIN ? 5 : 5 + APL;
+    constexpr int SB = SB_STEP, NAFTER = 18 - SB, PAFTER = VIN ? NPIECE : NAFTER;
     constexpr int UPF = U_AHEAD;
     static_assert(PAFTER <= NPIECE && NPIECE - PAFTER <= SB, "DMA schedule does not fit the tile");
 
@@ -210,13 +212,14 @@
             }
         };
         auto first_stage = [&](int cbx, int grpx) {
-            if (QUAD) xitem = p.x + (long long)grpx * (4 * 16 * 16) * p.ldx;
+            if (VIN) {}
+            else if (QUAD) xitem = p.x + (long long)grpx * (4 * 16 * 16) * p.ldx;
             else { offsets(grpx); xitem = p.x + (long long)(grpx / p.items_per_img) * p.H * p.W * p.ldx; }
 #pragma unroll
             for (int i = 0; i < NPIECE; ++i) issue_piece(i, 0, 0, cbx);
         };
         int cb = 0, grp = 0, cb_next = 0, grp_next = 0;
-        if (QUAD) offsets(0);
+        if (QUAD && !VIN) offsets(0);
         bool have = item_of(0, cb, grp);
         if (have) first_stage(cb, grp);
         for (int n = 0; have; ++n) {
@@ -226,7 +229,18 @@
             f32x4 acc[18][2];
 #pragma unroll
             for (int x = 0; x < 18; ++x) { acc[x][0] = f32x4{0.f, 0.f, 0.f, 0.f}; acc[x][1] = f32x4{0.f, 0.f, 0.f, 0.f}; }
-            if (n == 0) asm volatile("s_waitcnt vmcnt(0)" ::: "memory");
+            f32x2 Vg[VIN ? 18 : 1];
+            const float* vitem = p.x + (long long)(4 * grp + tg) * nkt * (36 * 128);
+            auto vload = [&](const __amdgpu_buffer_rsrc_t& rs, int x) {
+                return __builtin_bit_cast(f32x2, __builtin_amdgcn_raw_buffer_load_b64(rs, li * 32 + lq * 8, (18 * HALF + x) * 512, 0));
+            };
+            if (VIN) {
+                const __amdgpu_buffer_rsrc_t rs0 = make_rsrc(vitem);
+#pragma unroll
+                for (int x = 0; x < 18; ++x) Vg[x] = vload(rs0, x);
+                if (n == 0) asm volatile("s_waitcnt vmcnt(18)" ::: "memory");
+                else asm volatile("s_waitcnt vmcnt(34)" ::: "memory");
+            } else if (n == 0) asm volatile("s_waitcnt vmcnt(0)" ::: "memory");
             else asm volatile("s_waitcnt vmcnt(16)" ::: "memory");
             lds_barrier();
             stamp(1);
@@ -235,7 +249,7 @@
                 for (int i = 0; i < PAFTER; ++i) issue_piece(i, 1, 1, cb);
             }
             f32x2 R[3][6];
-            rowpass(smem + pbase, R, 0, 6);
+            if (!VIN) rowpass(smem + pbase, R, 0, 6);
             stamp(2);
             for (int kt = 0; kt < nkt; ++kt) {
                 const int st = kt & 1;
@@ -243,13 +257,14 @@
                 const float* san = smem + (st ^ 1) * STAGE + pbase;
                 const bool n1 = kt + 1 < nkt, n2 = kt + 2 < nkt;
                 f32x2 Rn[3][6];
+                const __amdgpu_buffer_rsrc_t vrs = make_rsrc(vitem + (long long)(VIN && n1 ? kt + 1 : 0) * (36 * 128), VIN && n1 ? (int)OOB : 0);
                 f32x4 uf[UPF + 1], ufl[NAFTER];
 #pragma unroll
                 for (int e = 0; e < UPF; ++e) uf[e] = *reinterpret_cast<const f32x4*>(su + (18 * HALF + e) * 256);
 #pragma unroll
                 for (int a = 0; a < 3; ++a) {
                     f32x2 V[6];
-                    bt_full2<FWD>(R[a], V);
+                    if (!VIN) bt_full2<FWD>(R[a], V);
 #pragma unroll
                     for (int b = 0; b < 6; ++b) {
                         const int xl = 6 * a + b;
@@ -263,6 +278,11 @@
                                 __syncthreads();
                                 const unsigned long long tc = __builtin_amdgcn_s_memtime();
                                 t_vm += tb - ta; t_bar += tc - tb;
+                            } else if (VIN) {
+                                static_assert(!VIN || (SB == 12 && PAFTER == 5), "vmcnt arithmetic of the V-input form");
+                                if (kt == 0) asm volatile("s_waitcnt vmcnt(12)" ::: "memory");
+                                else asm volatile("s_waitcnt vmcnt(14)" ::: "memory");
+                                lds_barrier();
                             } else {
                                 asm volatile("s_waitcnt vmcnt(0)" ::: "memory");
                                 __syncthreads();
@@ -271,20 +291,24 @@
                         if (xl + UPF < SB) uf[(xl + UPF) % (UPF + 1)] = *reinterpret_cast<const f32x4*>(su + (18 * HALF + xl + UPF) * 256);
                         if (xl + PAFTER < NPIECE) { if (n1) issue_piece(xl + PAFTER, kt + 1, st ^ 1, cb); }
                         if (xl >= SB) {
-                            if (n2) issue_piece(xl - SB, kt + 2, st, cb);
-                            rowpass(san, Rn, (6 * (xl - SB)) / NAFTER, (6 * (xl - SB + 1)) / NAFTER);
+                            if (n2 && xl - SB < PAFTER) issue_piece(xl - SB, kt + 2, st, cb);
+                            if (!VIN) rowpass(san, Rn, (6 * (xl - SB)) / NAFTER, (6 * (xl - SB + 1)) / NAFTER);
                         }
                         const f32x4 u = xl < SB ? uf[xl % (UPF + 1)] : ufl[xl < SB ? 0 : xl - SB];
-                        acc[xl][0] = __builtin_amdgcn_mfma_f32_16x16x4f32(u[0], V[b][0], acc[xl][0], 0, 0, 0);
-                        acc[xl][1] = __builtin_amdgcn_mfma_f32_16x16x4f32(u[2], V[b][0], acc[xl][1], 0, 0, 0);
-                        acc[xl][0] = __builtin_amdgcn_mfma_f32_16x16x4f32(u[1], V[b][1], acc[xl][0], 0, 0, 0);
-                        acc[xl][1] = __builtin_amdgcn_mfma_f32_16x16x4f32(u[3], V[b][1], acc[xl][1], 0, 0, 0);
+                        const f32x2 vop = VIN ? Vg[VIN ? xl : 0] : V[b];
+                        acc[xl][0] = __builtin_amdgcn_mfma_f32_16x16x4f32(u[0], vop[0], acc[xl][0], 0, 0, 0);
+                        acc[xl][1] = __builtin_amdgcn_mfma_f32_16x16x4f32(u[2], vop[0], acc[xl][1], 0, 0, 0);
+                        acc[xl][0] = __builtin_amdgcn_mfma_f32_16x16x4f32(u[1], vop[1], acc[xl][0], 0, 0, 0);
+                        acc[xl][1] = __builtin_amdgcn_mfma_f32_16x16x4f32(u[3], vop[1], acc[xl][1], 0, 0, 0);
+                        if (VIN) Vg[VIN ? xl : 0] = vload(vrs, xl);
                     }
                 }
-#pragma unroll
-                for (int a = 0; a < 3; ++a)
-#pragma unroll
-                    for (int q = 0; q < 6; ++q) R[a][q] = Rn[a][q];
+                if (!VIN) {
+#pragma unroll
+                    for (int a = 0; a < 3; ++a)
+#pragma unroll
+                        for (int q = 0; q < 6; ++q) R[a][q] = Rn[a][q];
+                }
             }
             stamp(3);
             __syncthreads();
@@ -488,16 +512,7 @@
                 (int)((long long)blockIdx.x - it[7]), (int)it[2]);
 }
 
-__device__ __forceinline__ void bt6(const f32x4 (&d)[6], f32x4 (&o)[6]) {
-    const f32x4 e1 = d[4] - 2.25f * d[2], f1 = 0.75f * d[3] - 1.6875f * d[1];
-    const f32x4 e2 = d[4] - 0.5625f * d[2], f2 = 1.5f * d[3] - 0.84375f * d[1];
-    o[0] = 1.265625f * d[0] + (d[4] - 2.8125f * d[2]);
-    o[1] = e1 + f1;
-    o[2] = e1 - f1;
-    o[3] = e2 + f2;
-    o[4] = e2 - f2;
-    o[5] = 1.265625f * d[1] + (d[5] - 2.8125f * d[3]);
-}
+__device__ __forceinline__ void bt6(const f32x4 (&d)[6], f32x4 (&o)[6]) { vd_wino43_bt6(d, o); }
 __device__ __forceinline__ void a6(const f32x4 (&y)[4], f32x4 (&o)[6]) {
     const f32x4 e1 = y[0] + 0.5625f * y[2], f1 = 0.75f * y[1] + 0.421875f * y[3];
     const f32x4 e2 = y[0] + 2.25f * y[2], f2 = 1.5f * y[1] + 3.375f * y[3];
@@ -514,6 +529,7 @@
     const float* x; long long ldx; const float* dy; long long lddy;
     float* V; float* dM;
     int nimg, H, W, Cin, Cout, TW, TPI, T;
+    int z0;
 };
 
 __global__ __launch_bounds__(256) void wino43_wgrad_transform_kernel(const WgT43 p) {
@@ -522,7 +538,7 @@
     const int img = tile / p.TPI, tin = tile - img * p.TPI;
     const int ty = tin / p.TW, tx = tin - ty * p.TW;
     const int c4 = 4 * quad;
-    if (blockIdx.z == 0) {
+    if (blockIdx.z + p.z0 == 0) {
         if (c4 >= p.Cin) return;
         f32x4 R[6][6];
 #pragma unroll
@@ -768,9 +784,9 @@
 
 extern "C" int vd_conv3x3_wino43_fwd_chunk_rows(int32_t H, int32_t W) { return W == 16 ? H * W : (W == 32 ? H * W : 16 * W); }
 
-extern "C" int vd_conv3x3_wino43_fwd(const float* xin, int64_t ldx, const float* U43f, const float* bias, const float* res, int64_t ldres,
-                                     float* y, int64_t ldy, int32_t nimg, int32_t H, int32_t W, int32_t Cin, int32_t Cout,
-                                     float* stats_part, void* stream) {
+static int wino43_fwd_impl(const float* xin, int64_t ldx, const float* U43f, const float* bias, const float* res, int64_t ldres,
+                           float* y, int64_t ldy, int32_t nimg, int32_t H, int32_t W, int32_t Cin, int32_t Cout,
+                           float* stats_part, void* stream, bool vin) {
     VD_REQUIRE(xin && U43f && y, "vd_conv3x3_wino43_fwd: null operand");
     VD_REQUIRE(vd_conv3x3_wino43_fwd_supported(nimg, H, W, Cin, Cout, ldx, ldy, res ? ldres : 0),
                "vd_conv3x3_wino43_fwd: unsupported geometry nimg=%d H=%d W=%d Cin=%d Cout=%d", nimg, H, W, Cin, Cout);
@@ -792,12 +808,35 @@
     const int ncu = vd_persistent_cus();
     const dim3 grid((unsigned)(items < ncu ? items : ncu)), blk(THREADS);
     hipStream_t st = (hipStream_t)stream;
-    if (W == 16) hipLaunchKernelGGL((wino43_conv_kernel<4, true>), grid, blk, 0, st, a);
+    if (vin) {
+        if (W == 16) hipLaunchKernelGGL((wino43_conv_kernel<4, true, true>), grid, blk, 0, st, a);
+        else if (W == 32) hipLaunchKernelGGL((wino43_conv_kernel<8, true, true>), grid, blk, 0, st, a);
+        else hipLaunchKernelGGL((wino43_conv_kernel<16, true, true>), grid, blk, 0, st, a);
+    } else if (W == 16) hipLaunchKernelGGL((wino43_conv_kernel<4, true>), grid, blk, 0, st, a);
     else if (W == 32) hipLaunchKernelGGL((wino43_conv_kernel<8, true>), grid, blk, 0, st, a);
     else hipLaunchKernelGGL((wino43_conv_kernel<16, true>), grid, blk, 0, st, a);
     VD_LAUNCH_CHECK("wino43_conv_kernel<., true>");
-    g_last43 = -(W / 4);
+    g_last43 = -(W / 4) - (vin ? 100 : 0);
     return 0;
+}
+
+extern "C" int vd_conv3x3_wino43_fwd(const float* xin, int64_t ldx, const float* U43f, const float* bias, const float* res, int64_t ldres,
+                                     float* y, int64_t ldy, int32_t nimg, int32_t H, int32_t W, int32_t Cin, int32_t Cout,
+                                     float* stats_part, void* stream) {
+    return wino43_fwd_impl(xin, ldx, U43f, bias, res, ldres, y, ldy, nimg, H, W, Cin, Cout, stats_part, stream, false);
+}
+
+extern "C" size_t vd_wino43_v_floats(int32_t nimg, int32_t H, int32_t W, int32_t Cin) {
+    return (size_t)36 * (((size_t)nimg * (H / 4) * (W / 4) + 15) / 16 * 16) * Cin;
+}
+extern "C" int vd_conv3x3_wino43_fwd_v_supported(int32_t nimg, int32_t H, int32_t W, int32_t Cin, int32_t Cout, int64_t ldy, int64_t ldres) {
+    return vd_conv3x3_wino43_fwd_supported(nimg, H, W, Cin, Cout, Cin, ldy, ldres) && Cin % 8 == 0;
+}
+extern "C" int vd_conv3x3_wino43_fwd_v(const float* V, const float* U43f, const float* bias, const float* res, int64_t ldres, float* y, int64_t ldy,
+                                       int32_t nimg, int32_t H, int32_t W, int32_t Cin, int32_t Cout, float* stats_part, void* stream) {
+    VD_REQUIRE(vd_conv3x3_wino43_fwd_v_supported(nimg, H, W, Cin, Cout, ldy, res ? ldres : 0),
+               "vd_conv3x3_wino43_fwd_v: unsupported geometry nimg=%d H=%d W=%d Cin=%d Cout=%d", nimg, H, W, Cin, Cout);
+    return wino43_fwd_impl(V, Cin, U43f, bias, res, ldres, y, ldy, nimg, H, W, Cin, Cout, stats_part, stream, true);
 }
 
 extern "C" int vd_wino43_pack_batched(const int64_t* items_dev, int32_t n, int64_t total_blocks, void* stream) {
@@ -825,7 +864,7 @@
 
 static int wgrad43_impl(const float* xin, int64_t ldx, const float* dy, int64_t lddy, int32_t nimg, int32_t H, int32_t W, int32_t Cin,
                         int32_t Cout, float* dw_oihw, float* dbias, int32_t Cin_w, int32_t Cout_w, int32_t accumulate, float* ws,
-                        size_t ws_bytes, void* stream, int phases) {
+                        size_t ws_bytes, void* stream, int phases, bool vin = false) {
     VD_REQUIRE(xin && dy && dw_oihw && ws, "vd_conv3x3_wgrad_wino43: null operand");
     VD_REQUIRE(vd_conv3x3_wgrad_wino43_supported(nimg, H, W, Cin, Cout, ldx, lddy),
                "vd_conv3x3_wgrad_wino43: unsupported geometry nimg=%d H=%d W=%d Cin=%d Cout=%d", nimg, H, W, Cin, Cout);
@@ -833,8 +872,9 @@
     VD_REQUIRE(vd_aligned16(xin) && vd_aligned16(dy) && vd_aligned16(ws), "vd_conv3x3_wgrad_wino43: operands must be 16-byte aligned");
     VD_REQUIRE(ws_bytes >= vd_conv3x3_wgrad_wino43_ws_bytes(nimg, H, W, Cin, Cout), "vd_conv3x3_wgrad_wino43: workspace too small");
     const Wg43Plan g = wg43_plan(nimg, H, W, Cin, Cout);
-    float* V = ws;
-    float* dM = V + g.v_f;
+    VD_REQUIRE(!vin || (Cin % 8 == 0 && g.T % 16 == 0), "vd_conv3x3_wgrad_wino43_v: needs Cin %% 8 == 0 and whole blocks of 16 tiles");
+    float* V = vin ? const_cast<float*>(xin) : ws;
+    float* dM = ws + g.v_f;
     float* dU = dM + g.m_f;
     float* cs = dU + g.u_f;
     float* gws = cs + g.cs_f;
@@ -843,19 +883,20 @@
         WgT43 t = {};
         t.x = xin; t.ldx = ldx; t.dy = dy; t.lddy = lddy; t.V = V; t.dM = dM;
         t.nimg = nimg; t.H = H; t.W = W; t.Cin = Cin; t.Cout = Cout; t.TW = W / 4; t.TPI = (H / 4) * (W / 4); t.T = g.T;
-        const int cmax = Cin > Cout ? Cin : Cout;
-        hipLaunchKernelGGL(wino43_wgrad_transform_kernel, dim3((unsigned)(g.T / 4), (unsigned)((cmax + 255) / 256), 2), dim3(64, 4), 0, st, t);
+        const int cmax = vin ? Cout : (Cin > Cout ? Cin : Cout);
+        t.z0 = vin ? 1 : 0;
+        hipLaunchKernelGGL(wino43_wgrad_transform_kernel, dim3((unsigned)(g.T / 4), (unsigned)((cmax + 255) / 256), vin ? 1 : 2), dim3(64, 4), 0, st, t);
         VD_LAUNCH_CHECK("wino43_wgrad_transform_kernel");
     }
     if (phases & 2) {
         const float* A[36]; const float* B[36]; float* C[36]; float* colsum[36];
         for (int e = 0; e < 36; ++e) {
-            A[e] = dM + (size_t)e * 16 * Cout; B[e] = V + (size_t)e * 16 * Cin;
+            A[e] = dM + (size_t)e * 16 * Cout; B[e] = V + (size_t)e * (vin ? 128 : 16 * Cin);
             C[e] = dU + (size_t)e * Cout * Cin; colsum[e] = cs + (size_t)e * Cout;
         }
-        const int rc = vd_gemm_grouped_wgrad_kblk(A, B, C, colsum, 36, Cout, Cin, g.T, Cout, Cin, Cin, g.S, gws, g.gemm_bytes, stream,
+        const int rc = vd_gemm_grouped_wgrad_kblk(A, B, C, colsum, 36, Cout, Cin, g.T, Cout, vin ? 8 : Cin, Cin, g.S, gws, g.gemm_bytes, stream,
                                                   36LL * 16 * Cout, 36LL * 16 * Cin,
-                                                  (long long)Cout * Cin >= FUSED_FINISH_MIN ? 1 : 0);
+                                                  (long long)Cout * Cin >= FUSED_FINISH_MIN ? 1 : 0, vin ? 36LL * 128 : 0);
         if (rc) return rc;
         g_last43w = g.S;
     }
@@ -888,3 +929,10 @@
 }
 
 extern "C" int vd_wino43_wgrad_last_kernel(void) { return g_last43w; }
+
+extern "C" int vd_conv3x3_wgrad_wino43_v(const float* V, const float* dy, int64_t lddy, int32_t nimg, int32_t H, int32_t W, int32_t Cin,
+                                         int32_t Cout, float* dw_oihw, float* dbias, int32_t Cin_w, int32_t Cout_w, int32_t accumulate,
+                                         float* ws, size_t ws_bytes, int32_t phase, void* stream) {
+    VD_REQUIRE(phase == 7 || phase == 1 || phase == 2 || phase == 4, "vd_conv3x3_wgrad_wino43_v: phase must be 7 (all), 1, 2 or 4");
+    return wgrad43_impl(V, Cin, dy, lddy, nimg, H, W, Cin, Cout, dw_oihw, dbias, Cin_w, Cout_w, accumulate, ws, ws_bytes, stream, phase, true);
+}
diff --git a/v-diffusion-torch_amd/v_diffusion/_hip.py b/v-diffusion-torch_amd/v_diffusion/_hip.py
--- a/v-diffusion-torch_amd/v_diffusion/_hip.py
+++ b/v-diffusion-torch_amd/v_diffusion/_hip.py
@@ -65,6 +65,13 @@
     "vd_conv3x3_wgrad_wino43": (C.c_int, [_vp, _i64, _vp, _i64, _i32, _i32, _i32, _i32, _i32, _vp, _vp, _i32, _i32, _i32, _vp, _sz, _vp]),
     "vd_wino43_wgrad_last_kernel": (C.c_int, []),
     "vd_conv3x3_wgrad_wino43_phase": (C.c_int, [_vp, _i64, _vp, _i64, _i32, _i32, _i32, _i32, _i32, _vp, _vp, _i32, _i32, _i32, _vp, _sz, _i32, _vp]),
+    "vd_wino43_v_floats": (_sz, [_i32, _i32, _i32, _i32]),
+    "vd_conv3x3_wino43_fwd_v_supported": (C.c_int, [_i32, _i32, _i32, _i32, _i32, _i64, _i64]),
+    "vd_conv3x3_wino43_fwd_v": (C.c_int, [_vp, _vp, _vp, _vp, _i64, _vp, _i64, _i32, _i32, _i32, _i32, _i32, _vp, _vp]),
+    "vd_conv3x3_wgrad_wino43_v": (C.c_int, [_vp, _vp, _i64, _i32, _i32, _i32, _i32, _i32, _vp, _vp, _i32, _i32, _i32, _vp, _sz, _i32, _vp]),
+    "vd_gn_apply_from_partials_v_supported": (C.c_int, [_i32, _i32, _i32, _i32, _i32, _i64]),
+    "vd_gn_apply_from_partials_v": (C.c_int, [_vp, _i64, _vp, _i32, _i32, _vp, _i32, _i32, _vp, _vp, _vp, _i32, _f32, _u64, _vp, _i32, _i32,
+                                              _i32, _i32, _i32, _f32, _vp, _vp]),
     "vd_gn_stats_from_partials": (C.c_int, [_vp, _i32, _i32, _vp, _i32, _i32, _i32, _i32, _i32, _f32, _vp, _vp]),
     "vd_gn_coef_from_partials": (C.c_int, [_vp, _i32, _i32, _vp, _i32, _i32, _i32, _i32, _i32, _f32, _vp, _vp, _vp, _vp, _vp]),
     "vd_conv3x3_wgrad_ws_bytes": (_sz, [_i32, _i32, _i32, _i32, _i32]),
@@ -406,7 +413,9 @@
     return int(lib().vd_conv3x3_wino43_fwd_chunk_rows(H, W))
 
 
-def conv3x3_wino43_fwd(x, ldx, U43f, bias, y, ldy, nimg, H, W, Cin, Cout, res=None, ldres=0, stats_part=None):
+def conv3x3_wino43_fwd(x, ldx, U43f, bias, y, ldy, nimg, H, W, Cin, Cout, res=None, ldres=0, stats_part=None, v_input=False):
+    if v_input:
+        return conv3x3_wino43_fwd_v(x, U43f, bias, y, ldy, nimg, H, W, Cin, Cout, res=res, ldres=ldres, stats_part=stats_part)
     name = f"wino43_conv_kernel<{W // 4}, true>"
     with _TimedName(name, 2.0 * nimg * H * W * Cout * 9 * Cin):
         _check(lib().vd_conv3x3_wino43_fwd(ptr(x), ldx, ptr(U43f), ptr(bias), ptr(res), ldres, ptr(y), ldy, nimg, H, W, Cin, Cout,
@@ -475,7 +484,54 @@
         _check(lib().vd_conv3x3_wgrad_wino43_phase(*args, 4, stream()), "vd_conv3x3_wgrad_wino43_phase")
 
 
-def conv3x3_wgrad(x, ldx, dy, lddy, nimg, H, W, Cin, Cout, dw, Cin_w, Cout_w, accumulate=False, dbias=None, direct=False):
+CONV_VIN = os.environ.get("VD_CONV_VIN", "1") != "0"
+
+
+def conv_vin_supported(nimg, H, W, Cin, Cout, ldx, ldy, ldres=0, G=32):
+    return (CONV_VIN and wino43_fwd_supported(nimg, H, W, Cin, Cout, Cin, ldy, ldres)
+            and wgrad43_supported(nimg, H, W, Cin, Cout, Cin, Cout)
+            and bool(lib().vd_conv3x3_wino43_fwd_v_supported(nimg, H, W, Cin, Cout, ldy, ldres))
+            and bool(lib().vd_gn_apply_from_partials_v_supported(nimg, H, W, Cin, G, ldx)))
+
+
+def wino43_v_new(ref, nimg, H, W, Cin):
+    return torch.empty(lib().vd_wino43_v_floats(nimg, H, W, Cin), dtype=torch.float32, device=ref.device)
+
+
+def gn_apply_from_partials_v(x, ldx, parts, gamma, beta, film, act, p_drop, seed, V, nimg, H, W, Cc, coef, G=32, eps=1e-6):
+    with _TimedBytes("gn_apply_v_kernel", 4.0 * nimg * Cc * H * W * (1 + 2.25)):
+        _check(lib().vd_gn_apply_from_partials_v(ptr(x), ldx, *_two_parts(parts), ptr(gamma), ptr(beta), ptr(film), int(act), float(p_drop),
+                                                 int(seed), ptr(V), nimg, H, W, Cc, G, eps, ptr(coef), stream()),
+               "vd_gn_apply_from_partials_v")
+
+
+def conv3x3_wino43_fwd_v(V, U43f, bias, y, ldy, nimg, H, W, Cin, Cout, res=None, ldres=0, stats_part=None):
+    name = f"wino43_conv_kernel<{W // 4}, true, true>"
+    with _TimedName(name, 2.0 * nimg * H * W * Cout * 9 * Cin):
+        _check(lib().vd_conv3x3_wino43_fwd_v(ptr(V), ptr(U43f), ptr(bias), ptr(res), ldres, ptr(y), ldy, nimg, H, W, Cin, Cout,
+                                             ptr(stats_part), stream()), "vd_conv3x3_wino43_fwd_v")
+    _note_bytes(name, 4.0 * (nimg * H * W * (2.25 * Cin + Cout + (Cout if res is not None else 0)) + 36 * Cout * Cin))
+
+
+def conv3x3_wgrad_wino43_v(V, dy, lddy, nimg, H, W, Cin, Cout, dw, Cin_w, Cout_w, accumulate=False, dbias=None):
+    nb = lib().vd_conv3x3_wgrad_wino43_ws_bytes(nimg, H, W, Cin, Cout)
+    ws = workspace(nb, V.device, "wgrad43")
+    args = (ptr(V), ptr(dy), lddy, nimg, H, W, Cin, Cout, ptr(dw), ptr(dbias), Cin_w, Cout_w, int(accumulate), ws.data_ptr(), ws.numel() * 4)
+    if PROFILE is None:
+        _check(lib().vd_conv3x3_wgrad_wino43_v(*args, 7, stream()), "vd_conv3x3_wgrad_wino43_v")
+        return
+    with _TimedBytes("wino43_wgrad_transform_kernel", 4.0 * nimg * H * W * Cout * (1 + 2.25)):
+        _check(lib().vd_conv3x3_wgrad_wino43_v(*args, 1, stream()), "vd_conv3x3_wgrad_wino43_v")
+    with _TimedTile("gemm_dma_kernel<{tile}, 1, 1, true, {kt}, true> " + W43_WGRAD_TAG, 2.0 * nimg * H * W * Cout * 9 * Cin):
+        _check(lib().vd_conv3x3_wgrad_wino43_v(*args, 2, stream()), "vd_conv3x3_wgrad_wino43_v")
+    _note_bytes(PROFILE[-1][0], 4.0 * (36.0 * nimg * (H // 4) * (W // 4) * (Cin + Cout) + 36.0 * Cout * Cin))
+    with _TimedName("wino43_wgrad_finish_kernel", 0.0):
+        _check(lib().vd_conv3x3_wgrad_wino43_v(*args, 4, stream()), "vd_conv3x3_wgrad_wino43_v")
+
+
+def conv3x3_wgrad(x, ldx, dy, lddy, nimg, H, W, Cin, Cout, dw, Cin_w, Cout_w, accumulate=False, dbias=None, direct=False, v_input=False):
+    if v_input:
+        return conv3x3_wgrad_wino43_v(x, dy, lddy, nimg, H, W, Cin, Cout, dw, Cin_w, Cout_w, accumulate, dbias)
     if not direct and wgrad43_supported(nimg, H, W, Cin, Cout, ldx, lddy):
         return conv3x3_wgrad_wino43(x, ldx, dy, lddy, nimg, H, W, Cin, Cout, dw, Cin_w, Cout_w, accumulate, dbias)
     if WINO and not direct and lib().vd_conv3x3_wgrad_wino_supported(nimg, H, W, Cin, Cout, ldx, lddy):
diff --git a/v-diffusion-torch_amd/v_diffusion/engine.py b/v-diffusion-torch_amd/v_diffusion/engine.py
--- a/v-diffusion-torch_amd/v_diffusion/engine.py
+++ b/v-diffusion-torch_amd/v_diffusion/engine.py
@@ -149,6 +149,24 @@
         H.gn_apply(x, _ld(x), stats, gn.weight, gn.bias, film, act, p_drop, seed, rs, y, _ld(y), B, Hh, Ww, C, coef, GROUPS)
         return coef
 
+    def _norm_conv(self, x, x_parts, gn, film, p_drop, seed, rs, conv, y, ldy, B, Hh, Ww, Ho, Wo, Cin, Cout, res, ldres, stats_part, keep):
+        wino = getattr(self, "_wino", None)
+        w = conv.weight
+        ldr = ldres if res is not None else 0
+        if keep and rs == H.RS_NONE and x_parts is not None and H.GN_FOLD and max(k for _, _, k in x_parts) <= H.GN_FOLD_MAX_CHUNKS \
+                and wino is not None and id(w) in wino and wino[id(w)][3] is not None \
+                and H.conv_vin_supported(B, Ho, Wo, Cin, Cout, _ld(x), ldy, ldr, GROUPS):
+            V = H.wino43_v_new(x, B, Ho, Wo, Cin)
+            coef = self._new(x, B, 4, Cin)
+            H.gn_apply_from_partials_v(x, _ld(x), x_parts, gn.weight, gn.bias, film, 1, p_drop, seed, V, B, Hh, Ww, Cin, coef, GROUPS, EPS)
+            H.conv3x3_wino43_fwd(V, Cin, wino[id(w)][3], conv.bias, y, ldy, B, Ho, Wo, Cin, Cout, res=res, ldres=ldr, stats_part=stats_part,
+                                 v_input=True)
+            return coef, V, True, H.wino43_fwd_chunk_rows(Ho, Wo)
+        a = self._new(x, B, Ho, Wo, Cin)
+        coef = self._norm(x, x_parts, gn, film, 1, p_drop, seed, rs, a, B, Hh, Ww, Cin)
+        rows = self._conv(a, Cin, w, conv.bias, y, ldy, B, Ho, Wo, Cin, Cout, res=res, ldres=ldres, stats_part=stats_part)
+        return coef, a, False, rows
+
     def _wgrad(self, dy, x, dw, db, M, N, K, lda, ldb, ldc):
         if self._wq is None or not H.GROUPED_WGRAD:
             H.gemm(dy, x, dw, M, N, K, a_kind=H.COL, b_kind=H.COL, lda=lda, ldb=ldb, ldc=ldc, splitk=_splitk(M, N, K), colsum=db)
@@ -159,15 +177,16 @@
         if len(q) == H.GROUP_MAX:
             self._wgrad_flush_key(key)
 
-    def _cwgrad(self, x, ldx, dy, lddy, *args, **kw):
+    def _cwgrad(self, x, ldx, dy, lddy, *args, vin=False, **kw):
+        run = lambda: H.conv3x3_wgrad(x, ldx, dy, lddy, *args, v_input=vin, **kw)
         side = self._side
         if side is None:
-            return H.conv3x3_wgrad(x, ldx, dy, lddy, *args, **kw)
+            return run()
         side.wait_stream(torch.cuda.current_stream())
         x.record_stream(side)
         dy.record_stream(side)
         with torch.cuda.stream(side):
-            H.conv3x3_wgrad(x, ldx, dy, lddy, *args, **kw)
+            run()
 
     def _side_join(self):
         if self._side is not None:
@@ -497,16 +516,13 @@
         B, Hh, Ww, Cin, ldx = _chk(x)
         Cout, rs = blk.cout, blk.rs
         Ho, Wo = (Hh // 2, Ww // 2) if rs == H.RS_DOWN else ((Hh * 2, Ww * 2) if rs == H.RS_UP else (Hh, Ww))
-        a1 = self._new(x, B, Ho, Wo, Cin)
-        coef1 = self._norm(x, x_parts, mod.norm1, None, 1, 0.0, 0, rs, a1, B, Hh, Ww, Cin)
         h1 = self._new(x, B, Ho, Wo, Cout)
         ph = self._part(x, B, Ho * Wo, Cout)
-        rows = self._conv(a1, Cin, mod.conv1.weight, mod.conv1.bias, h1, Cout, B, Ho, Wo, Cin, Cout, stats_part=ph)
+        coef1, a1, v1, rows = self._norm_conv(x, x_parts, mod.norm1, None, 0.0, 0, rs, mod.conv1, h1, Cout, B, Hh, Ww, Ho, Wo, Cin, Cout,
+                                              None, 0, ph, tape is not None)
         h1_parts = self._parts(ph, Cout, Ho * Wo, rows)
         c2, fi = self.film_slot[prefix]
         film = films[c2][fi]
-        a2 = self._new(x, B, Ho, Wo, Cout)
-        coef2 = self._norm(h1, h1_parts, mod.norm2, film, 1, p_drop, seed, H.RS_NONE, a2, B, Ho, Wo, Cout)
         if rs != H.RS_NONE:
             xs = self._new(x, B, Ho, Wo, Cin)
             H.gn_apply(x, ldx, None, None, None, None, 0, 0.0, 0, rs, xs, Cin, B, Hh, Ww, Cin, None, GROUPS)
@@ -520,12 +536,12 @@
         else:
             sk = xs
         pd = self._part(x, B, Ho * Wo, Cout)
-        rows = self._conv(a2, Cout, mod.conv2.weight, mod.conv2.bias, dest, _ld(dest), B, Ho, Wo, Cout, Cout, res=sk,
-                          ldres=_ld(sk), stats_part=pd)
+        coef2, a2, v2, rows = self._norm_conv(h1, h1_parts, mod.norm2, film, p_drop, seed, H.RS_NONE, mod.conv2, dest, _ld(dest), B, Ho, Wo,
+                                              Ho, Wo, Cout, Cout, sk, _ld(sk), pd, tape is not None)
         out_parts = self._parts(pd, Cout, Ho * Wo, rows)
         if tape is not None:
             tape[prefix] = dict(x=x, coef1=coef1, a1=a1, h1=h1, coef2=coef2, a2=a2, film=film, xs=xs if has_skip else None,
-                                seed=seed, p=p_drop)
+                                seed=seed, p=p_drop, v1=v1, v2=v2)
         return out_parts
 
     def _res_bwd(self, blk, mod, prefix, ctx, dy, dx, dx_accumulate, ta, dfilms, G):
@@ -534,7 +550,7 @@
         _, Ho, Wo, Cout, lddy = _chk(dy)
         rs = blk.rs
         self._cwgrad(a2, Cout, dy, lddy, B, Ho, Wo, Cout, Cout, G[prefix + ".conv2.weight"], Cout, Cout,
-                        dbias=G[prefix + ".conv2.bias"])
+                        dbias=G[prefix + ".conv2.bias"], vin=ctx["v2"])
         da2 = self._new(x, B, Ho, Wo, Cout)
         self._conv(dy, lddy, mod.conv2.weight, None, da2, Cout, B, Ho, Wo, Cout, Cout, dgrad=True)
         dh1 = self._new(x, B, Ho, Wo, Cout)
@@ -545,7 +561,7 @@
                        pgb_keep=self._pgb(B, Cout, G[prefix + ".norm2.weight"], G[prefix + ".norm2.bias"]))
         del da2
         self._cwgrad(a1, Cin, dh1, Cout, B, Ho, Wo, Cin, Cout, G[prefix + ".conv1.weight"], Cin, Cout,
-                        dbias=G[prefix + ".conv1.bias"])
+                        dbias=G[prefix + ".conv1.bias"], vin=ctx["v1"])
         da1 = self._new(x, B, Ho, Wo, Cin)
         self._conv(dh1, Cout, mod.conv1.weight, None, da1, Cin, B, Ho, Wo, Cout, Cin, dgrad=True)
         del dh1
```

After: 2240, median of 4. Within noise of the previous version (+1.3%).
